# ml-jku/LRAM

Hardware: NVIDIA B200
Metric: env-steps/sec batched xLSTM recurrent inference (higher is better)
Workload: dtype f32

## Files before the change

include/xlstm_b200.h:

```cpp
#ifndef XLSTM_B200_H
#define XLSTM_B200_H

#include <stddef.h>
#include <stdint.h>

#ifdef __cplusplus
extern "C" {
#endif
#if defined(__GNUC__)
#pragma GCC visibility push(default)
#endif

#define XL_ABI_VERSION 3

typedef enum {
  XL_OK = 0,
  XL_ERR_INVALID_ARG = -1,
  XL_ERR_UNSUPPORTED = -2,
  XL_ERR_CUDA = -3,
  XL_ERR_NOT_READY = -4,
  XL_ERR_NO_DEVICE = -5
} xl_status;

typedef struct xl_handle xl_handle;

typedef struct {
  int32_t embedding_dim;
  int32_t num_blocks;
  int32_t num_heads;
  int32_t inner_dim;
  int32_t conv_kernel;
  int32_t qkv_blocksize;
  int32_t state_dim;
  int32_t act_dim;
  int32_t action_channels;
  int32_t discrete_actions;
  int32_t tokens_per_step;
  int32_t action_token_pos;
  int32_t max_batch;
  float ln_eps;
  float cell_eps;
  float embed_ln_eps;
  float tok_min_val;
  float tok_max_val;
  uint32_t slstm_mask_lo;
  uint32_t slstm_mask_hi;
  int32_t ffn_dim;
} xl_config;

typedef enum {
  XL_W_XLSTM_NORM = 0,
  XL_W_PROJ_UP = 1,
  XL_W_Q_PROJ = 2,
  XL_W_K_PROJ = 3,
  XL_W_V_PROJ = 4,
  XL_W_CONV_W = 5,
  XL_W_CONV_B = 6,
  XL_W_IGATE_W = 7,
  XL_W_IGATE_B = 8,
  XL_W_FGATE_W = 9,
  XL_W_FGATE_B = 10,
  XL_W_OUTNORM = 11,
  XL_W_SKIP = 12,
  XL_W_PROJ_DOWN = 13,
  XL_W_S_GATE_I = 14,
  XL_W_S_GATE_F = 15,
  XL_W_S_GATE_Z = 16,
  XL_W_S_GATE_O = 17,
  XL_W_S_RECURRENT = 18,
  XL_W_S_BIAS = 19,
  XL_W_S_GROUP_NORM = 20,
  XL_W_FFN_NORM = 21,
  XL_W_FFN_UP = 22,
  XL_W_FFN_DOWN = 23,
  XL_W_PER_BLOCK_COUNT = 24,
  XL_W_POST_NORM = 32,
  XL_W_EMBED_STATE_W = 33,
  XL_W_EMBED_STATE_B = 34,
  XL_W_EMBED_RETURN_W = 35,
  XL_W_EMBED_RETURN_B = 36,
  XL_W_EMBED_REWARD_W = 37,
  XL_W_EMBED_REWARD_B = 38,
  XL_W_EMBED_LN_W = 39,
  XL_W_EMBED_LN_B = 40,
  XL_W_HEAD_W = 41,
  XL_W_HEAD_B = 42
} xl_weight_id;

typedef enum { XL_STATE_C = 0, XL_STATE_N = 1, XL_STATE_M = 2, XL_STATE_CONV = 3, XL_STATE_SLSTM = 4 } xl_state_part;

#define XL_MODE_PER_TOKEN 0
#define XL_MODE_FUSED 1

#define XL_FLAG_DISCRETE 1u
#define XL_FLAG_GRAPH 2u
#define XL_FLAG_SIMPLE_GEMM 4u
#define XL_FLAG_STATE_EMBEDS 8u

int xl_abi_version(void);
const char* xl_last_error(void);

int xl_create(const xl_config* cfg, xl_handle** out);
void xl_destroy(xl_handle* h);

int xl_state_dim_padded(const xl_handle* h);

int xl_bind_weight(xl_handle* h, int layer, int which, const void* dev_ptr, int dtype, int64_t numel);
int xl_weights_ready(const xl_handle* h);
int xl_encoder_weights_ready(const xl_handle* h);

size_t xl_state_bytes(const xl_handle* h, int B);
int xl_state_layout(const xl_handle* h, int B, int layer, int part, size_t* offset_bytes, size_t* size_bytes);

int xl_state_reset(xl_handle* h, void* state, const uint8_t* env_mask, int B, void* stream);

int xl_set_token_ring(xl_handle* h, int32_t* ring, int slots, int next_slot, void* stream);

typedef struct {
  float temperature;
  float top_p;
  int32_t top_k;
  int32_t env_id_base;
  int32_t env_id_stride;
  uint64_t seed;
} xl_sampling;
int xl_set_sampling(xl_handle* h, const xl_sampling* params, uint32_t step0, void* stream);
int xl_sample_actions(xl_handle* h, const float* logits, int B, unsigned flags, const xl_sampling* params,
                      uint32_t step, int32_t* tokens, float* actions, void* stream);

int xl_encoder_step(xl_handle* h, void* state, const float* x_in, float* x_out, int B, int T, int mode,
                    unsigned flags, void* stream);

int xl_mlstm_cell_step(xl_handle* h, float* C, float* n, float* m, const float* qkv, const float* igate,
                       const float* fgate, const float* outnorm_w, float* h_norm, float* h_raw, int B, int T,
                       int rows_split, int cols_per_cta, void* stream);

int xl_policy_step(xl_handle* h, void* state, const float* states, const float* rtg, const float* rewards,
                   int32_t* tokens, float* actions, float* logits, float* hidden, int B, int mode,
                   unsigned flags, void* stream);

int xl_policy_step_host(xl_handle* h, void* state, const float* h_states, const float* h_rtg,
                        const float* h_rewards, int32_t* h_tokens, float* h_actions, int B, int mode,
                        unsigned flags, void* stream);

int xl_prefill(xl_handle* h, void* state, const float* x_in, float* y_out, int B, int S, unsigned flags, void* stream);

int xl_policy_prefill(xl_handle* h, void* state, const float* states, const float* rtg, const float* rewards, int B,
                      int Tn, unsigned flags, void* stream);

int xl_prefill_ragged(xl_handle* h, void* state, const float* x_in, float* y_out, const int32_t* lengths, int B, int S,
                      unsigned flags, void* stream);
int xl_policy_prefill_ragged(xl_handle* h, void* state, const float* states, const float* rtg, const float* rewards,
                             const int32_t* lengths, int B, int Tn, unsigned flags, void* stream);

typedef struct {
  int32_t* tokens;
  float* actions;
  float* logits;
  const int32_t* targets;
  float* logprobs;
} xl_seq_outputs;

int xl_policy_forward(xl_handle* h, void* state, const float* states, const float* rtg, const float* rewards,
                      const int32_t* lengths, int B, int Tn, const xl_seq_outputs* out, unsigned flags, void* stream);

int xl_policy_prefill_embeds(xl_handle* h, void* state, const float* state_embeds, const float* rtg,
                             const float* rewards, const int32_t* lengths, int B, int Tn, unsigned flags,
                             void* stream);
int xl_policy_forward_embeds(xl_handle* h, void* state, const float* state_embeds, const float* rtg,
                             const float* rewards, const int32_t* lengths, int B, int Tn, const xl_seq_outputs* out,
                             unsigned flags, void* stream);

int xl_linear(xl_handle* h, const float* A, const void* W_bf16, const float* bias, const float* residual,
              float* out, int M, int N, int K, int impl, void* stream);

int xl_set_option(xl_handle* h, const char* name, int value);

int64_t xl_launch_count(xl_handle* h);

int xl_profile_begin(xl_handle* h);
int xl_profile_end(xl_handle* h, double* state_kernel_ms, int64_t* state_kernel_launches, double* step_ms);

#if defined(__GNUC__)
#pragma GCC visibility pop
#endif
#ifdef __cplusplus
}
#endif
#endif
```

lram_b200/_lib.py:

```python
from __future__ import annotations

import ctypes as C
import os
import re

HERE = os.path.dirname(os.path.abspath(__file__))
LIB_PATH = os.path.join(HERE, "libxlstm_b200.so")
HEADER_PATH = os.path.join(os.path.dirname(HERE), "include", "xlstm_b200.h")

XL_OK = 0
XL_ERR_INVALID_ARG, XL_ERR_UNSUPPORTED, XL_ERR_CUDA, XL_ERR_NOT_READY, XL_ERR_NO_DEVICE = -1, -2, -3, -4, -5

XL_MODE_PER_TOKEN, XL_MODE_FUSED = 0, 1
XL_FLAG_DISCRETE, XL_FLAG_GRAPH, XL_FLAG_SIMPLE_GEMM, XL_FLAG_STATE_EMBEDS = 1, 2, 4, 8

XL_STATE_C, XL_STATE_N, XL_STATE_M, XL_STATE_CONV, XL_STATE_SLSTM = 0, 1, 2, 3, 4
XL_ABI_VERSION = 3

W = dict(
    XLSTM_NORM=0, PROJ_UP=1, Q_PROJ=2, K_PROJ=3, V_PROJ=4, CONV_W=5, CONV_B=6, IGATE_W=7, IGATE_B=8,
    FGATE_W=9, FGATE_B=10, OUTNORM=11, SKIP=12, PROJ_DOWN=13,
    S_GATE_I=14, S_GATE_F=15, S_GATE_Z=16, S_GATE_O=17, S_RECURRENT=18, S_BIAS=19, S_GROUP_NORM=20,
    FFN_NORM=21, FFN_UP=22, FFN_DOWN=23,
    POST_NORM=32, EMBED_STATE_W=33, EMBED_STATE_B=34, EMBED_RETURN_W=35, EMBED_RETURN_B=36,
    EMBED_REWARD_W=37, EMBED_REWARD_B=38, EMBED_LN_W=39, EMBED_LN_B=40, HEAD_W=41, HEAD_B=42,
)


class XLConfig(C.Structure):
    _fields_ = [
        ("embedding_dim", C.c_int32), ("num_blocks", C.c_int32), ("num_heads", C.c_int32),
        ("inner_dim", C.c_int32), ("conv_kernel", C.c_int32), ("qkv_blocksize", C.c_int32),
        ("state_dim", C.c_int32), ("act_dim", C.c_int32), ("action_channels", C.c_int32),
        ("discrete_actions", C.c_int32), ("tokens_per_step", C.c_int32), ("action_token_pos", C.c_int32),
        ("max_batch", C.c_int32),
        ("ln_eps", C.c_float), ("cell_eps", C.c_float), ("embed_ln_eps", C.c_float),
        ("tok_min_val", C.c_float), ("tok_max_val", C.c_float),
        ("slstm_mask_lo", C.c_uint32), ("slstm_mask_hi", C.c_uint32), ("ffn_dim", C.c_int32),
    ]


class XLSampling(C.Structure):
    _fields_ = [("temperature", C.c_float), ("top_p", C.c_float), ("top_k", C.c_int32), ("env_id_base", C.c_int32),
                ("env_id_stride", C.c_int32), ("seed", C.c_uint64)]


class XLSeqOutputs(C.Structure):
    _fields_ = [("tokens", C.c_void_p), ("actions", C.c_void_p), ("logits", C.c_void_p), ("targets", C.c_void_p),
                ("logprobs", C.c_void_p)]


class XLError(RuntimeError):
    def __init__(self, code: int, msg: str):
        super().__init__(f"xlstm_b200 error {code}: {msg}")
        self.code = code


_lib = None


def declared_symbols():
    with open(HEADER_PATH) as fh:
        src = fh.read()
    src = re.sub(r"/\*.*?\*/", "", src, flags=re.S)
    return sorted(set(re.findall(r"\b(xl_[a-z_0-9]+)\s*\(", src)))


def load():
    global _lib
    if _lib is not None:
        return _lib
    if not os.path.exists(LIB_PATH):
        from . import build as _build
        _build.build()
    if not os.path.exists(LIB_PATH):
        raise RuntimeError(f"{LIB_PATH} is missing and could not be built: the xlstm_b200 path has no "
                           f"CPU fallback")
    lib = C.CDLL(LIB_PATH)
    vp, i32, i64, u32, sz = C.c_void_p, C.c_int, C.c_int64, C.c_uint, C.c_size_t
    lib.xl_abi_version.restype = i32
    lib.xl_last_error.restype = C.c_char_p
    lib.xl_create.argtypes = [C.POINTER(XLConfig), C.POINTER(vp)]
    lib.xl_create.restype = i32
    lib.xl_destroy.argtypes = [vp]
    lib.xl_destroy.restype = None
    lib.xl_state_dim_padded.argtypes = [vp]
    lib.xl_state_dim_padded.restype = i32
    lib.xl_bind_weight.argtypes = [vp, i32, i32, vp, i32, i64]
    lib.xl_bind_weight.restype = i32
    lib.xl_weights_ready.argtypes = [vp]
    lib.xl_weights_ready.restype = i32
    lib.xl_encoder_weights_ready.argtypes = [vp]
    lib.xl_encoder_weights_ready.restype = i32
    lib.xl_state_bytes.argtypes = [vp, i32]
    lib.xl_state_bytes.restype = sz
    lib.xl_state_layout.argtypes = [vp, i32, i32, i32, C.POINTER(sz), C.POINTER(sz)]
    lib.xl_state_layout.restype = i32
    lib.xl_state_reset.argtypes = [vp, vp, vp, i32, vp]
    lib.xl_state_reset.restype = i32
    lib.xl_encoder_step.argtypes = [vp, vp, vp, vp, i32, i32, i32, u32, vp]
    lib.xl_encoder_step.restype = i32
    lib.xl_mlstm_cell_step.argtypes = [vp, vp, vp, vp, vp, vp, vp, vp, vp, vp, i32, i32, i32, i32, vp]
    lib.xl_mlstm_cell_step.restype = i32
    lib.xl_policy_step.argtypes = [vp, vp, vp, vp, vp, vp, vp, vp, vp, i32, i32, u32, vp]
    lib.xl_policy_step.restype = i32
    lib.xl_policy_step_host.argtypes = [vp, vp, vp, vp, vp, vp, vp, i32, i32, u32, vp]
    lib.xl_policy_step_host.restype = i32
    lib.xl_prefill.argtypes = [vp, vp, vp, vp, i32, i32, u32, vp]
    lib.xl_prefill.restype = i32
    lib.xl_policy_prefill.argtypes = [vp, vp, vp, vp, vp, i32, i32, u32, vp]
    lib.xl_policy_prefill.restype = i32
    lib.xl_prefill_ragged.argtypes = [vp, vp, vp, vp, vp, i32, i32, u32, vp]
    lib.xl_prefill_ragged.restype = i32
    lib.xl_policy_prefill_ragged.argtypes = [vp, vp, vp, vp, vp, vp, i32, i32, u32, vp]
    lib.xl_policy_prefill_ragged.restype = i32
    lib.xl_policy_forward.argtypes = [vp, vp, vp, vp, vp, vp, i32, i32, C.POINTER(XLSeqOutputs), u32, vp]
    lib.xl_policy_forward.restype = i32
    lib.xl_policy_prefill_embeds.argtypes = [vp, vp, vp, vp, vp, vp, i32, i32, u32, vp]
    lib.xl_policy_prefill_embeds.restype = i32
    lib.xl_policy_forward_embeds.argtypes = [vp, vp, vp, vp, vp, vp, i32, i32, C.POINTER(XLSeqOutputs), u32, vp]
    lib.xl_policy_forward_embeds.restype = i32
    lib.xl_linear.argtypes = [vp, vp, vp, vp, vp, vp, i32, i32, i32, i32, vp]
    lib.xl_linear.restype = i32
    lib.xl_set_token_ring.argtypes = [vp, vp, i32, i32, vp]
    lib.xl_set_token_ring.restype = i32
    lib.xl_set_sampling.argtypes = [vp, C.POINTER(XLSampling), u32, vp]
    lib.xl_set_sampling.restype = i32
    lib.xl_sample_actions.argtypes = [vp, vp, i32, u32, C.POINTER(XLSampling), u32, vp, vp, vp]
    lib.xl_sample_actions.restype = i32
    lib.xl_set_option.argtypes = [vp, C.c_char_p, i32]
    lib.xl_set_option.restype = i32
    lib.xl_profile_begin.argtypes = [vp]
    lib.xl_profile_begin.restype = i32
    lib.xl_profile_end.argtypes = [vp, C.POINTER(C.c_double), C.POINTER(i64), C.POINTER(C.c_double)]
    lib.xl_profile_end.restype = i32
    lib.xl_launch_count.argtypes = [vp]
    lib.xl_launch_count.restype = i64
    _lib = lib
    return lib


def check(rc: int):
    if rc != XL_OK:
        raise XLError(rc, load().xl_last_error().decode("utf-8", "replace"))
```

lram_b200/csrc/xl_api.cu:

```cuda
#include <cuda_bf16.h>
#include <cuda_runtime.h>

#include <algorithm>
#include <cmath>
#include <cstdarg>
#include <cstdio>
#include <cstring>
#include <new>
#include <utility>
#include <vector>

#include "../../include/xlstm_b200.h"
#include "xl_internal.h"

namespace {

thread_local char g_err[512] = "";

int fail(int code, const char* fmt, ...) {
  va_list ap;
  va_start(ap, fmt);
  vsnprintf(g_err, sizeof(g_err), fmt, ap);
  va_end(ap);
  return code;
}

#define XL_CUDA(expr)                                                                          \
  do {                                                                                         \
    cudaError_t _e = (expr);                                                                   \
    if (_e != cudaSuccess)                                                                     \
      return fail(XL_ERR_CUDA, "%s failed: %s (%s:%d)", #expr, cudaGetErrorString(_e), __FILE__, \
                  __LINE__);                                                                   \
  } while (0)

inline size_t align_up(size_t v, size_t a) { return (v + a - 1) / a * a; }

struct BlockWeights {
  const void* w[XL_W_PER_BLOCK_COUNT];
};

struct GraphCacheEntry {
  cudaGraphExec_t exec = nullptr;
  void* state = nullptr;
  const void *states = nullptr, *rtg = nullptr, *rewards = nullptr;
  void *tokens = nullptr, *actions = nullptr, *logits = nullptr, *hidden = nullptr;
  int B = 0, mode = 0;
  unsigned flags = 0;
  int64_t launches = 0;
};

}

constexpr int kCntRing = 0, kCntSample = 1, kCntUnitStep = 2, kCntArmed = 8, kCntUnit = 16;
constexpr int kMaxMicro = 8;
constexpr int kSplitMax = 8;
constexpr size_t kSplitRows = 1024;

struct xl_handle {
  xl_config cfg;
  int device = 0;
  int num_sms = 148;
  int DH = 0, NCH = 0, Kpad = 0, head_out = 0, num_actions = 0;
  uint64_t slstm_mask = 0;
  std::vector<BlockWeights> blocks;
  const void* pw[16];
  char* ws = nullptr;
  size_t ws_bytes = 0;
  float *x = nullptr, *xn = nullptr, *u = nullptr, *qkv = nullptr, *act = nullptr, *gate_part = nullptr,
        *gated = nullptr, *partial = nullptr, *s_emb = nullptr, *states_pad = nullptr, *logits = nullptr,
        *d_states = nullptr, *d_rtg = nullptr, *d_rew = nullptr, *d_actions = nullptr, *xtok = nullptr, *hid = nullptr;
  float* d_embeds = nullptr;
  int32_t* d_tokens = nullptr;
  unsigned int* counters = nullptr;
  __nv_bfloat16 *a_hi = nullptr, *a_lo = nullptr;
  int64_t launches = 0;
  std::vector<GraphCacheEntry> graphs;
  size_t a_cap = 0;
  size_t a_env = 0;
  int num_tickets = 0;
  cudaStream_t cap_stream = nullptr;
  cudaStream_t side[kMaxMicro - 1] = {};
  cudaEvent_t ev_fork = nullptr, ev_join[kMaxMicro - 1] = {}, ev_state[kMaxMicro] = {};
  int state_impl = 1;
  int state_stages = 0;
  int state_ctas_per_sm = 0;
  int state_rows_split = 0;
  int fuse_ends = 1;
  int up_fuse = 0;
  int gp_chunks = 16;
  int state_fuse = 0;
  int small_state_fuse = 0;
  int gemm_impl = 0;
  int gemm_splitk = 8;
  int gemm_up_bn = 0, gemm_up_splits = 0, gemm_down_bn = 0, gemm_down_splits = 0;
  int debug_skip = 0;
  float *part_up = nullptr, *part_down = nullptr;
  size_t part_rows = 0;
  int l2_prefetch_policy = 0;
  int conv_impl = 2;
  int microbatches = 0;
  int pipeline_order = 1;
  int l2_prefetch_mb = -1;
  char* pf_buf = nullptr;
  int pf_rows = 0;
  size_t pf_gsc_floats = 0;
  float *pf_x = nullptr, *pf_xn = nullptr, *pf_u = nullptr, *pf_qkv = nullptr, *pf_act = nullptr, *pf_gp = nullptr,
        *pf_gated = nullptr, *pf_num = nullptr, *pf_qn = nullptr, *pf_f = nullptr, *pf_i = nullptr, *pf_m = nullptr,
        *pf_semb = nullptr, *pf_spad = nullptr, *pf_sin = nullptr, *pf_rtg = nullptr, *pf_rew = nullptr, *pf_gsc = nullptr;
  __nv_bfloat16 *pf_hi = nullptr, *pf_lo = nullptr;
  uint8_t *pf_pc = nullptr, *pf_pv = nullptr;
  char* rg_state = nullptr;
  size_t rg_state_bytes = 0;
  int32_t* rg_idx = nullptr;
  std::vector<int32_t> rg_host;
  float* sq_logits = nullptr;
  size_t sq_logits_floats = 0;
  int prefill_gemm_2cta = 0;
  int prefill_rows = 16384;
  char* pf_tc = nullptr;
  size_t pf_tc_bytes = 0;
  int prefill_cell = 2;
  int smallm = -1;
  int host_zero_copy = 1;
  std::vector<std::pair<const void*, void*>> host_map;
  int32_t* tok_ring = nullptr;
  int tok_slots = 0;
  bool sampling = false;
  bool profiling = false;
  std::vector<cudaEvent_t> prof_state;
  std::vector<cudaEvent_t> prof_step;
};

namespace {

struct StateLayout {
  size_t c_off, n_off, m_off, conv_off, layer_bytes;
  size_t s_off, sconv_off, slayer_bytes;
};

inline bool is_slstm(const xl_handle* h, int i) { return (h->slstm_mask >> i) & 1ull; }

StateLayout state_layout(const xl_handle* h, int B) {
  const xl_config& c = h->cfg;
  StateLayout L;
  size_t off = 0;
  L.c_off = off;
  off = align_up(off + sizeof(float) * (size_t)B * c.num_heads * h->DH * h->DH, 256);
  L.n_off = off;
  off = align_up(off + sizeof(float) * (size_t)B * c.num_heads * h->DH, 256);
  L.m_off = off;
  off = align_up(off + sizeof(float) * (size_t)B * c.num_heads, 256);
  L.conv_off = off;
  off = align_up(off + sizeof(float) * (size_t)B * c.conv_kernel * c.inner_dim, 256);
  L.layer_bytes = off;
  off = 0;
  L.s_off = off;
  off = align_up(off + sizeof(float) * (size_t)4 * B * c.embedding_dim, 256);
  L.sconv_off = off;
  off = align_up(off + sizeof(float) * (size_t)B * c.conv_kernel * c.embedding_dim, 256);
  L.slayer_bytes = off;
  return L;
}

size_t layer_base(const xl_handle* h, const StateLayout& L, int i) {
  const uint64_t below = i >= 64 ? ~0ull : ((1ull << i) - 1ull);
  const int ns = __builtin_popcountll(h->slstm_mask & below);
  return (size_t)(i - ns) * L.layer_bytes + (size_t)ns * L.slayer_bytes;
}

int check_batch(const xl_handle* h, int B) {
  if (!h) return fail(XL_ERR_INVALID_ARG, "null handle");
  if (B <= 0 || B > h->cfg.max_batch)
    return fail(XL_ERR_INVALID_ARG, "B=%d outside [1, max_batch=%d]", B, h->cfg.max_batch);
  return XL_OK;
}

struct Ws {
  float *x, *xn, *xtok, *hid, *u, *qkv, *act, *gate_part, *gated, *partial, *s_emb, *states_pad, *logits;
  __nv_bfloat16 *a_hi, *a_lo;
  size_t a_cap;
  int low_smem;
};

Ws ws_slice(const xl_handle* h, int b0, int Bk) {
  const xl_config& c = h->cfg;
  const size_t d = c.embedding_dim, inner = c.inner_dim, e = (size_t)b0;
  Ws w;
  w.x = h->x + e * 4 * d; w.xn = h->xn + e * 4 * d; w.xtok = h->xtok + e * 4 * d; w.hid = h->hid + e * 4 * d;
  w.u = h->u + e * 4 * 2 * inner; w.qkv = h->qkv + e * 4 * 3 * inner; w.act = h->act + e * 4 * inner;
  w.gate_part = h->gate_part + e * 4 * h->gp_chunks * 2 * c.num_heads; w.gated = h->gated + e * 4 * inner;
  w.partial = h->partial + e * c.num_heads * 32 * 4 * h->DH;
  w.s_emb = h->s_emb + e * d; w.states_pad = h->states_pad + e * h->Kpad; w.logits = h->logits + e * h->head_out;
  w.a_hi = h->a_hi + e * h->a_env; w.a_lo = h->a_lo + e * h->a_env;
  w.a_cap = (size_t)Bk * h->a_env;
  w.low_smem = 0;
  return w;
}

int linear(xl_handle* h, const Ws& w, const float* A, const void* W, const float* bias, const float* residual,
           float* out, int M, int N, int K, int impl, cudaStream_t s, bool presplit = false, int bn = 0,
           int splits = 1, long long split_stride = 0) {
  if (K % 8 != 0) return fail(XL_ERR_UNSUPPORTED, "linear: K=%d must be a multiple of 8", K);
  const bool tc_ok = xl::gemm_tc_supported(M, N, K) && (size_t)M * K <= w.a_cap;
  if (impl == 2 && !tc_ok)
    return fail(XL_ERR_UNSUPPORTED, "linear: tcgen05 path needs K %% 64 == 0 and M*K <= %zu (got M=%d K=%d)",
                w.a_cap, M, K);
  if (impl == 2 || (impl == 0 && tc_ok)) {
    if (!presplit) {
      xl::launch_split_bf16(A, K, w.a_hi, w.a_lo, M, K, s);
      h->launches += 1;
    }
    XL_CUDA(xl::launch_gemm_tc(w.a_hi, w.a_lo, (const __nv_bfloat16*)W, bias, residual, out, M, N, K,
                               h->num_sms, bn, splits, split_stride, w.low_smem, s));
    h->launches += 1;
    return XL_OK;
  }
  if (splits > 1) return fail(XL_ERR_INVALID_ARG, "linear: split-K needs the tcgen05 path");
  xl::launch_gemm_simple(A, (const __nv_bfloat16*)W, bias, residual, out, M, N, K, s);
  h->launches += 1;
  XL_CUDA(cudaGetLastError());
  return XL_OK;
}

struct Slice {
  int B, b0, Bk;
  Ws ws;
  cudaStream_t s;
};

Slice make_slice(const xl_handle* h, int B, int b0, int Bk, cudaStream_t s) {
  Slice sl;
  sl.B = B; sl.b0 = b0; sl.Bk = Bk; sl.s = s;
  sl.ws = ws_slice(h, b0, Bk);
  return sl;
}

int smallm_chunks(const xl_handle* h, const Slice& sl, int T, unsigned flags) {
  const xl_config& c = h->cfg;
  if (!h->smallm || h->debug_skip || (flags & XL_FLAG_SIMPLE_GEMM)) return 0;
  if (h->smallm < 0 && (sl.Bk * T > 4 || c.embedding_dim > 1024)) return 0;
  if (sl.b0 != 0 || sl.Bk != sl.B || sl.ws.low_smem) return 0;
  return xl::smallm_pre_chunks(sl.Bk, T, c.embedding_dim, c.inner_dim, c.num_heads, c.conv_kernel);
}

constexpr unsigned kFlagLn0DoneEarly = 1u << 29;
constexpr unsigned kFlagHeadOnlyEarly = 1u << 28;

struct BlockPlan {
  bool tc_up, tc_down;
  bool up_fused;
  int impl;
  int up_bn, up_sp, down_bn, down_sp;
};

BlockPlan block_plan(const xl_handle* h, const Slice& sl, int T, unsigned flags) {
  const xl_config& c = h->cfg;
  const int M = sl.Bk * T;
  BlockPlan p;
  p.impl = (flags & XL_FLAG_SIMPLE_GEMM) ? 1 : h->gemm_impl;
  p.tc_up = p.impl != 1 && xl::gemm_tc_supported(M, 2 * c.inner_dim, c.embedding_dim) &&
            (size_t)M * c.embedding_dim <= sl.ws.a_cap;
  p.tc_down = p.impl != 1 && xl::gemm_tc_supported(M, c.embedding_dim, c.inner_dim) &&
              (size_t)M * c.inner_dim <= sl.ws.a_cap;
  const bool can_split = !sl.ws.low_smem && sl.b0 == 0 && (size_t)M <= h->part_rows && c.embedding_dim <= 4096 &&
                         !smallm_chunks(h, sl, T, flags);
  const int max_sp = can_split ? std::min(std::max(h->gemm_splitk, 1), kSplitMax) : 1;
  p.up_bn = p.down_bn = 0;
  p.up_sp = p.down_sp = 1;
  if (p.tc_up) {
    xl::gemm_tc_plan(M, 2 * c.inner_dim, c.embedding_dim, h->num_sms, max_sp, &p.up_bn, &p.up_sp);
    if (h->gemm_up_bn) p.up_bn = h->gemm_up_bn;
    if (h->gemm_up_splits && can_split && (c.embedding_dim / 64) % h->gemm_up_splits == 0 &&
        h->gemm_up_splits <= kSplitMax)
      p.up_sp = h->gemm_up_splits;
  }
  p.up_fused = h->up_fuse && p.tc_up && !sl.ws.low_smem && !h->debug_skip && !smallm_chunks(h, sl, T, flags) &&
               xl::gemm_up_conv_chunks(c.inner_dim) <= h->gp_chunks &&
               xl::gemm_up_conv_supported(T, c.conv_kernel, c.num_heads, c.inner_dim, c.embedding_dim);
  if (p.up_fused) { p.up_bn = 64; p.up_sp = 1; }
  if (p.tc_down) {
    xl::gemm_tc_plan(M, c.embedding_dim, c.inner_dim, h->num_sms, max_sp, &p.down_bn, &p.down_sp);
    if (h->gemm_down_bn) p.down_bn = h->gemm_down_bn;
    if (h->gemm_down_splits && can_split && (c.inner_dim / 64) % h->gemm_down_splits == 0 &&
        h->gemm_down_splits <= kSplitMax)
      p.down_sp = h->gemm_down_splits;
  }
  return p;
}

xl::StateStepParams state_params(const xl_handle* h, void* state, const Slice& sl, int i, int T, bool tc_down,
                                 int up_sp = 1, int small_nch = 0, bool up_fused = false) {
  const xl_config& c = h->cfg;
  const int inner = c.inner_dim, NH = c.num_heads, DH = h->DH;
  const StateLayout L = state_layout(h, sl.B);
  const BlockWeights& w = h->blocks[i];
  char* base = (char*)state + layer_base(h, L, i);
  const int M = sl.Bk * T;
  xl::StateStepParams sp;
  memset(&sp, 0, sizeof(sp));
  sp.C = (float*)(base + L.c_off) + (size_t)sl.b0 * NH * DH * DH;
  sp.n = (float*)(base + L.n_off) + (size_t)sl.b0 * NH * DH;
  sp.m = (float*)(base + L.m_off) + (size_t)sl.b0 * NH;
  sp.qk = sl.ws.qkv;
  sp.v = sl.ws.qkv + (size_t)2 * M * inner;
  sp.gate_part = sl.ws.gate_part;
  sp.igate_b = (const float*)w.w[XL_W_IGATE_B];
  sp.fgate_b = (const float*)w.w[XL_W_FGATE_B];
  sp.outnorm_w = (const float*)w.w[XL_W_OUTNORM];
  sp.skip = (const float*)w.w[XL_W_SKIP];
  sp.act = sl.ws.act;
  sp.u = up_sp > 1 ? h->part_up : sl.ws.u;
  sp.u_splits = up_sp;
  sp.u_stride = (int64_t)M * 2 * inner;
  sp.out = tc_down ? nullptr : sl.ws.gated;
  sp.out_hi = tc_down ? sl.ws.a_hi : nullptr;
  sp.out_lo = tc_down ? sl.ws.a_lo : nullptr;
  sp.partial = sl.ws.partial;
  sp.B = sl.Bk; sp.T = T; sp.NH = NH; sp.DH = DH; sp.inner = inner; sp.NCH = h->NCH;
  if (small_nch) sp.NCH = small_nch;
  if (up_fused) sp.NCH = xl::gemm_up_conv_chunks(inner);
  sp.ln_eps = c.ln_eps; sp.cell_eps = c.cell_eps;
  sp.impl = h->state_impl; sp.num_layers = c.num_blocks;
  sp.stages = h->state_stages; sp.ctas_per_sm = h->state_ctas_per_sm; sp.rows_split = h->state_rows_split;
  sp.fuse_finalize = (h->debug_skip & (8 | 16)) ? 0 : h->state_fuse;
  if (small_nch && h->state_fuse == 0 && h->small_state_fuse) {
    sp.fuse_finalize = 2;
    sp.max_cluster = h->small_state_fuse > 1 ? h->small_state_fuse : 0;
  }
  if (sl.ws.low_smem) {
    if (sp.stages <= 0) sp.stages = 4;
    sp.meta_slots = 2;
  }
  return sp;
}

int block_pre(xl_handle* h, void* state, const Slice& sl, int i, int T, unsigned flags) {
  const xl_config& c = h->cfg;
  const int d = c.embedding_dim, inner = c.inner_dim, NH = c.num_heads;
  const int M = sl.Bk * T;
  const StateLayout L = state_layout(h, sl.B);
  const BlockPlan bp = block_plan(h, sl, T, flags);
  const BlockWeights& w = h->blocks[i];
  const Ws& ws = sl.ws;
  char* base = (char*)state + layer_base(h, L, i);
  if (const int nch = smallm_chunks(h, sl, T, flags)) {
    xl::SmallPreParams sp;
    memset(&sp, 0, sizeof(sp));
    sp.x = ws.x;
    sp.norm_w = (const float*)w.w[XL_W_XLSTM_NORM];
    sp.w_up = (const __nv_bfloat16*)w.w[XL_W_PROJ_UP];
    sp.conv_w = (const float*)w.w[XL_W_CONV_W]; sp.conv_b = (const float*)w.w[XL_W_CONV_B];
    sp.wq = (const float*)w.w[XL_W_Q_PROJ]; sp.wk = (const float*)w.w[XL_W_K_PROJ]; sp.wv = (const float*)w.w[XL_W_V_PROJ];
    sp.wi = (const float*)w.w[XL_W_IGATE_W]; sp.wf = (const float*)w.w[XL_W_FGATE_W];
    sp.conv_state = (float*)(base + L.conv_off);
    sp.u = ws.u; sp.qk = ws.qkv; sp.v = ws.qkv + (size_t)2 * M * inner; sp.act = ws.act;
    sp.gate_part = ws.gate_part;
    sp.B = sl.Bk; sp.T = T; sp.d = d; sp.inner = inner; sp.NH = NH; sp.NCH = nch;
    sp.ln_eps = c.ln_eps;
    XL_CUDA(xl::launch_smallm_pre(sp, sl.s));
    h->launches += 1;
    return XL_OK;
  }
  if (h->debug_skip & 1) {
  } else if (i == 0 && (flags & kFlagLn0DoneEarly)) {
    h->launches -= 1;
  } else if (i > 0 && bp.down_sp > 1 && !is_slstm(h, i - 1)) {
    xl::launch_ln_rows_reduce(ws.x, h->part_down, bp.down_sp, (int64_t)M * d, bp.tc_up ? nullptr : ws.xn, d,
                              (const float*)w.w[XL_W_XLSTM_NORM], c.ln_eps, M, d, bp.tc_up ? ws.a_hi : nullptr,
                              bp.tc_up ? ws.a_lo : nullptr, sl.s);
  } else {
    xl::launch_ln_rows(ws.x, d, bp.tc_up ? nullptr : ws.xn, d, (const float*)w.w[XL_W_XLSTM_NORM], nullptr, 1,
                       c.ln_eps, M, d, bp.tc_up ? ws.a_hi : nullptr, bp.tc_up ? ws.a_lo : nullptr, sl.s);
  }
  h->launches += 1;
  if (bp.up_fused) {
    xl::UpEpiParams ep;
    ep.conv_state = (float*)(base + L.conv_off) + (size_t)sl.b0 * c.conv_kernel * inner;
    ep.conv_w = (const float*)w.w[XL_W_CONV_W]; ep.conv_b = (const float*)w.w[XL_W_CONV_B];
    ep.wq = (const float*)w.w[XL_W_Q_PROJ]; ep.wk = (const float*)w.w[XL_W_K_PROJ]; ep.wv = (const float*)w.w[XL_W_V_PROJ];
    ep.wi = (const float*)w.w[XL_W_IGATE_W]; ep.wf = (const float*)w.w[XL_W_FGATE_W];
    ep.qk = ws.qkv; ep.v = ws.qkv + (size_t)2 * M * inner; ep.act = ws.act; ep.gate_part = ws.gate_part;
    ep.B = sl.Bk; ep.T = T; ep.inner = inner; ep.NCH = xl::gemm_up_conv_chunks(inner);
    XL_CUDA(xl::launch_gemm_up_conv(ws.a_hi, ws.a_lo, (const __nv_bfloat16*)w.w[XL_W_PROJ_UP], ws.u, M, d, ep, sl.s));
    h->launches += 1;
    return XL_OK;
  }
  int rc = (h->debug_skip & 2) ? 0 : linear(h, ws, ws.xn, w.w[XL_W_PROJ_UP], nullptr, nullptr,
                  bp.up_sp > 1 ? h->part_up : ws.u, M, 2 * inner,
                  d, bp.impl, sl.s, bp.tc_up, bp.up_bn, bp.up_sp, (long long)M * 2 * inner);
  if (rc) return rc;
  if (h->debug_skip & 4) return XL_OK;
  xl::ConvQkvParams cp;
  cp.u = bp.up_sp > 1 ? h->part_up : ws.u;
  cp.u_splits = bp.up_sp;
  cp.u_stride = (int64_t)M * 2 * inner;
  cp.conv_state = (float*)(base + L.conv_off) + (size_t)sl.b0 * c.conv_kernel * inner;
  cp.conv_w = (const float*)w.w[XL_W_CONV_W];
  cp.conv_b = (const float*)w.w[XL_W_CONV_B];
  cp.wq = (const float*)w.w[XL_W_Q_PROJ];
  cp.wk = (const float*)w.w[XL_W_K_PROJ];
  cp.wv = (const float*)w.w[XL_W_V_PROJ];
  cp.wi = (const float*)w.w[XL_W_IGATE_W];
  cp.wf = (const float*)w.w[XL_W_FGATE_W];
  cp.qk = ws.qkv;
  cp.v = ws.qkv + (size_t)2 * M * inner;
  cp.act = ws.act;
  cp.gate_part = ws.gate_part;
  cp.B = sl.Bk; cp.T = T; cp.inner = inner; cp.NH = NH; cp.KS = c.conv_kernel; cp.NCH = h->NCH;
  cp.impl = h->conv_impl;
  if (!xl::launch_conv_qkv_gates(cp, sl.s))
    return fail(XL_ERR_UNSUPPORTED, "conv/qkv kernel not instantiated for KS=%d T=%d NH=%d", cp.KS, cp.T, cp.NH);
  h->launches += 1;
  return XL_OK;
}

int block_state(xl_handle* h, void* state, const Slice& sl, int i, int T, unsigned flags) {
  const BlockPlan bp = block_plan(h, sl, T, flags);
  const int small_nch = smallm_chunks(h, sl, T, flags);
  const xl::StateStepParams sp = small_nch ? state_params(h, state, sl, i, T, false, 1, small_nch)
                                           : state_params(h, state, sl, i, T, bp.tc_down, bp.up_sp, 0, bp.up_fused);
  cudaEvent_t pe0 = nullptr, pe1 = nullptr;
  if (h->profiling) {
    XL_CUDA(cudaEventCreate(&pe0));
    XL_CUDA(cudaEventCreate(&pe1));
    XL_CUDA(cudaEventRecord(pe0, sl.s));
  }
  if (!(h->debug_skip & 8)) XL_CUDA(xl::launch_state_step(sp, h->num_sms, sl.s));
  h->launches += 1;
  if (h->profiling) {
    XL_CUDA(cudaEventRecord(pe1, sl.s));
    h->prof_state.push_back(pe0);
    h->prof_state.push_back(pe1);
  }
  return XL_OK;
}

int block_post(xl_handle* h, void* state, const Slice& sl, int i, int T, unsigned flags) {
  const xl_config& c = h->cfg;
  const BlockPlan bp = block_plan(h, sl, T, flags);
  const int small_nch = smallm_chunks(h, sl, T, flags);
  const Ws& ws = sl.ws;
  const int M = sl.Bk * T;
  if (small_nch) {
    xl::StateStepParams sp = state_params(h, state, sl, i, T, false, 1, small_nch);
    const bool fused = xl::state_step_fuses_finalize(sp, h->num_sms);
    if (!fused) XL_CUDA(xl::launch_state_finalize(sp, h->num_sms, sl.s));
    xl::SmallDownParams dp;
    dp.g = ws.gated; dp.w_down = (const __nv_bfloat16*)h->blocks[i].w[XL_W_PROJ_DOWN]; dp.x = ws.x;
    dp.M = M; dp.d = c.embedding_dim; dp.inner = c.inner_dim;
    XL_CUDA(xl::launch_smallm_down(dp, sl.s));
    h->launches += fused ? 1 : 2;
    return XL_OK;
  }
  const xl::StateStepParams sp = state_params(h, state, sl, i, T, bp.tc_down, bp.up_sp, small_nch, bp.up_fused);
  if (!xl::state_step_fuses_finalize(sp, h->num_sms)) {
    if (!(h->debug_skip & 16)) XL_CUDA(xl::launch_state_finalize(sp, h->num_sms, sl.s));
    h->launches += 1;
  }
  if (h->debug_skip & 32) return XL_OK;
  if (bp.down_sp > 1)
    return linear(h, ws, ws.gated, h->blocks[i].w[XL_W_PROJ_DOWN], nullptr, nullptr, h->part_down, M,
                  c.embedding_dim, c.inner_dim, bp.impl, sl.s, bp.tc_down, bp.down_bn, bp.down_sp,
                  (long long)M * c.embedding_dim);
  return linear(h, ws, ws.gated, h->blocks[i].w[XL_W_PROJ_DOWN], nullptr, ws.x, ws.x, M, c.embedding_dim,
                c.inner_dim, bp.impl, sl.s, bp.tc_down, bp.down_bn);
}

int slstm_block(xl_handle* h, void* state, const Ws& ws, int Btot, int b0, int Bk, int i, int T, unsigned flags,
                int pend_sp, cudaStream_t s, const int32_t* len = nullptr, int pos = 0) {
  const xl_config& c = h->cfg;
  const int d = c.embedding_dim, NH = c.num_heads, ff = c.ffn_dim, KS = c.conv_kernel, M = Bk * T;
  const StateLayout L = state_layout(h, Btot);
  const BlockWeights& w = h->blocks[i];
  char* base = (char*)state + layer_base(h, L, i);
  float* st = (float*)(base + L.s_off) + (size_t)b0 * d;
  float* conv = (float*)(base + L.sconv_off) + (size_t)b0 * KS * d;
  const int impl = (flags & XL_FLAG_SIMPLE_GEMM) ? 1 : h->gemm_impl;
  const bool tc_up = impl != 1 && xl::gemm_tc_supported(M, 2 * ff, d) && (size_t)M * d <= ws.a_cap;
  const bool tc_down = impl != 1 && xl::gemm_tc_supported(M, d, ff) && (size_t)M * ff <= ws.a_cap;
  auto F = [&](int id) { return (const float*)w.w[id]; };
  if (pend_sp > 1)
    xl::launch_ln_rows_reduce(ws.x, h->part_down, pend_sp, (int64_t)M * d, ws.xn, d, F(XL_W_XLSTM_NORM), c.ln_eps, M,
                              d, nullptr, nullptr, s);
  else
    xl::launch_ln_rows(ws.x, d, ws.xn, d, F(XL_W_XLSTM_NORM), nullptr, 1, c.ln_eps, M, d, nullptr, nullptr, s);
  if (!xl::launch_slstm_conv(ws.xn, conv, F(XL_W_CONV_W), F(XL_W_CONV_B), ws.act, Bk, T, d, KS, s, len, pos))
    return fail(XL_ERR_UNSUPPORTED, "sLSTM conv kernel not instantiated for KS=%d", KS);
  xl::launch_slstm_gates(ws.act, ws.xn, F(XL_W_S_GATE_I), F(XL_W_S_GATE_F), F(XL_W_S_GATE_Z), F(XL_W_S_GATE_O),
                         F(XL_W_S_BIAS), ws.u, M, d, NH, s);
  for (int t = 0; t < T; ++t)
    XL_CUDA(xl::launch_slstm_cell(ws.u, F(XL_W_S_RECURRENT), st, ws.gated, Bk, Btot, T, t, d, NH, s, len, pos));
  xl::launch_slstm_out(ws.gated, F(XL_W_S_GROUP_NORM), ws.x, st, M, T, d, NH, c.ln_eps, s);
  xl::launch_ln_rows(ws.x, d, tc_up ? nullptr : ws.xn, d, F(XL_W_FFN_NORM), nullptr, 1, c.ln_eps, M, d,
                     tc_up ? ws.a_hi : nullptr, tc_up ? ws.a_lo : nullptr, s);
  h->launches += 5 + T;
  int rc = linear(h, ws, ws.xn, w.w[XL_W_FFN_UP], nullptr, nullptr, ws.qkv, M, 2 * ff, d, impl, s, tc_up);
  if (rc) return rc;
  xl::launch_ffn_gate(ws.qkv, tc_down ? nullptr : ws.gated, tc_down ? ws.a_hi : nullptr, tc_down ? ws.a_lo : nullptr,
                      M, ff, s);
  h->launches += 1;
  rc = linear(h, ws, ws.gated, w.w[XL_W_FFN_DOWN], nullptr, ws.x, ws.x, M, d, ff, impl, s, tc_down);
  if (rc) return rc;
  XL_CUDA(cudaGetLastError());
  return XL_OK;
}

int pending_planes(const xl_handle* h, const Slice& sl, int i, int T, unsigned flags) {
  if (i == 0 || is_slstm(h, i - 1)) return 1;
  return block_plan(h, sl, T, flags).down_sp;
}

void final_norm(xl_handle* h, const Slice& sl, int T, unsigned flags, float* out, int64_t out_stride) {
  const xl_config& c = h->cfg;
  const int d = c.embedding_dim, M = sl.Bk * T;
  const BlockPlan bp = block_plan(h, sl, T, flags);
  const float* post_w = (const float*)h->pw[XL_W_POST_NORM - XL_W_POST_NORM];
  if (bp.down_sp > 1 && !is_slstm(h, c.num_blocks - 1))
    xl::launch_ln_rows_reduce(sl.ws.x, h->part_down, bp.down_sp, (int64_t)M * d, out, out_stride, post_w, c.ln_eps,
                              M, d, nullptr, nullptr, sl.s);
  else
    xl::launch_ln_rows(sl.ws.x, d, out, out_stride, post_w, nullptr, 1, c.ln_eps, M, d, nullptr, nullptr, sl.s);
  h->launches += 1;
}

int run_blocks(xl_handle* h, void* state, const Slice& sl, int T, unsigned flags) {
  const int L = h->cfg.num_blocks;
  const StateLayout lay = state_layout(h, sl.B);
  const size_t c_bytes = sizeof(float) * (size_t)sl.B * h->cfg.num_heads * h->DH * h->DH;
  int warm_mb = h->l2_prefetch_mb;
  if (warm_mb < 0) warm_mb = (c_bytes >= ((size_t)100 << 20) && c_bytes <= ((size_t)300 << 20)) ? 48 : 0;
  const bool warm = warm_mb > 0 && sl.b0 == 0 && sl.Bk == sl.B && L > 1;
  const size_t warm_bytes = std::min(c_bytes, (size_t)warm_mb << 20);
  int rc = XL_OK;
  for (int i = 0; i < L && !rc; ++i) {
    if (is_slstm(h, i)) {
      rc = slstm_block(h, state, sl.ws, sl.B, sl.b0, sl.Bk, i, T, flags, pending_planes(h, sl, i, T, flags), sl.s);
      continue;
    }
    rc = block_pre(h, state, sl, i, T, flags);
    if (!rc) rc = block_state(h, state, sl, i, T, flags);
    if (!rc && warm) {
      XL_CUDA(cudaEventRecord(h->ev_state[0], sl.s));
      XL_CUDA(cudaStreamWaitEvent(h->side[0], h->ev_state[0], 0));
      int nx = (i + 1) % L;
      while (is_slstm(h, nx) && nx != i) nx = (nx + 1) % L;
      const char* next_c = (const char*)state + layer_base(h, lay, nx) + lay.c_off;
      xl::launch_l2_prefetch(next_c, warm_bytes, h->num_sms, h->l2_prefetch_policy, h->side[0]);
      h->launches += 1;
    }
    if (!rc) rc = block_post(h, state, sl, i, T, flags);
  }
  if (warm) {
    cudaEventRecord(h->ev_join[0], h->side[0]);
    cudaStreamWaitEvent(sl.s, h->ev_join[0], 0);
  }
  if (rc) return rc;
  XL_CUDA(cudaGetLastError());
  return XL_OK;
}

int run_encoder(xl_handle* h, void* state, const Slice& sl, const float* x_in, float* x_out, int T, int mode,
                unsigned flags) {
  const xl_config& c = h->cfg;
  const int d = c.embedding_dim;
  const int B = sl.Bk;
  const Ws& ws = sl.ws;
  cudaStream_t s = sl.s;
  const float* post_w = (const float*)h->pw[XL_W_POST_NORM - XL_W_POST_NORM];
  if (mode == XL_MODE_FUSED || T == 1) {
    if (x_in != ws.x) {
      XL_CUDA(cudaMemcpyAsync(ws.x, x_in, sizeof(float) * (size_t)B * T * d, cudaMemcpyDeviceToDevice, s));
    }
    int rc = run_blocks(h, state, sl, T, flags);
    if (rc) return rc;
    if (!(flags & kFlagHeadOnlyEarly)) final_norm(h, sl, T, flags, x_out, d);
  } else if (mode == XL_MODE_PER_TOKEN) {
    const float* src = x_in;
    if (x_in == x_out) {
      XL_CUDA(cudaMemcpyAsync(ws.xtok, x_in, sizeof(float) * (size_t)B * T * d, cudaMemcpyDeviceToDevice, s));
      src = ws.xtok;
    }
    for (int t = 0; t < T; ++t) {
      xl::launch_copy_rows(src + (size_t)t * d, (int64_t)T * d, ws.x, d, B, d, s);
      h->launches += 1;
      int rc = run_blocks(h, state, sl, 1, flags);
      if (rc) return rc;
      final_norm(h, sl, 1, flags, x_out + (size_t)t * d, (int64_t)T * d);
    }
  } else {
    return fail(XL_ERR_INVALID_ARG, "unknown mode %d", mode);
  }
  XL_CUDA(cudaGetLastError());
  return XL_OK;
}

constexpr unsigned kFlagLn0Done = 1u << 29;
constexpr unsigned kFlagHeadOnly = 1u << 28;
constexpr unsigned kFlagNoRing = 1u << 30;

struct StepArgs {
  void* state;
  const float *states, *rtg, *rewards;
  int32_t* tokens;
  float *actions, *logits, *hidden;
  int B, mode;
  unsigned flags;
};

int policy_front(xl_handle* h, const StepArgs& a, const Slice& sl, float* xt) {
  const xl_config& c = h->cfg;
  const int d = c.embedding_dim;
  const int impl = (a.flags & XL_FLAG_SIMPLE_GEMM) ? 1 : h->gemm_impl;
  auto PW = [&](int id) { return h->pw[id - XL_W_POST_NORM]; };
  const Ws& ws = sl.ws;
  const float* s_emb = ws.s_emb;
  if (a.flags & XL_FLAG_STATE_EMBEDS) {
    s_emb = a.states + (size_t)sl.b0 * d;
  } else {
    const bool tc = impl != 1 && xl::gemm_tc_supported(sl.Bk, d, h->Kpad) && (size_t)sl.Bk * h->Kpad <= ws.a_cap;
    if (tc) {
      xl::launch_pad_split(a.states + (size_t)sl.b0 * c.state_dim, c.state_dim, ws.a_hi, ws.a_lo, h->Kpad, sl.Bk, sl.s);
    } else {
      xl::launch_pad_rows(a.states + (size_t)sl.b0 * c.state_dim, c.state_dim, ws.states_pad, h->Kpad, sl.Bk, sl.s);
    }
    h->launches += 1;
    int rc = linear(h, ws, ws.states_pad, PW(XL_W_EMBED_STATE_W), (const float*)PW(XL_W_EMBED_STATE_B), nullptr,
                    ws.s_emb, sl.Bk, d, h->Kpad, impl, sl.s, tc);
    if (rc) return rc;
  }
  const float* ln0_w = nullptr;
  float* xn0 = nullptr;
  void *hi0 = nullptr, *lo0 = nullptr;
  if (a.flags & kFlagLn0Done) {
    const BlockPlan bp = block_plan(h, sl, c.tokens_per_step, a.flags);
    ln0_w = (const float*)h->blocks[0].w[XL_W_XLSTM_NORM];
    if (bp.tc_up) { hi0 = ws.a_hi; lo0 = ws.a_lo; } else { xn0 = ws.xn; }
  }
  xl::launch_embed_tokens(s_emb, a.rtg + sl.b0, a.rewards ? a.rewards + sl.b0 : nullptr,
                          (const float*)PW(XL_W_EMBED_RETURN_W), (const float*)PW(XL_W_EMBED_RETURN_B),
                          (const float*)PW(XL_W_EMBED_REWARD_W), (const float*)PW(XL_W_EMBED_REWARD_B),
                          (const float*)PW(XL_W_EMBED_LN_W), (const float*)PW(XL_W_EMBED_LN_B), c.embed_ln_eps, xt,
                          sl.Bk, d, (h->tok_ring && sl.b0 == 0 && !(a.flags & kFlagNoRing)) ? h->counters + kCntRing : nullptr,
                          (h->sampling && sl.b0 == 0 && !(a.flags & kFlagNoRing)) ? h->counters + kCntSample : nullptr,
                          ln0_w, c.ln_eps, xn0, hi0, lo0, sl.s);
  h->launches += 1;
  return XL_OK;
}

int policy_back(xl_handle* h, const StepArgs& a, const Slice& sl, const float* hid) {
  const xl_config& c = h->cfg;
  const int d = c.embedding_dim, T = c.tokens_per_step;
  const int impl = (a.flags & XL_FLAG_SIMPLE_GEMM) ? 1 : h->gemm_impl;
  auto PW = [&](int id) { return h->pw[id - XL_W_POST_NORM]; };
  const Ws& ws = sl.ws;
  cudaStream_t s = sl.s;
  const int Bk = sl.Bk;
  float* xa = ws.s_emb;
  const bool head_only = (a.flags & kFlagHeadOnly) != 0;
  if (head_only) {
    const BlockPlan bp = block_plan(h, sl, T, a.flags);
    const int pend = is_slstm(h, c.num_blocks - 1) ? 1 : bp.down_sp;
    xl::launch_ln_rows_gather(ws.x, h->part_down, pend, (int64_t)Bk * T * d, (const float*)PW(XL_W_POST_NORM), c.ln_eps,
                              Bk, d, T, c.action_token_pos, ws.a_hi, ws.a_lo, s);
  } else {
    xl::launch_copy_rows(hid + (size_t)c.action_token_pos * d, (int64_t)T * d, xa, d, Bk, d, s);
  }
  h->launches += 1;
  const bool discrete = (a.flags & XL_FLAG_DISCRETE) != 0;
  const int n_out = discrete ? h->num_actions : h->head_out;
  int32_t* tokens = a.tokens + (size_t)sl.b0 * c.act_dim;
  float* actions = a.actions + (size_t)sl.b0 * c.act_dim;
  float* logits = a.logits ? a.logits + (size_t)sl.b0 * n_out : nullptr;
  int rc;
  int32_t* ring = (h->tok_ring && !(a.flags & kFlagNoRing)) ? h->tok_ring + (size_t)sl.b0 * c.act_dim : nullptr;
  const int64_t ring_stride = (int64_t)a.B * c.act_dim;
  const bool sample = h->sampling && !(a.flags & kFlagNoRing);
  const float bw = (c.tok_max_val - c.tok_min_val) / (float)c.action_channels;
  if (discrete) {
    rc = linear(h, ws, xa, PW(XL_W_HEAD_W), (const float*)PW(XL_W_HEAD_B), nullptr, ws.logits, Bk, n_out, d, impl, s,
                head_only);
    if (rc) return rc;
    if (logits) {
      XL_CUDA(cudaMemcpyAsync(logits, ws.logits, sizeof(float) * (size_t)Bk * n_out, cudaMemcpyDeviceToDevice, s));
    }
    if (sample)
      xl::launch_sample_tokens(ws.logits, n_out, Bk, c.act_dim, n_out, c.discrete_actions, 1, 0.f, 0.f, tokens, actions,
                               ring, h->counters + kCntRing, h->tok_slots, ring_stride, h->counters + kCntArmed,
                               h->counters + kCntSample, sl.b0, s);
    else
      xl::launch_argmax_tokens(ws.logits, n_out, Bk, c.act_dim, n_out, c.discrete_actions, 1, 0.f, 0.f, tokens,
                               actions, ring, h->counters + kCntRing, h->tok_slots, ring_stride, s);
  } else {
    float* lg = logits ? logits : ws.logits;
    rc = linear(h, ws, xa, PW(XL_W_HEAD_W), (const float*)PW(XL_W_HEAD_B), nullptr, lg, Bk, n_out, d, impl, s, head_only);
    if (rc) return rc;
    if (sample)
      xl::launch_sample_tokens(lg, h->head_out, Bk, c.act_dim, h->num_actions, c.discrete_actions, 0, bw, c.tok_min_val,
                               tokens, actions, ring, h->counters + kCntRing, h->tok_slots, ring_stride,
                               h->counters + kCntArmed, h->counters + kCntSample, sl.b0, s);
    else
      xl::launch_argmax_tokens(lg, h->head_out, Bk, c.act_dim, h->num_actions, c.discrete_actions, 0, bw,
                               c.tok_min_val, tokens, actions, ring, h->counters + kCntRing, h->tok_slots, ring_stride, s);
  }
  h->launches += 1;
  return XL_OK;
}

int pick_microbatches(const xl_handle* h, int B, int mode) {
  if (mode != XL_MODE_FUSED) return 1;
  int mb = h->microbatches > 0 ? h->microbatches : 1;
  if (mb > kMaxMicro) mb = kMaxMicro;
  if (mb > B) mb = B;
  return mb < 1 ? 1 : mb;
}

int run_policy(xl_handle* h, const StepArgs& a, cudaStream_t s) {
  const xl_config& c = h->cfg;
  const int d = c.embedding_dim, T = c.tokens_per_step;
  const float* post_w = (const float*)h->pw[XL_W_POST_NORM - XL_W_POST_NORM];
  const int MB = pick_microbatches(h, a.B, a.mode);
  if (MB == 1) {
    const Slice sl = make_slice(h, a.B, 0, a.B, s);
    float* xt = (a.mode == XL_MODE_FUSED) ? sl.ws.x : sl.ws.xtok;
    StepArgs af = a;
    if (h->fuse_ends && a.mode == XL_MODE_FUSED && !h->debug_skip) {
      if (!is_slstm(h, 0) && !smallm_chunks(h, sl, T, a.flags)) af.flags |= kFlagLn0Done;
      const int impl = (a.flags & XL_FLAG_SIMPLE_GEMM) ? 1 : h->gemm_impl;
      const int n_out = (a.flags & XL_FLAG_DISCRETE) ? h->num_actions : h->head_out;
      if (!a.hidden && impl != 1 && xl::gemm_tc_supported(a.B, n_out, d) && (size_t)a.B * d <= sl.ws.a_cap &&
          d <= 4096)
        af.flags |= kFlagHeadOnly;
    }
    const StepArgs& a = af;
    int rc = policy_front(h, a, sl, xt);
    if (rc) return rc;
    float* hid = a.hidden ? a.hidden : sl.ws.hid;
    rc = run_encoder(h, a.state, sl, xt, hid, T, a.mode, a.flags);
    if (rc) return rc;
    rc = policy_back(h, a, sl, hid);
    if (rc) return rc;
    XL_CUDA(cudaGetLastError());
    return XL_OK;
  }
  Slice sl[kMaxMicro];
  int b0 = 0;
  for (int k = 0; k < MB; ++k) {
    const int Bk = a.B / MB + (k < a.B % MB ? 1 : 0);
    sl[k] = make_slice(h, a.B, b0, Bk, k == 0 ? s : h->side[k - 1]);
    sl[k].ws.low_smem = 1;
    b0 += Bk;
  }
  XL_CUDA(cudaEventRecord(h->ev_fork, s));
  for (int k = 1; k < MB; ++k) XL_CUDA(cudaStreamWaitEvent(sl[k].s, h->ev_fork, 0));
  int rc = XL_OK;
  for (int k = 0; k < MB && !rc; ++k) rc = policy_front(h, a, sl[k], sl[k].ws.x);
  for (int i = 0; i < c.num_blocks && !rc; ++i) {
    if (is_slstm(h, i)) {
      for (int k = 0; k < MB && !rc; ++k)
        rc = slstm_block(h, a.state, sl[k].ws, a.B, sl[k].b0, sl[k].Bk, i, T, a.flags,
                         pending_planes(h, sl[k], i, T, a.flags), sl[k].s);
      continue;
    }
    for (int k = 0; k < MB && !rc; ++k) rc = block_pre(h, a.state, sl[k], i, T, a.flags);
    for (int k = 0; k < MB && !rc; ++k) {
      if (h->pipeline_order && !(i == 0 && k == 0)) {
        XL_CUDA(cudaStreamWaitEvent(sl[k].s, h->ev_state[(k + MB - 1) % MB], 0));
      }
      rc = block_state(h, a.state, sl[k], i, T, a.flags);
      if (!rc && h->pipeline_order) XL_CUDA(cudaEventRecord(h->ev_state[k], sl[k].s));
    }
    for (int k = 0; k < MB && !rc; ++k) rc = block_post(h, a.state, sl[k], i, T, a.flags);
  }
  for (int k = 0; k < MB && !rc; ++k) {
    float* hid = a.hidden ? a.hidden + (size_t)sl[k].b0 * T * d : sl[k].ws.hid;
    final_norm(h, sl[k], T, a.flags, hid, d);
    rc = policy_back(h, a, sl[k], hid);
  }
  for (int k = 1; k < MB; ++k) {
    cudaEventRecord(h->ev_join[k - 1], sl[k].s);
    cudaStreamWaitEvent(s, h->ev_join[k - 1], 0);
  }
  if (rc) return rc;
  XL_CUDA(cudaGetLastError());
  return XL_OK;
}

int ensure_prefill_ws(xl_handle* h, int rows, size_t gsc_floats) {
  if (rows <= h->pf_rows && gsc_floats <= h->pf_gsc_floats) return XL_OK;
  rows = std::max(rows, h->pf_rows);
  gsc_floats = std::max(gsc_floats, h->pf_gsc_floats);
  const xl_config& c = h->cfg;
  const size_t d = c.embedding_dim, inner = c.inner_dim, NH = c.num_heads, R = (size_t)rows;
  const size_t kmax = std::max(std::max(inner, d), (size_t)h->Kpad);
  size_t off = 0;
  auto carve = [&](size_t bytes) {
    size_t o = off;
    off = align_up(off + bytes, 256);
    return o;
  };
  const size_t o_x = carve(4 * R * d), o_xn = carve(4 * R * d), o_u = carve(4 * R * 2 * inner);
  const size_t o_qkv = carve(4 * R * 3 * inner), o_act = carve(4 * R * inner), o_gp = carve(4 * R * 16 * 2 * NH);
  const size_t o_gated = carve(4 * R * inner), o_num = carve(4 * R * inner), o_qn = carve(4 * R * NH);
  const size_t o_f = carve(4 * R * NH), o_i = carve(4 * R * NH), o_m = carve(4 * R * NH);
  const size_t o_semb = carve(4 * R * d), o_spad = carve(4 * R * h->Kpad), o_sin = carve(4 * R * c.state_dim);
  const size_t o_rtg = carve(4 * R), o_rew = carve(4 * R);
  const size_t o_gsc = carve(4 * gsc_floats);
  const size_t o_hi = carve(2 * R * kmax), o_lo = carve(2 * R * kmax);
  size_t pc_bytes = 0, pv_bytes = 0;
  if (xl::prefill_cell_mma_supported(h->DH)) xl::prefill_cell_mma_ws(rows, (int)NH, h->DH, &pc_bytes, &pv_bytes);
  const size_t o_pc = carve(pc_bytes), o_pv = carve(pv_bytes);
  XL_CUDA(cudaDeviceSynchronize());
  if (h->pf_buf) cudaFree(h->pf_buf);
  h->pf_buf = nullptr;
  h->pf_rows = 0;
  h->pf_gsc_floats = 0;
  cudaError_t e = cudaMalloc((void**)&h->pf_buf, off);
  if (e != cudaSuccess) return fail(XL_ERR_CUDA, "cudaMalloc(prefill workspace %zu B) failed: %s", off, cudaGetErrorString(e));
  char* b = h->pf_buf;
  h->pf_x = (float*)(b + o_x); h->pf_xn = (float*)(b + o_xn); h->pf_u = (float*)(b + o_u);
  h->pf_qkv = (float*)(b + o_qkv); h->pf_act = (float*)(b + o_act); h->pf_gp = (float*)(b + o_gp);
  h->pf_gated = (float*)(b + o_gated); h->pf_num = (float*)(b + o_num); h->pf_qn = (float*)(b + o_qn);
  h->pf_f = (float*)(b + o_f); h->pf_i = (float*)(b + o_i); h->pf_m = (float*)(b + o_m);
  h->pf_semb = (float*)(b + o_semb); h->pf_spad = (float*)(b + o_spad); h->pf_sin = (float*)(b + o_sin);
  h->pf_rtg = (float*)(b + o_rtg); h->pf_rew = (float*)(b + o_rew);
  h->pf_gsc = (float*)(b + o_gsc);
  h->pf_hi = (__nv_bfloat16*)(b + o_hi); h->pf_lo = (__nv_bfloat16*)(b + o_lo);
  h->pf_pc = (uint8_t*)(b + o_pc); h->pf_pv = (uint8_t*)(b + o_pv);
  h->pf_rows = rows;
  h->pf_gsc_floats = gsc_floats;
  return XL_OK;
}

int ensure_prefill_tc_ws(xl_handle* h, int B, int Sc) {
  const size_t need = xl::prefill_cell_tc_ws_bytes(B, Sc, h->cfg.num_heads, h->DH);
  if (need <= h->pf_tc_bytes) return XL_OK;
  XL_CUDA(cudaDeviceSynchronize());
  if (h->pf_tc) cudaFree(h->pf_tc);
  h->pf_tc = nullptr;
  h->pf_tc_bytes = 0;
  cudaError_t e = cudaMalloc((void**)&h->pf_tc, need);
  if (e != cudaSuccess) return fail(XL_ERR_CUDA, "cudaMalloc(prefill cell workspace %zu B) failed: %s", need, cudaGetErrorString(e));
  h->pf_tc_bytes = need;
  return XL_OK;
}

Ws prefill_ws(const xl_handle* h) {
  Ws w;
  memset(&w, 0, sizeof(w));
  w.x = h->pf_x; w.xn = h->pf_xn; w.u = h->pf_u; w.qkv = h->pf_qkv; w.act = h->pf_act; w.gate_part = h->pf_gp;
  w.gated = h->pf_gated; w.s_emb = h->pf_semb; w.states_pad = h->pf_spad;
  w.a_hi = h->pf_hi; w.a_lo = h->pf_lo;
  const size_t kmax = std::max(std::max((size_t)h->cfg.inner_dim, (size_t)h->cfg.embedding_dim), (size_t)h->Kpad);
  w.a_cap = (size_t)h->pf_rows * kmax;
  w.low_smem = h->prefill_gemm_2cta;
  return w;
}

int prefill_chunk_tokens(const xl_handle* h, int B) {
  int sc = h->prefill_rows / B;
  if (sc < 48) sc = 48;
  return sc / 48 * 48;
}

int prefill_blocks(xl_handle* h, void* state, int Btot, int B, int Sc, unsigned flags, cudaStream_t s,
                   const int32_t* len = nullptr, int pos = 0) {
  const xl_config& c = h->cfg;
  const int d = c.embedding_dim, inner = c.inner_dim, NH = c.num_heads, DH = h->DH;
  const int M = B * Sc;
  const StateLayout L = state_layout(h, Btot);
  const Ws ws = prefill_ws(h);
  const int impl = (flags & XL_FLAG_SIMPLE_GEMM) ? 1 : h->gemm_impl;
  const bool tc_up = impl != 1 && xl::gemm_tc_supported(M, 2 * inner, d) && (size_t)M * d <= ws.a_cap;
  const bool tc_down = impl != 1 && xl::gemm_tc_supported(M, d, inner) && (size_t)M * inner <= ws.a_cap;
// ... 378 lines not shown
  const size_t o_semb = carve(4 * B * d), o_sp = carve(4 * B * h->Kpad), o_lg = carve(4 * B * h->head_out);
  const size_t o_ds = carve(4 * B * c.state_dim), o_dr = carve(4 * B), o_dw = carve(4 * B);
  const size_t o_da = carve(4 * B * c.act_dim), o_dt = carve(4 * B * c.act_dim);
  h->num_tickets = 4096;
  const size_t o_cnt = carve(4 * (size_t)h->num_tickets);

  size_t a_cap = M * (inner > d ? inner : d);
  if (a_cap < B * (size_t)h->Kpad) a_cap = B * (size_t)h->Kpad;
  if (a_cap < (size_t)1 << 20) a_cap = (size_t)1 << 20;
  h->a_cap = a_cap;
  h->a_env = 4 * (inner > d ? inner : d);
  const size_t o_hi = carve(2 * a_cap), o_lo = carve(2 * a_cap);
  h->part_rows = M < kSplitRows ? M : kSplitRows;
  const size_t o_pu = carve(4 * (size_t)kSplitMax * h->part_rows * 2 * inner);
  const size_t o_pd = carve(4 * (size_t)kSplitMax * h->part_rows * d);
  const size_t o_de = carve(4 * B * d);
  h->ws_bytes = off;
  cudaError_t e = cudaMalloc((void**)&h->ws, h->ws_bytes);
  if (e != cudaSuccess) {
    delete h;
    return fail(XL_ERR_CUDA, "cudaMalloc(workspace %zu B) failed: %s", off, cudaGetErrorString(e));
  }
  cudaMemset(h->ws, 0, h->ws_bytes);
  cudaStreamCreateWithFlags(&h->cap_stream, cudaStreamNonBlocking);
  for (int k = 0; k < kMaxMicro - 1; ++k) {
    cudaStreamCreateWithFlags(&h->side[k], cudaStreamNonBlocking);
    cudaEventCreateWithFlags(&h->ev_join[k], cudaEventDisableTiming);
  }
  for (int k = 0; k < kMaxMicro; ++k) cudaEventCreateWithFlags(&h->ev_state[k], cudaEventDisableTiming);
  cudaEventCreateWithFlags(&h->ev_fork, cudaEventDisableTiming);
  h->x = (float*)(h->ws + o_x); h->xn = (float*)(h->ws + o_xn); h->xtok = (float*)(h->ws + o_xtok);
  h->hid = (float*)(h->ws + o_hid);
  h->u = (float*)(h->ws + o_u); h->qkv = (float*)(h->ws + o_qkv); h->act = (float*)(h->ws + o_act);
  h->gate_part = (float*)(h->ws + o_gp); h->gated = (float*)(h->ws + o_gated);
  h->partial = (float*)(h->ws + o_part); h->s_emb = (float*)(h->ws + o_semb);
  h->states_pad = (float*)(h->ws + o_sp); h->logits = (float*)(h->ws + o_lg);
  h->d_states = (float*)(h->ws + o_ds); h->d_rtg = (float*)(h->ws + o_dr); h->d_rew = (float*)(h->ws + o_dw);
  h->d_actions = (float*)(h->ws + o_da); h->d_tokens = (int32_t*)(h->ws + o_dt);
  h->counters = (unsigned int*)(h->ws + o_cnt);

  h->a_hi = (__nv_bfloat16*)(h->ws + o_hi); h->a_lo = (__nv_bfloat16*)(h->ws + o_lo);
  h->part_up = (float*)(h->ws + o_pu); h->part_down = (float*)(h->ws + o_pd);
  h->d_embeds = (float*)(h->ws + o_de);
  *out = h;
  return XL_OK;
}

void xl_destroy(xl_handle* h) {
  if (!h) return;
  for (auto& g : h->graphs)
    if (g.exec) cudaGraphExecDestroy(g.exec);
  if (h->ws) cudaFree(h->ws);
  if (h->pf_tc) cudaFree(h->pf_tc);
  if (h->pf_buf) cudaFree(h->pf_buf);
  if (h->rg_state) cudaFree(h->rg_state);
  if (h->rg_idx) cudaFree(h->rg_idx);
  if (h->sq_logits) cudaFree(h->sq_logits);
  if (h->cap_stream) cudaStreamDestroy(h->cap_stream);
  for (int k = 0; k < kMaxMicro - 1; ++k) {
    if (h->side[k]) cudaStreamDestroy(h->side[k]);
    if (h->ev_join[k]) cudaEventDestroy(h->ev_join[k]);
  }
  for (int k = 0; k < kMaxMicro; ++k)
    if (h->ev_state[k]) cudaEventDestroy(h->ev_state[k]);
  if (h->ev_fork) cudaEventDestroy(h->ev_fork);
  delete h;
}

int xl_state_dim_padded(const xl_handle* h) { return h ? h->Kpad : 0; }

int xl_bind_weight(xl_handle* h, int layer, int which, const void* dev_ptr, int dtype, int64_t numel) {
  if (!h || !dev_ptr) return fail(XL_ERR_INVALID_ARG, "null argument");
  const xl_config& c = h->cfg;
  const int64_t d = c.embedding_dim, inner = c.inner_dim, NH = c.num_heads, KS = c.conv_kernel;
  int64_t want = -1;
  int want_dtype = 0;
  if (layer >= 0) {
    if (layer >= c.num_blocks) return fail(XL_ERR_INVALID_ARG, "layer %d >= num_blocks", layer);
    const int64_t DHs = d / NH, ff = c.ffn_dim;
    if (is_slstm(h, layer)) switch (which) {
      case XL_W_XLSTM_NORM: case XL_W_CONV_B: case XL_W_S_GROUP_NORM: case XL_W_FFN_NORM: want = d; break;
      case XL_W_CONV_W: want = d * KS; break;
      case XL_W_S_GATE_I: case XL_W_S_GATE_F: case XL_W_S_GATE_Z: case XL_W_S_GATE_O: want = NH * DHs * DHs; break;
      case XL_W_S_RECURRENT: want = NH * DHs * 4 * DHs; break;
      case XL_W_S_BIAS: want = NH * 4 * DHs; break;
      case XL_W_FFN_UP: want = 2 * ff * d; want_dtype = 1; break;
      case XL_W_FFN_DOWN: want = d * ff; want_dtype = 1; break;
      default: return fail(XL_ERR_INVALID_ARG, "weight id %d does not belong to an sLSTM block (layer %d)", which, layer);
    }
    else switch (which) {
      case XL_W_XLSTM_NORM: want = d; break;
      case XL_W_PROJ_UP: want = 2 * inner * d; want_dtype = 1; break;
      case XL_W_Q_PROJ: case XL_W_K_PROJ: case XL_W_V_PROJ: want = inner * 4; break;
      case XL_W_CONV_W: want = inner * KS; break;
      case XL_W_CONV_B: want = inner; break;
      case XL_W_IGATE_W: case XL_W_FGATE_W: want = NH * 3 * inner; break;
      case XL_W_IGATE_B: case XL_W_FGATE_B: want = NH; break;
      case XL_W_OUTNORM: case XL_W_SKIP: want = inner; break;
      case XL_W_PROJ_DOWN: want = d * inner; want_dtype = 1; break;
      default: return fail(XL_ERR_INVALID_ARG, "unknown per-block weight id %d", which);
    }
  } else {
    switch (which) {
      case XL_W_POST_NORM: want = d; break;
      case XL_W_EMBED_STATE_W: want = d * h->Kpad; want_dtype = 1; break;
      case XL_W_EMBED_STATE_B: case XL_W_EMBED_RETURN_W: case XL_W_EMBED_RETURN_B:
      case XL_W_EMBED_REWARD_W: case XL_W_EMBED_REWARD_B: case XL_W_EMBED_LN_W: case XL_W_EMBED_LN_B:
        want = d; break;
      case XL_W_HEAD_W: want = (int64_t)h->head_out * d; want_dtype = 1; break;
      case XL_W_HEAD_B: want = h->head_out; break;
      default: return fail(XL_ERR_INVALID_ARG, "unknown policy weight id %d", which);
    }
  }
  if (numel != want) return fail(XL_ERR_INVALID_ARG, "weight %d (layer %d): numel %lld, expected %lld", which,
                                 layer, (long long)numel, (long long)want);
  if (dtype != want_dtype)
    return fail(XL_ERR_INVALID_ARG, "weight %d (layer %d): dtype %d, expected %d (0=fp32,1=bf16)", which, layer,
                dtype, want_dtype);
  if (((uintptr_t)dev_ptr) % 16) return fail(XL_ERR_INVALID_ARG, "weight pointer must be 16-byte aligned");
  if (layer >= 0) h->blocks[layer].w[which] = dev_ptr;
  else h->pw[which - XL_W_POST_NORM] = dev_ptr;
  for (auto& g : h->graphs)
    if (g.exec) cudaGraphExecDestroy(g.exec);
  h->graphs.clear();
  return XL_OK;
}

static int weights_ready(const xl_handle* h, bool encoder_only) {
  if (!h) return fail(XL_ERR_INVALID_ARG, "null handle");
  static const int s_ids[] = {XL_W_XLSTM_NORM, XL_W_CONV_W, XL_W_CONV_B, XL_W_S_GATE_I, XL_W_S_GATE_F, XL_W_S_GATE_Z,
                              XL_W_S_GATE_O, XL_W_S_RECURRENT, XL_W_S_BIAS, XL_W_S_GROUP_NORM, XL_W_FFN_NORM,
                              XL_W_FFN_UP, XL_W_FFN_DOWN};
  for (int i = 0; i < h->cfg.num_blocks; ++i) {
    if (is_slstm(h, i)) {
      for (int k : s_ids)
        if (!h->blocks[i].w[k]) return fail(XL_ERR_NOT_READY, "sLSTM block %d weight id %d not bound", i, k);
      continue;
    }
    for (int k = 0; k <= XL_W_PROJ_DOWN; ++k)
      if (!h->blocks[i].w[k]) return fail(XL_ERR_NOT_READY, "block %d weight id %d not bound", i, k);
  }
  const int last = encoder_only ? XL_W_POST_NORM : XL_W_HEAD_B;
  for (int id = XL_W_POST_NORM; id <= last; ++id)
    if (!h->pw[id - XL_W_POST_NORM]) return fail(XL_ERR_NOT_READY, "policy weight id %d not bound", id);
  return XL_OK;
}

int xl_weights_ready(const xl_handle* h) { return weights_ready(h, false); }

int xl_encoder_weights_ready(const xl_handle* h) { return weights_ready(h, true); }

size_t xl_state_bytes(const xl_handle* h, int B) {
  if (!h || B <= 0) return 0;
  return layer_base(h, state_layout(h, B), h->cfg.num_blocks);
}

int xl_state_layout(const xl_handle* h, int B, int layer, int part, size_t* offset_bytes, size_t* size_bytes) {
  if (!h || !offset_bytes || !size_bytes) return fail(XL_ERR_INVALID_ARG, "null argument");
  if (layer < 0 || layer >= h->cfg.num_blocks || B <= 0) return fail(XL_ERR_INVALID_ARG, "bad layer/B");
  const StateLayout L = state_layout(h, B);
  const xl_config& c = h->cfg;
  size_t o, sz;
  if (is_slstm(h, layer)) {
    switch (part) {
      case XL_STATE_SLSTM: o = L.s_off; sz = sizeof(float) * (size_t)4 * B * c.embedding_dim; break;
      case XL_STATE_CONV: o = L.sconv_off; sz = sizeof(float) * (size_t)B * c.conv_kernel * c.embedding_dim; break;
      default: return fail(XL_ERR_INVALID_ARG, "state part %d does not exist in sLSTM block %d", part, layer);
    }
    *offset_bytes = layer_base(h, L, layer) + o;
    *size_bytes = sz;
    return XL_OK;
  }
  switch (part) {
    case XL_STATE_C: o = L.c_off; sz = sizeof(float) * (size_t)B * c.num_heads * h->DH * h->DH; break;
    case XL_STATE_N: o = L.n_off; sz = sizeof(float) * (size_t)B * c.num_heads * h->DH; break;
    case XL_STATE_M: o = L.m_off; sz = sizeof(float) * (size_t)B * c.num_heads; break;
    case XL_STATE_CONV: o = L.conv_off; sz = sizeof(float) * (size_t)B * c.conv_kernel * c.inner_dim; break;
    default: return fail(XL_ERR_INVALID_ARG, "bad state part %d", part);
  }
  *offset_bytes = layer_base(h, L, layer) + o;
  *size_bytes = sz;
  return XL_OK;
}

int xl_state_reset(xl_handle* h, void* state, const uint8_t* env_mask, int B, void* stream) {
  int rc = check_batch(h, B);
  if (rc) return rc;
  if (!state) return fail(XL_ERR_INVALID_ARG, "null state");
  cudaStream_t s = (cudaStream_t)stream;
  const StateLayout L = state_layout(h, B);
  const xl_config& c = h->cfg;
  if (!env_mask) {
    XL_CUDA(cudaMemsetAsync(state, 0, layer_base(h, L, c.num_blocks), s));
    return XL_OK;
  }
  for (int i = 0; i < c.num_blocks; ++i) {
    char* base = (char*)state + layer_base(h, L, i);
    if (is_slstm(h, i)) {
      const int64_t d = c.embedding_dim, Bd = (int64_t)B * d;
      float* st = (float*)(base + L.s_off);
      xl::launch_state_reset((float*)(base + L.sconv_off), st, st + Bd, st + 2 * Bd, env_mask, B,
                             (int64_t)c.conv_kernel * d, d, d, d, s);
      xl::launch_state_reset(nullptr, st + 3 * Bd, nullptr, nullptr, env_mask, B, 0, d, 0, 0, s);
      h->launches += 2;
      continue;
    }
    xl::launch_state_reset((float*)(base + L.c_off), (float*)(base + L.n_off), (float*)(base + L.m_off),
                           (float*)(base + L.conv_off), env_mask, B, (int64_t)c.num_heads * h->DH * h->DH,
                           (int64_t)c.num_heads * h->DH, c.num_heads, (int64_t)c.conv_kernel * c.inner_dim, s);
    h->launches += 1;
  }
  XL_CUDA(cudaGetLastError());
  return XL_OK;
}

int xl_encoder_step(xl_handle* h, void* state, const float* x_in, float* x_out, int B, int T, int mode,
                    unsigned flags, void* stream) {
  int rc = check_batch(h, B);
  if (rc) return rc;
  if (!state || !x_in || !x_out) return fail(XL_ERR_INVALID_ARG, "null argument");
  if (T < 1 || T > 4) return fail(XL_ERR_UNSUPPORTED, "T=%d outside [1,4]", T);
  rc = weights_ready(h, true);
  if (rc) return rc;
  cudaStream_t s = (cudaStream_t)stream;
  if (!(flags & XL_FLAG_GRAPH) || h->profiling) {
    const Slice sl = make_slice(h, B, 0, B, s);
    return run_encoder(h, state, sl, x_in, x_out, T, mode, flags & ~(unsigned)XL_FLAG_GRAPH);
  }
  const int key_mode = mode | (T << 8) | (1 << 16);
  for (auto& g : h->graphs) {
    if (g.state == state && g.states == x_in && g.hidden == x_out && !g.rtg && !g.tokens && g.B == B &&
        g.mode == key_mode && g.flags == flags) {
      XL_CUDA(cudaGraphLaunch(g.exec, s));
      h->launches += g.launches;
      return XL_OK;
    }
  }
  GraphCacheEntry g;
  g.state = state; g.states = x_in; g.hidden = x_out; g.B = B; g.mode = key_mode; g.flags = flags;
  cudaGraph_t graph = nullptr;
  const int64_t before = h->launches;
  XL_CUDA(cudaStreamBeginCapture(h->cap_stream, cudaStreamCaptureModeThreadLocal));
  {
    const Slice sl = make_slice(h, B, 0, B, h->cap_stream);
    rc = run_encoder(h, state, sl, x_in, x_out, T, mode, flags & ~(unsigned)XL_FLAG_GRAPH);
  }
  cudaError_t e = cudaStreamEndCapture(h->cap_stream, &graph);
  g.launches = h->launches - before;
  h->launches = before;
  if (rc) {
    if (graph) cudaGraphDestroy(graph);
    return rc;
  }
  if (e != cudaSuccess) return fail(XL_ERR_CUDA, "cudaStreamEndCapture: %s", cudaGetErrorString(e));
  e = cudaGraphInstantiate(&g.exec, graph, 0);
  cudaGraphDestroy(graph);
  if (e != cudaSuccess) return fail(XL_ERR_CUDA, "cudaGraphInstantiate: %s", cudaGetErrorString(e));
  if (h->graphs.size() >= 8) {
    cudaGraphExecDestroy(h->graphs.front().exec);
    h->graphs.erase(h->graphs.begin());
  }
  h->graphs.push_back(g);
  XL_CUDA(cudaGraphLaunch(g.exec, s));
  h->launches += g.launches;
  return XL_OK;
}

int xl_mlstm_cell_step(xl_handle* h, float* C, float* n, float* m, const float* qkv, const float* igate,
                       const float* fgate, const float* outnorm_w, float* h_norm, float* h_raw, int B, int T,
                       int rows_split, int cols_per_cta, void* stream) {
  int rc = check_batch(h, B);
  if (rc) return rc;
  if (!C || !n || !m || !qkv || !igate || !fgate || !outnorm_w || !h_norm)
    return fail(XL_ERR_INVALID_ARG, "null argument");
  if (T < 1 || T > 4) return fail(XL_ERR_UNSUPPORTED, "T=%d outside [1,4]", T);
  if (rows_split > 32) return fail(XL_ERR_UNSUPPORTED, "rows_split > 32");
  const xl_config& c = h->cfg;
  cudaStream_t s = (cudaStream_t)stream;
  const int M = B * T, NH = c.num_heads;
  XL_CUDA(cudaMemcpy2DAsync(h->gate_part, sizeof(float) * 2 * NH, igate, sizeof(float) * NH, sizeof(float) * NH,
                            M, cudaMemcpyDeviceToDevice, s));
  XL_CUDA(cudaMemcpy2DAsync(h->gate_part + NH, sizeof(float) * 2 * NH, fgate, sizeof(float) * NH,
                            sizeof(float) * NH, M, cudaMemcpyDeviceToDevice, s));
  xl::StateStepParams sp;
  memset(&sp, 0, sizeof(sp));
  xl::launch_repack_qkv(qkv, h->qkv, h->qkv + (size_t)2 * M * c.inner_dim, M, c.inner_dim, s);
  sp.C = C; sp.n = n; sp.m = m; sp.qk = h->qkv; sp.v = h->qkv + (size_t)2 * M * c.inner_dim;
  sp.gate_part = h->gate_part;
  sp.outnorm_w = outnorm_w; sp.out = h_norm; sp.h_raw = h_raw;
  sp.partial = h->partial;
  sp.B = B; sp.T = T; sp.NH = NH; sp.DH = h->DH; sp.inner = c.inner_dim; sp.NCH = 1;
  sp.rows_split = rows_split; sp.cols_per_cta = cols_per_cta;
  sp.ln_eps = c.ln_eps; sp.cell_eps = c.cell_eps;
  sp.impl = h->state_impl; sp.num_layers = c.num_blocks;
  sp.stages = h->state_stages; sp.ctas_per_sm = h->state_ctas_per_sm;
  sp.fuse_finalize = h->state_fuse;
  cudaEvent_t pe0 = nullptr, pe1 = nullptr;
  if (h->profiling) {
    XL_CUDA(cudaEventCreate(&pe0));
    XL_CUDA(cudaEventCreate(&pe1));
    XL_CUDA(cudaEventRecord(pe0, s));
  }
  XL_CUDA(xl::launch_state_step(sp, h->num_sms, s));
  if (h->profiling) {
    XL_CUDA(cudaEventRecord(pe1, s));
    h->prof_state.push_back(pe0);
    h->prof_state.push_back(pe1);
  }
  if (!xl::state_step_fuses_finalize(sp, h->num_sms)) XL_CUDA(xl::launch_state_finalize(sp, h->num_sms, s));
  h->launches += 3;
  return XL_OK;
}

int xl_policy_step(xl_handle* h, void* state, const float* states, const float* rtg, const float* rewards,
                   int32_t* tokens, float* actions, float* logits, float* hidden, int B, int mode,
                   unsigned flags, void* stream) {
  int rc = check_batch(h, B);
  if (rc) return rc;
  if (!state || !states || !rtg || !tokens || !actions) return fail(XL_ERR_INVALID_ARG, "null argument");
  if (mode != XL_MODE_FUSED && mode != XL_MODE_PER_TOKEN) return fail(XL_ERR_INVALID_ARG, "unknown mode %d", mode);
  cudaStream_t s = (cudaStream_t)stream;
  StepArgs args;
  args.state = state; args.states = states; args.rtg = rtg; args.rewards = rewards; args.tokens = tokens;
  args.actions = actions; args.logits = logits; args.hidden = hidden; args.B = B; args.mode = mode; args.flags = flags;
  if (!(flags & XL_FLAG_GRAPH) || h->profiling) {
    rc = xl_weights_ready(h);
    if (rc) return rc;
    args.flags &= ~(unsigned)XL_FLAG_GRAPH;
    cudaEvent_t pe0 = nullptr, pe1 = nullptr;
    if (h->profiling) {
      XL_CUDA(cudaEventCreate(&pe0));
      XL_CUDA(cudaEventCreate(&pe1));
      XL_CUDA(cudaEventRecord(pe0, s));
    }
    rc = run_policy(h, args, s);
    if (h->profiling) {
      cudaEventRecord(pe1, s);
      h->prof_step.push_back(pe0);
      h->prof_step.push_back(pe1);
    }
    return rc;
  }
  for (auto& g : h->graphs) {
    if (g.state == state && g.states == states && g.rtg == rtg && g.rewards == rewards &&
        g.tokens == tokens && g.actions == actions && g.logits == logits && g.hidden == hidden && g.B == B &&
        g.mode == mode && g.flags == flags) {
      XL_CUDA(cudaGraphLaunch(g.exec, s));
      h->launches += g.launches;
      return XL_OK;
    }
  }
  rc = xl_weights_ready(h);
  if (rc) return rc;
  GraphCacheEntry g;
  g.state = state; g.states = states; g.rtg = rtg; g.rewards = rewards; g.tokens = tokens; g.actions = actions;
  g.logits = logits; g.hidden = hidden; g.B = B; g.mode = mode; g.flags = flags;
  cudaGraph_t graph = nullptr;
  const int64_t before = h->launches;
  XL_CUDA(cudaStreamBeginCapture(h->cap_stream, cudaStreamCaptureModeThreadLocal));
  rc = run_policy(h, args, h->cap_stream);
  cudaError_t e = cudaStreamEndCapture(h->cap_stream, &graph);
  g.launches = h->launches - before;
  h->launches = before;
  if (rc) {
    if (graph) cudaGraphDestroy(graph);
    return rc;
  }
  if (e != cudaSuccess) return fail(XL_ERR_CUDA, "cudaStreamEndCapture: %s", cudaGetErrorString(e));
  e = cudaGraphInstantiate(&g.exec, graph, 0);
  cudaGraphDestroy(graph);
  if (e != cudaSuccess) return fail(XL_ERR_CUDA, "cudaGraphInstantiate: %s", cudaGetErrorString(e));
  if (h->graphs.size() >= 8) {
    cudaGraphExecDestroy(h->graphs.front().exec);
    h->graphs.erase(h->graphs.begin());
  }
  h->graphs.push_back(g);
  XL_CUDA(cudaGraphLaunch(g.exec, s));
  h->launches += g.launches;
  return XL_OK;
}

int xl_policy_step_host(xl_handle* h, void* state, const float* h_states, const float* h_rtg,
                        const float* h_rewards, int32_t* h_tokens, float* h_actions, int B, int mode,
                        unsigned flags, void* stream) {
  int rc = check_batch(h, B);
  if (rc) return rc;
  if (!state || !h_states || !h_rtg || !h_tokens || !h_actions) return fail(XL_ERR_INVALID_ARG, "null argument");
  if (flags & XL_FLAG_STATE_EMBEDS)
    return fail(XL_ERR_UNSUPPORTED, "xl_policy_step_host takes raw states; state embeddings are device tensors "
                                    "(use xl_policy_step with XL_FLAG_STATE_EMBEDS)");
  cudaStream_t s = (cudaStream_t)stream;
  const xl_config& c = h->cfg;
  if (h->host_zero_copy) {
    auto alias = [&](const void* p) -> void* {
      for (auto& kv : h->host_map)
        if (kv.first == p) return kv.second;
      cudaPointerAttributes at;
      void* d = nullptr;
      if (cudaPointerGetAttributes(&at, p) == cudaSuccess && at.type == cudaMemoryTypeHost) d = at.devicePointer;
      cudaGetLastError();
      if (h->host_map.size() >= 64) h->host_map.erase(h->host_map.begin());
      h->host_map.emplace_back(p, d);
      return d;
    };
    void* ds = alias(h_states);
    void* dr = alias(h_rtg);
    void* dw = h_rewards ? alias(h_rewards) : nullptr;
    void* dt = alias(h_tokens);
    void* da = alias(h_actions);
    if (ds && dr && dt && da && (!h_rewards || dw)) {
      rc = xl_policy_step(h, state, (const float*)ds, (const float*)dr, (const float*)dw, (int32_t*)dt, (float*)da,
                          nullptr, nullptr, B, mode, flags, s);
      if (rc) return rc;
      XL_CUDA(cudaStreamSynchronize(s));
      return XL_OK;
    }
  }
  XL_CUDA(cudaMemcpyAsync(h->d_states, h_states, sizeof(float) * (size_t)B * c.state_dim, cudaMemcpyHostToDevice, s));
  XL_CUDA(cudaMemcpyAsync(h->d_rtg, h_rtg, sizeof(float) * (size_t)B, cudaMemcpyHostToDevice, s));
  if (h_rewards) XL_CUDA(cudaMemcpyAsync(h->d_rew, h_rewards, sizeof(float) * (size_t)B, cudaMemcpyHostToDevice, s));
  rc = xl_policy_step(h, state, h->d_states, h->d_rtg, h_rewards ? h->d_rew : nullptr, h->d_tokens, h->d_actions,
                      nullptr, nullptr, B, mode, flags, s);
  if (rc) return rc;
  XL_CUDA(cudaMemcpyAsync(h_tokens, h->d_tokens, sizeof(int32_t) * (size_t)B * c.act_dim, cudaMemcpyDeviceToHost, s));
  XL_CUDA(cudaMemcpyAsync(h_actions, h->d_actions, sizeof(float) * (size_t)B * c.act_dim, cudaMemcpyDeviceToHost, s));
  XL_CUDA(cudaStreamSynchronize(s));
  return XL_OK;
}

static void seq_embed_chunk(xl_handle* h, const float* embeds, const float* rtg, const float* rewards,
                            const int32_t* perm, const int32_t* len, int Bk, int Tn, int Tc, int pos, cudaStream_t s) {
  const xl_config& c = h->cfg;
  auto PW = [&](int id) { return (const float*)h->pw[id - XL_W_POST_NORM]; };
  xl::SeqEmbedParams p;
  p.s_emb = embeds; p.rtg = rtg; p.rew = rewards;
  p.perm = perm; p.len = len; p.len_div = c.tokens_per_step;
  p.Tn = Tn; p.Tc = Tc; p.pos = pos; p.rows = Bk * Tc; p.d = c.embedding_dim;
  p.w_ret = PW(XL_W_EMBED_RETURN_W); p.b_ret = PW(XL_W_EMBED_RETURN_B);
  p.w_rew = PW(XL_W_EMBED_REWARD_W); p.b_rew = PW(XL_W_EMBED_REWARD_B);
  p.ln_w = PW(XL_W_EMBED_LN_W); p.ln_b = PW(XL_W_EMBED_LN_B); p.eps = c.embed_ln_eps;
  p.x = prefill_ws(h).x;
  xl::launch_seq_embed_tokens(p, s);
  h->launches += 1;
}

struct SeqCall {
  enum Input { kTokens, kStates, kEmbeds };
  const char* fn;
  Input in;
  void* state;
  const float *x, *rtg, *rewards;
  const int32_t* lengths;
  int B, S;
  unsigned flags;
  void* stream;
  bool ragged = false;
  float* y_out = nullptr;
  bool head = false;
  const xl_seq_outputs* out = nullptr;
  SeqCall(const char* fn, Input in, void* state, const float* x, const float* rtg, const float* rewards,
          const int32_t* lengths, int B, int S, unsigned flags, void* stream)
      : fn(fn), in(in), state(state), x(x), rtg(rtg), rewards(rewards), lengths(lengths), B(B), S(S), flags(flags),
        stream(stream) {}
};

static int run_seq(xl_handle* h, SeqCall c) {
  const bool enc = c.in == SeqCall::kTokens;
  if (c.head) {
    if (!h) return fail(XL_ERR_INVALID_ARG, "null handle");
    if (!c.out) return fail(XL_ERR_INVALID_ARG, "null outputs");
    if (c.out->logprobs && !c.out->targets) return fail(XL_ERR_INVALID_ARG, "logprobs need targets");
  }
  if (c.in == SeqCall::kStates && (c.flags & XL_FLAG_STATE_EMBEDS))
    return fail(XL_ERR_UNSUPPORTED, "%s takes raw states; state embeddings go through xl_policy_prefill_embeds / "
                                    "xl_policy_forward_embeds", c.fn);
  if (c.in == SeqCall::kEmbeds) {
    if (!h) return fail(XL_ERR_INVALID_ARG, "null handle");
    if ((uintptr_t)c.x % 16)
      return fail(XL_ERR_INVALID_ARG, "state_embeds must be 16-byte aligned (rows are loaded as float4)");
    c.flags |= XL_FLAG_STATE_EMBEDS;
  }
  int rc = check_batch(h, c.B);
  if (rc) return rc;
  if (!c.state || !c.x || (!enc && !c.rtg)) return fail(XL_ERR_INVALID_ARG, "null argument");
  const char* unit = enc ? "S" : "Tn";
  if (c.S <= 0) return fail(XL_ERR_INVALID_ARG, "%s=%d must be positive", unit, c.S);
  if ((c.lengths || c.ragged) && (rc = check_lengths(c.lengths, c.B, c.S, unit))) return rc;
  if ((rc = weights_ready(h, enc))) return rc;
  cudaStream_t s = (cudaStream_t)c.stream;
  const xl_config& cf = h->cfg;
  const int B = c.B, S = c.S, d = cf.embedding_dim, sd = cf.state_dim;
  SeqHead hd;
  const SeqHead* head = nullptr;
  if (c.head) {
    hd.out = *c.out;
    hd.discrete = (c.flags & XL_FLAG_DISCRETE) ? 1 : 0;
    hd.n_out = hd.discrete ? h->num_actions : h->head_out;
    hd.Tn = S;
    head = &hd;
  }
  const int32_t* lengths = c.lengths;
  if (lengths) {
    const int nfull = (int)std::count(lengths, lengths + B, S), nzero = (int)std::count(lengths, lengths + B, 0);
    if (nfull == B) {
      lengths = nullptr;
    } else {
      if (nzero < B && !prefill_fast_path(h))
        return fail(XL_ERR_UNSUPPORTED, "ragged prefill needs the sequence path (conv_kernel 4, a cell plan for DH=%d)",
                    h->DH);
      if (c.y_out) XL_CUDA(cudaMemsetAsync(c.y_out, 0, sizeof(float) * (size_t)B * S * d, s));
      if (head && (rc = seq_clear_outputs(h, hd, B, s))) return rc;
      if (nzero == B) return XL_OK;
    }
  }
  SeqPlan p;
  p.T = enc ? 1 : cf.tokens_per_step;
  if ((rc = seq_plan(h, c.state, lengths, B, S, p, s))) return rc;
  auto gather = [&](const SeqChunk& ch, const float* src, float* dst, int width) {
    return chunk_rows(h, p, ch, const_cast<float*>(src), dst, S, width, 0, s);
  };
  const Ws ws = prefill_ws(h);
  const int impl = (c.flags & XL_FLAG_SIMPLE_GEMM) ? 1 : h->gemm_impl;
  auto PW = [&](int id) { return (const float*)h->pw[id - XL_W_POST_NORM]; };
  for (const SeqChunk& ch : p.chunks) {
    const int rows = ch.Bk * ch.n;
    if (c.in == SeqCall::kTokens) {
      if ((rc = gather(ch, c.x, ws.x, d))) return rc;
    } else if (c.in == SeqCall::kEmbeds) {
      seq_embed_chunk(h, c.x, c.rtg, c.rewards, p.d_perm, p.d_len, ch.Bk, S, ch.n, ch.pos, s);
    } else {
      if ((rc = gather(ch, c.x, h->pf_sin, sd)) || (rc = gather(ch, c.rtg, h->pf_rtg, 1)) ||
          (c.rewards && (rc = gather(ch, c.rewards, h->pf_rew, 1))))
        return rc;
      xl::launch_pad_rows(h->pf_sin, sd, ws.states_pad, h->Kpad, rows, s);
      h->launches += 1;
      rc = linear(h, ws, ws.states_pad, PW(XL_W_EMBED_STATE_W), PW(XL_W_EMBED_STATE_B), nullptr,
                  ws.s_emb, rows, d, h->Kpad, impl, s);
      if (rc) return rc;
      xl::launch_embed_tokens(ws.s_emb, h->pf_rtg, c.rewards ? h->pf_rew : nullptr, PW(XL_W_EMBED_RETURN_W),
                              PW(XL_W_EMBED_RETURN_B), PW(XL_W_EMBED_REWARD_W), PW(XL_W_EMBED_REWARD_B),
                              PW(XL_W_EMBED_LN_W), PW(XL_W_EMBED_LN_B), cf.embed_ln_eps, ws.x, rows, d, nullptr, nullptr,
                              nullptr, 0.f, nullptr, nullptr, nullptr, s);
      h->launches += 1;
    }
    if ((rc = prefill_blocks(h, p.st, p.Btot, ch.Bk, ch.n * p.T, c.flags, s, p.d_len, ch.pos * p.T))) return rc;
    if (c.y_out) {
      xl::launch_ln_rows(h->pf_x, d, h->pf_xn, d, PW(XL_W_POST_NORM), nullptr, 1, cf.ln_eps, rows, d, nullptr, nullptr,
                         s);
      h->launches += 1;
      if ((rc = chunk_rows(h, p, ch, c.y_out, h->pf_xn, S, d, 1, s))) return rc;
    }
    if (head && (rc = seq_head_chunk(h, hd, ch.Bk, ch.n, ch.pos, p.d_perm, p.d_len, c.flags, s))) return rc;
    XL_CUDA(cudaGetLastError());
  }
  if ((rc = ragged_end(h, c.state, B, p, s))) return rc;
  if (enc) {
    const Slice sl = make_slice(h, B, 0, B, s);
    for (int pos = p.tail; pos < S;) {
      const SeqChunk ch = {pos, B, std::min(4, S - pos)};
      if ((rc = gather(ch, c.x, sl.ws.x, d))) return rc;
      if ((rc = run_encoder(h, c.state, sl, sl.ws.x, sl.ws.hid, ch.n, XL_MODE_FUSED, c.flags))) return rc;
      if (c.y_out && (rc = chunk_rows(h, p, ch, c.y_out, sl.ws.hid, S, d, 1, s))) return rc;
      pos += ch.n;
    }
    return XL_OK;
  }
  if (head && p.tail < S && (rc = ensure_seq_logits(h, (size_t)B * hd.n_out))) return rc;
  const bool embeds = c.in == SeqCall::kEmbeds;
  float* stage = embeds ? h->d_embeds : h->d_states;
  for (int pos = p.tail; pos < S; ++pos) {
    const SeqChunk ch = {pos, B, 1};
    if ((rc = gather(ch, c.x, stage, embeds ? d : sd)) || (rc = gather(ch, c.rtg, h->d_rtg, 1)) ||
        (c.rewards && (rc = gather(ch, c.rewards, h->d_rew, 1))))
      return rc;
    StepArgs a;
    a.state = c.state; a.states = stage; a.rtg = h->d_rtg; a.rewards = c.rewards ? h->d_rew : nullptr;
    a.tokens = h->d_tokens; a.actions = h->d_actions; a.logits = head ? h->sq_logits : nullptr; a.hidden = nullptr;
    a.B = B; a.mode = XL_MODE_FUSED; a.flags = (c.flags & ~(unsigned)XL_FLAG_GRAPH) | kFlagNoRing;
    if ((rc = run_policy(h, a, s))) return rc;
    if (head) seq_head_reduce(h, hd, B, 1, pos, nullptr, nullptr, s);
  }
  return XL_OK;
}

int xl_prefill(xl_handle* h, void* state, const float* x_in, float* y_out, int B, int S, unsigned flags, void* stream) {
  SeqCall c("xl_prefill", SeqCall::kTokens, state, x_in, nullptr, nullptr, nullptr, B, S, flags, stream);
  c.y_out = y_out;
  return run_seq(h, c);
}

int xl_prefill_ragged(xl_handle* h, void* state, const float* x_in, float* y_out, const int32_t* lengths, int B, int S,
                      unsigned flags, void* stream) {
  SeqCall c("xl_prefill_ragged", SeqCall::kTokens, state, x_in, nullptr, nullptr, lengths, B, S, flags, stream);
  c.ragged = true;
  c.y_out = y_out;
  return run_seq(h, c);
}

int xl_policy_prefill(xl_handle* h, void* state, const float* states, const float* rtg, const float* rewards, int B,
                      int Tn, unsigned flags, void* stream) {
  return run_seq(h, SeqCall("xl_policy_prefill", SeqCall::kStates, state, states, rtg, rewards, nullptr, B, Tn, flags,
                            stream));
}

int xl_policy_prefill_ragged(xl_handle* h, void* state, const float* states, const float* rtg, const float* rewards,
                             const int32_t* lengths, int B, int Tn, unsigned flags, void* stream) {
  SeqCall c("xl_policy_prefill_ragged", SeqCall::kStates, state, states, rtg, rewards, lengths, B, Tn, flags, stream);
  c.ragged = true;
  return run_seq(h, c);
}

int xl_policy_forward(xl_handle* h, void* state, const float* states, const float* rtg, const float* rewards,
                      const int32_t* lengths, int B, int Tn, const xl_seq_outputs* out, unsigned flags, void* stream) {
  SeqCall c("xl_policy_forward", SeqCall::kStates, state, states, rtg, rewards, lengths, B, Tn, flags, stream);
  c.head = true;
  c.out = out;
  return run_seq(h, c);
}

int xl_policy_prefill_embeds(xl_handle* h, void* state, const float* state_embeds, const float* rtg,
                             const float* rewards, const int32_t* lengths, int B, int Tn, unsigned flags,
                             void* stream) {
  return run_seq(h, SeqCall("xl_policy_prefill_embeds", SeqCall::kEmbeds, state, state_embeds, rtg, rewards, lengths, B,
                            Tn, flags, stream));
}

int xl_policy_forward_embeds(xl_handle* h, void* state, const float* state_embeds, const float* rtg,
                             const float* rewards, const int32_t* lengths, int B, int Tn, const xl_seq_outputs* out,
                             unsigned flags, void* stream) {
  SeqCall c("xl_policy_forward_embeds", SeqCall::kEmbeds, state, state_embeds, rtg, rewards, lengths, B, Tn, flags,
            stream);
  c.head = true;
  c.out = out;
  return run_seq(h, c);
}

int xl_linear(xl_handle* h, const float* A, const void* W_bf16, const float* bias, const float* residual,
              float* out, int M, int N, int K, int impl, void* stream) {
  if (!h || !A || !W_bf16 || !out) return fail(XL_ERR_INVALID_ARG, "null argument");
  if (M <= 0 || N <= 0 || K <= 0) return fail(XL_ERR_INVALID_ARG, "bad GEMM shape");
  Ws w = ws_slice(h, 0, h->cfg.max_batch);
  w.a_cap = h->a_cap;
  return linear(h, w, A, W_bf16, bias, residual, out, M, N, K, impl, (cudaStream_t)stream);
}

int xl_set_token_ring(xl_handle* h, int32_t* ring, int slots, int next_slot, void* stream) {
  if (!h) return fail(XL_ERR_INVALID_ARG, "null handle");
  if (ring && (slots <= 0 || next_slot < 0 || next_slot >= slots))
    return fail(XL_ERR_INVALID_ARG, "token ring: slots=%d next_slot=%d", slots, next_slot);
  if (ring != h->tok_ring || (ring && slots != h->tok_slots)) {
    for (auto& g : h->graphs)
      if (g.exec) cudaGraphExecDestroy(g.exec);
    h->graphs.clear();
    h->tok_ring = ring;
    h->tok_slots = ring ? slots : 0;
  }
  if (ring) {
    xl::launch_set_u32(h->counters + kCntRing, (unsigned)next_slot, (cudaStream_t)stream);
    XL_CUDA(cudaGetLastError());
  }
  return XL_OK;
}

static int check_sampling(const xl_handle* h, const xl_sampling* p) {
  if (!(p->temperature > 0.f) || !std::isfinite(p->temperature))
    return fail(XL_ERR_INVALID_ARG, "sampling: temperature %g must be finite and > 0", (double)p->temperature);
  if (!(p->top_p >= 0.f && p->top_p <= 1.f)) return fail(XL_ERR_INVALID_ARG, "sampling: top_p %g outside [0, 1]", (double)p->top_p);
// ... 210 lines not shown
```

lram_b200/csrc/xl_internal.h:

```cpp
#pragma once
#include <cuda_bf16.h>
#include <cuda_runtime.h>
#include <stdint.h>

namespace xl {

extern int g_use_pdl;

void launch_ln_rows(const float* in, int64_t in_stride, float* out, int64_t out_stride, const float* w,
                    const float* bias, int residual_weight, float eps, int rows, int d, void* a_hi,
                    void* a_lo, cudaStream_t s);
void launch_ln_rows_reduce(float* x, const float* part, int splits, int64_t part_stride, float* out,
                           int64_t out_stride, const float* w, float eps, int rows, int d, void* a_hi, void* a_lo,
                           cudaStream_t s);

void launch_embed_tokens(const float* s_emb, const float* rtg, const float* rew, const float* w_ret,
                         const float* b_ret, const float* w_rew, const float* b_rew, const float* ln_w,
                         const float* ln_b, float eps, float* x, int B, int d, unsigned* step_counter,
                         unsigned* sample_counter, const float* ln0_w, float ln0_eps, float* xn0, void* a_hi,
                         void* a_lo, cudaStream_t s);
void launch_pad_split(const float* in, int K, void* hi, void* lo, int Kpad, int rows, cudaStream_t s);
void launch_ln_rows_gather(const float* x, const float* part, int splits, int64_t part_stride, const float* w,
                           float eps, int rows, int d, int row_mul, int row_off, void* a_hi, void* a_lo,
                           cudaStream_t s);

void launch_pad_rows(const float* in, int K, float* out, int Kpad, int rows, cudaStream_t s);
void launch_copy_rows(const float* in, int64_t in_stride, float* out, int64_t out_stride, int rows, int d,
                      cudaStream_t s);

struct ConvQkvParams {
  const float* u;
  int u_splits;
  int64_t u_stride;
  float* conv_state;
  const float* conv_w;
  const float* conv_b;
  const float* wq;
  const float* wk;
  const float* wv;
  const float* wi;
  const float* wf;
  float* qk;
  float* v;
  float* act;
  float* gate_part;
  int B, T, inner, NH, KS, NCH;
  int impl;
};
bool launch_conv_qkv_gates(const ConvQkvParams& p, cudaStream_t s);

void launch_argmax_tokens(const float* logits, int64_t row_pitch, int B, int act_dim, int num_actions,
                          int discrete_actions, int discrete, float bin_width, float min_val,
                          int32_t* tokens, float* actions, int32_t* ring, const unsigned* step_counter,
                          int ring_slots, int64_t ring_slot_stride, cudaStream_t s);
void launch_set_u32(unsigned* p, unsigned v, cudaStream_t s);

constexpr int kSampleMaxActions = 512;
constexpr int kSampleMaxRows = 8;
void launch_sample_tokens(const float* logits, int64_t row_pitch, int B, int act_dim, int num_actions,
                          int discrete_actions, int discrete, float bin_width, float min_val, int32_t* tokens,
                          float* actions, int32_t* ring, const unsigned* ring_counter, int ring_slots,
                          int64_t ring_slot_stride, const void* prm, const unsigned* step_counter, int env_offset,
                          cudaStream_t s);
void launch_set_sampling(void* dst, const void* params, unsigned* counter, unsigned counter_value, cudaStream_t s);

void launch_state_reset(float* C, float* n, float* m, float* conv, const uint8_t* mask, int B,
                        int64_t c_per_env, int64_t n_per_env, int64_t m_per_env, int64_t conv_per_env,
                        cudaStream_t s);

struct StateCopyGeom {
  uint64_t slstm_mask;
  int num_blocks;
  int B[2];
  size_t layer_bytes[2], slayer_bytes[2];
  size_t c_off[2], n_off[2], m_off[2], conv_off[2], s_off[2], sconv_off[2];
  size_t c_env, n_env, m_env, conv_env, s_env, sconv_env;
};
void launch_state_permute(void* caller, void* compact, const int32_t* perm, int Bc, const StateCopyGeom& g,
                          int to_caller, cudaStream_t s);
void launch_ragged_rows(float* caller, float* compact, const int32_t* perm, const int32_t* len, int len_div, int Bk,
                        int S, int Sc, int pos, int width, int to_caller, cudaStream_t s);

struct SeqHeadParams {
  const float* logits;
  int rows, Tc, pos, Tn;
  int n_out, act_dim, num_actions, discrete_actions, discrete;
  float bin_width, min_val;
  const int32_t* perm;
  const int32_t* len;
  int len_div;
  int32_t* tokens;
  float* actions;
  float* out_logits;
  const int32_t* targets;
  float* logprobs;
};
void launch_seq_head(const SeqHeadParams& p, cudaStream_t s);

struct SeqEmbedParams {
  const float* s_emb;
  const float* rtg;
  const float* rew;
  const int32_t* perm;
  const int32_t* len;
  int len_div, Tn, Tc, pos;
  int rows, d;
  const float *w_ret, *b_ret, *w_rew, *b_rew, *ln_w, *ln_b;
  float eps;
  float* x;
};
void launch_seq_embed_tokens(const SeqEmbedParams& p, cudaStream_t s);

void launch_l2_prefetch(const void* base, size_t bytes, int num_sms, int evict_last, cudaStream_t s);

struct StateStepParams {
  float* C;
  float* n;
  float* m;
  const float* qk;
  const float* v;
  const float* gate_part;
  const float* igate_b;
  const float* fgate_b;
  const float* outnorm_w;
  const float* skip;
  const float* act;
  const float* u;
  int u_splits;
  int64_t u_stride;
  float* out;
  void* out_hi;
  void* out_lo;
  float* h_raw;
  float* partial;
  int B, T, NH, DH, inner, NCH;
  int rows_split;
  int cols_per_cta;
  int impl;
  int stages;
  int ctas_per_sm;
  int meta_slots;
  int sk_grid, sk_q, sk_r, sk_smax;
  int num_layers;
  int max_cluster;
  int fuse_finalize;
  float ln_eps, cell_eps;
};
cudaError_t launch_state_step(StateStepParams p, int num_sms, cudaStream_t s);
bool state_step_fuses_finalize(StateStepParams p, int num_sms);
cudaError_t launch_state_finalize(StateStepParams p, int num_sms, cudaStream_t s);
void state_step_auto_tiling(int B, int NH, int DH, int num_sms, int* rows_split, int* cols_per_cta);
void launch_repack_qkv(const float* qkv, float* qk, float* v, int M, int inner, cudaStream_t s);

bool launch_slstm_conv(const float* xn, float* conv_state, const float* cw, const float* cb, float* xc, int B,
                       int T, int d, int KS, cudaStream_t s, const int32_t* len = nullptr, int pos = 0);
void launch_slstm_gates(const float* xc, const float* xn, const float* w_i, const float* w_f, const float* w_z,
                        const float* w_o, const float* bias, float* pre, int M, int d, int NH, cudaStream_t s);
cudaError_t launch_slstm_cell(const float* pre, const float* R, float* st, float* y_out, int B, int stB, int T, int t,
                              int d, int NH, cudaStream_t s, const int32_t* len = nullptr, int pos = 0);
void launch_slstm_out(const float* y_out, const float* gn_w, float* x, float* st_y, int M, int T, int d, int NH,
                      float eps, cudaStream_t s);
void launch_ffn_gate(const float* up, float* out, void* hi, void* lo, int M, int ff, cudaStream_t s);

bool prefill_cell_supported(int DH);
bool launch_conv_qkv_gates_seq(const ConvQkvParams& p, int S, cudaStream_t s, const int32_t* len = nullptr,
                               int pos = 0);
size_t gate_scan_seq_scratch_floats(int B, int S, int NH);
void launch_gate_scan_seq(const float* gate_part, const float* igate_b, const float* fgate_b, float* m_state,
                          float* fseq, float* iseq, float* mseq, float* scratch, int B, int S, int NH, int NCH,
                          cudaStream_t s, const int32_t* len = nullptr, int pos = 0);
cudaError_t launch_cell_seq(float* C, float* n, const float* q, const float* k, const float* v, const float* fseq,
                            const float* iseq, float* num, float* qn, int B, int S, int NH, int DH, int inner,
                            cudaStream_t s);
bool prefill_cell_mma_supported(int DH);
int prefill_cell_mma_chunk();
void prefill_cell_mma_ws(int rows, int NH, int DH, size_t* common_bytes, size_t* vblk_bytes);
cudaError_t launch_cell_mma(float* C, float* n, const float* q, const float* k, const float* v, const float* fseq,
                            const float* iseq, float* num, float* qn, void* common, void* vblk, int B, int S, int NH,
                            int DH, int inner, cudaStream_t s);
extern int g_gemm_2cta;
extern int g_prefill_tc_fused;
extern int g_prefill_conv_run;
extern int g_prefill_conv_impl;
extern int g_prefill_conv_persist;
extern int g_prefill_prep;
bool prefill_cell_tc_supported(int DH);
int prefill_cell_tc_chunk();
size_t prefill_cell_tc_ws_bytes(int B, int S, int NH, int DH);
extern int g_prefill_tc_overlap;
extern int g_prefill_scan_split;
struct CellSideStream {
  cudaStream_t stream;
  cudaEvent_t fork, join;
};
cudaError_t launch_cell_tc(float* C, float* n, const float* q, const float* k, const float* v, const float* fseq,
                           const float* iseq, float* num, float* qn, void* ws, int B, int S, int NH, int DH, int inner,
                           cudaStream_t s, const CellSideStream* side = nullptr);
cudaError_t launch_finalize_seq(const float* num, const float* qn, const float* mseq, const float* outnorm_w,
                                const float* skip, const float* act, const float* u, float* out, void* out_hi,
                                void* out_lo, int B, int S, int NH, int DH, int inner, float ln_eps, float cell_eps,
                                cudaStream_t s);

struct SmallPreParams {
  const float* x;
  const float* norm_w;
  const __nv_bfloat16* w_up;
  const float *conv_w, *conv_b, *wq, *wk, *wv, *wi, *wf;
  float* conv_state;
  float* u;
  float* qk;
  float* v;
  float* act;
  float* gate_part;
  int B, T, d, inner, NH, NCH;
  float ln_eps;
};
int smallm_pre_chunks(int B, int T, int d, int inner, int NH, int KS);
cudaError_t launch_smallm_pre(const SmallPreParams& p, cudaStream_t s);
struct SmallDownParams {
  const float* g;
  const __nv_bfloat16* w_down;
  float* x;
  int M, d, inner;
};
cudaError_t launch_smallm_down(const SmallDownParams& p, cudaStream_t s);

void launch_gemm_simple(const float* A, const __nv_bfloat16* W, const float* bias, const float* residual,
                        float* out, int M, int N, int K, cudaStream_t s);

struct UpEpiParams {
  float* conv_state;
  const float *conv_w, *conv_b, *wq, *wk, *wv, *wi, *wf;
  float *qk, *v, *act, *gate_part;
  int B, T, inner, NCH;
};
bool gemm_up_conv_supported(int T, int KS, int NH, int inner, int d);
int gemm_up_conv_chunks(int inner);
cudaError_t launch_gemm_up_conv(const void* a_hi, const void* a_lo, const __nv_bfloat16* W, float* u, int M, int d,
                                const UpEpiParams& ep, cudaStream_t s);

bool gemm_tc_supported(int M, int N, int K);
extern int g_gemm_cluster;
extern int g_gemm_bm;
void gemm_tc_set_m64_layout(int contiguous);
void launch_split_bf16(const float* in, int64_t in_stride, void* hi, void* lo, int rows, int K, cudaStream_t s);
cudaError_t launch_gemm_tc(const void* a_hi, const void* a_lo, const __nv_bfloat16* W, const float* bias,
                           const float* residual, float* out, int M, int N, int K, int num_sms, int bn, int splits,
                           long long split_stride, int low_smem, cudaStream_t s);
void gemm_tc_plan(int M, int N, int K, int num_sms, int max_splits, int* bn_out, int* splits_out);

}
```

lram_b200/csrc/xl_state_step.cu:

```cuda
#include <cuda.h>
#include <cuda_bf16.h>

#include "xl_common.cuh"
#include "xl_internal.h"

namespace xl {

constexpr int kThreads = 256;
constexpr int kUnroll = 8;
constexpr int kMaxNCH = 128;

__host__ __device__ __forceinline__ int sk_start(const StateStepParams& p, int c) {
  return c * p.sk_q + (c < p.sk_r ? c : p.sk_r);
}
__host__ __device__ __forceinline__ int sk_cta_of(const StateStepParams& p, int tile) {
  const int big = p.sk_r * (p.sk_q + 1);
  return tile < big ? tile / (p.sk_q + 1) : p.sk_r + (tile - big) / p.sk_q;
}

template <int T>
__device__ __forceinline__ float gate_preact(const StateStepParams& p, int b, int hd, int lane) {
  const int NH = p.NH;
  const int pair = lane >> 2, sub = lane & 3;
  const int t = pair >> 1, is_f = pair & 1;
// ... 314 lines not shown
    float M2 = 0.f;
    for (int k = 0; k < CS; ++k) {
      const float dk = s_x[k * 8 + t] * (1.f / W) - mu;
      M2 += s_x[k * 8 + T + t] + (float)W * dk * dk;
    }
    mean[t] = mu;
    rstd[t] = rsqrtf(M2 / (float)DH + p.ln_eps);
  }
  if (col) {
#pragma unroll
    for (int t = 0; t < T; ++t) {
      const int64_t row = (int64_t)tc.b * T + t;
      float o = (num[t] - mean[t]) * rstd[t] * (1.f + wn);
      if (p.h_raw) p.h_raw[row * inner + ch] = num[t];
      if (p.skip) o = (o + wskip * act[t]) * silu_fast(zz[t]);
      if (p.out) p.out[row * inner + ch] = o;
      if (p.out_hi) {
        const __nv_bfloat16 hi = __float2bfloat16_rn(o);
        reinterpret_cast<__nv_bfloat16*>(p.out_hi)[row * inner + ch] = hi;
        reinterpret_cast<__nv_bfloat16*>(p.out_lo)[row * inner + ch] = __float2bfloat16_rn(o - __bfloat162float(hi));
      }
    }
  }
  if (tc.cs == 0) {
#pragma unroll
    for (int j = 0; j < kNRowsMax; ++j) {
      const int r = tid + j * kThreads;
      if (r < DH) p.n[(int64_t)tc.bh * DH + r] = nreg[j];
    }
    if (tid == 0) p.m[tc.bh] = s_m[T];
  }
}

template <int T>
__device__ __forceinline__ void leader_sum(float (&v)[kNRowsMax][T], float (&out)[T], float* red ,
                                           int warp, int lane, int nw) {
#pragma unroll
  for (int j = 0; j < kNRowsMax; ++j)
#pragma unroll
    for (int t = 0; t < T; ++t) v[j][t] = warp_sum(v[j][t]);
  asm volatile("bar.sync 1, %0;" ::"n"(kThreads) : "memory");
  if (lane == 0) {
#pragma unroll
    for (int j = 0; j < kNRowsMax; ++j)
      if (warp + 8 * j < nw) {
#pragma unroll
        for (int t = 0; t < T; ++t) red[t * 32 + warp + 8 * j] = v[j][t];
      }
  }
  asm volatile("bar.sync 1, %0;" ::"n"(kThreads) : "memory");
#pragma unroll
  for (int t = 0; t < T; ++t) out[t] = warp_sum(lane < nw ? red[t * 32 + lane] : 0.f);
}

template <int T>
__device__ __forceinline__ void leader_finalize(const StateStepParams& p, const TileCoord& tc, const float* sacc,
                                                const float* sqk, const float* sqkh, const float* sn, float* snum,
                                                int tstride, const float* s_f, const float* s_i, const float* s_m,
                                                float* s_red, uint32_t xbar, int tid) {
  constexpr int W = 128;
  const int DH = p.DH, inner = p.inner, CS = DH / W, RS = p.rows_split;
  const int warp = tid >> 5, lane = tid & 31;
  const int tile = tc.rs * CS + tc.cs;
  if (tid < W) {
    const uint32_t rbase = mapa_u32(smem_u32(snum + (tile * T) * W + tid), 0u);
    const uint32_t rbar = mapa_u32(xbar, 0u);
#pragma unroll
    for (int t = 0; t < T; ++t) {
      float s = 0.f;
      for (int y = 0; y < 8; ++y) s += sacc[(y * T + t) * W + tid];
      st_async_f32(rbase + (uint32_t)(t * W * sizeof(float)), s, rbar);
    }
  }
  if (tile != 0) return;
  const float* qkh = RS > 1 ? sqkh : sqk;
  const int hstride = RS > 1 ? 2 * DH : tstride;
  const int nw = (DH + 31) >> 5;
  const float kscale = rsqrtf((float)DH);
  float nreg[kNRowsMax], v[kNRowsMax][T], qn[T];
#pragma unroll
  for (int j = 0; j < kNRowsMax; ++j) {
    const int r = tid + j * kThreads;
    float nv = r < DH ? sn[r] : 0.f;
#pragma unroll
    for (int t = 0; t < T; ++t) {
      const float2 q2 = r < DH ? *reinterpret_cast<const float2*>(qkh + t * hstride + 2 * r) : make_float2(0.f, 0.f);
      nv = fmaf(s_f[t], nv, s_i[t] * kscale * q2.y);
      v[j][t] = q2.x * nv;
    }
    nreg[j] = nv;
  }
  leader_sum<T>(v, qn, s_red, warp, lane, nw);
  float den[T];
#pragma unroll
  for (int t = 0; t < T; ++t) den[t] = fmaxf(fabsf(qn[t]), expf(-s_m[t + 1])) + p.cell_eps;
  mbar_wait(xbar, 0);
  float hh[kNRowsMax][T], mean[T], var[T];
#pragma unroll
  for (int j = 0; j < kNRowsMax; ++j) {
    const int c = tid + j * kThreads;
#pragma unroll
    for (int t = 0; t < T; ++t) {
      float s = 0.f;
      if (c < DH)
        for (int r = 0; r < RS; ++r) s += snum[((r * CS + (c >> 7)) * T + t) * W + (c & 127)];
      hh[j][t] = s / den[t];
      v[j][t] = hh[j][t];
    }
  }
  leader_sum<T>(v, mean, s_red, warp, lane, nw);
#pragma unroll
  for (int t = 0; t < T; ++t) mean[t] /= (float)DH;
#pragma unroll
  for (int j = 0; j < kNRowsMax; ++j) {
    const int c = tid + j * kThreads;
#pragma unroll
    for (int t = 0; t < T; ++t) {
      const float dlt = c < DH ? hh[j][t] - mean[t] : 0.f;
      v[j][t] = dlt * dlt;
    }
  }
  leader_sum<T>(v, var, s_red, warp, lane, nw);
#pragma unroll
  for (int j = 0; j < kNRowsMax; ++j) {
    const int c = tid + j * kThreads;
    if (c < DH) {
      const int ch = tc.hd * DH + c;
      const float wn = p.outnorm_w[ch];
      const float wskip = p.skip ? p.skip[ch] : 0.f;
#pragma unroll
      for (int t = 0; t < T; ++t) {
        const int64_t row = (int64_t)tc.b * T + t;
        const float rstd = rsqrtf(var[t] / (float)DH + p.ln_eps);
        float o = (hh[j][t] - mean[t]) * rstd * (1.f + wn);
        if (p.h_raw) p.h_raw[row * inner + ch] = hh[j][t];
        if (p.skip) {
          float z = p.u[row * 2 * inner + inner + ch];
          for (int zz = 1; zz < p.u_splits; ++zz) z += p.u[zz * p.u_stride + row * 2 * inner + inner + ch];
          o = (o + wskip * p.act[row * inner + ch]) * silu_fast(z);
        }
        if (p.out) p.out[row * inner + ch] = o;
        if (p.out_hi) {
          const __nv_bfloat16 hi = __float2bfloat16_rn(o);
          reinterpret_cast<__nv_bfloat16*>(p.out_hi)[row * inner + ch] = hi;
          reinterpret_cast<__nv_bfloat16*>(p.out_lo)[row * inner + ch] = __float2bfloat16_rn(o - __bfloat162float(hi));
        }
      }
      p.n[(int64_t)tc.bh * DH + c] = nreg[j];
    }
  }
  if (tid == 0) p.m[tc.bh] = s_m[T];
}

template <int T, bool kStream, bool kFused>
__global__ void __launch_bounds__(kBlock, 3)
mlstm_state_stream_tma_kernel(const __grid_constant__ CUtensorMap mapC, StateStepParams p) {
  extern __shared__ uint8_t smem_raw[];
  __shared__ float s_f[T], s_i[T], s_m[T + 1], s_pre[2 * T];
  __shared__ __align__(8) uint64_t s_bar[2 * kStages + 2];
  __shared__ float s_red[4 * 32], s_x[kMaxCluster * 8];

  const TileCoord tc = tile_coord(p);
  const int DH = p.DH;
  const int W = p.cols_per_cta;
  const bool leader = kFused && p.fuse_finalize == 2 && tc.rs == 0 && tc.cs == 0;
  const bool head_qk = leader && p.rows_split > 1;
  const int TX = W >> 2, TY = kThreads / TX;
  const int tid = threadIdx.x, warp = tid >> 5, lane = tid & 31;
  const int tstride = 2 * tc.rows_per;
  const int nblk = (tc.nrows + kStageRows - 1) / kStageRows;
  const uint32_t stage_bytes = (uint32_t)(kStageRows * W * sizeof(float));

  const uint32_t sbase = (smem_u32(smem_raw) + 127u) & ~127u;
  float* stage0 = reinterpret_cast<float*>(smem_raw + (sbase - smem_u32(smem_raw)));
  float* sqk = stage0 + (size_t)kStages * kStageRows * W;
  float* sn = sqk + (size_t)T * tstride;
  float* snum = sn + DH;
  float* sqkh = snum + (size_t)p.rows_split * T * DH;
  float* sacc = stage0;
  const uint32_t bar0 = smem_u32(s_bar);
  auto full_bar = [&](int s) { return bar0 + 8u * s; };
  auto empty_bar = [&](int s) { return bar0 + 8u * (kStages + s); };
  const uint32_t qk_bar = bar0 + 8u * (2 * kStages);
  const uint32_t xbar = bar0 + 8u * (2 * kStages + 1);

  if (tid == 0) {
    for (int s = 0; s < kStages; ++s) {
      mbar_init(full_bar(s), 1);
      mbar_init(empty_bar(s), kConsumerWarps);
    }
    mbar_init(qk_bar, 1);
    if (kFused) {
      mbar_init(xbar, 1);
      if (p.fuse_finalize == 2) {
        if (leader) mbar_expect_tx(xbar, (uint32_t)(p.rows_split * DH * T * sizeof(float)));
      } else {
        mbar_expect_tx(xbar, (uint32_t)((DH / 128) * 2 * T * sizeof(float)));
      }
    }
    asm volatile("fence.mbarrier_init.release.cluster;" ::: "memory");
  }
  __syncthreads();
  if (kFused) cluster_arrive();

  if (warp == kConsumerWarps) {
    if (lane == 0) {
      asm volatile("prefetch.tensormap [%0];" ::"l"(&mapC) : "memory");
      uint64_t policy = 0;
      if (kStream) asm volatile("createpolicy.fractional.L2::evict_first.b64 %0, 1.0;" : "=l"(policy));
      const int grow0 = tc.slab_row0;
      auto issue = [&](int i) {
        const int s = i % kStages;
        mbar_wait(empty_bar(s), ((i / kStages) & 1) ^ 1);
        mbar_expect_tx(full_bar(s), stage_bytes);
        const uint32_t dst = sbase + s * stage_bytes;
        if (kStream) {
          asm volatile(
              "cp.async.bulk.tensor.2d.shared::cluster.global.mbarrier::complete_tx::bytes.L2::cache_hint "
              "[%0], [%1, {%3, %4}], [%2], %5;"
              ::"r"(dst), "l"(&mapC), "r"(full_bar(s)), "r"(tc.cin), "r"(grow0 + i * kStageRows), "l"(policy)
              : "memory");
        } else {
          asm volatile(
              "cp.async.bulk.tensor.2d.shared::cluster.global.mbarrier::complete_tx::bytes [%0], [%1, {%3, %4}], [%2];"
              ::"r"(dst), "l"(&mapC), "r"(full_bar(s)), "r"(tc.cin), "r"(grow0 + i * kStageRows)
              : "memory");
        }
      };
      const int pre = nblk < kStages ? nblk : kStages;
      for (int i = 0; i < pre; ++i) issue(i);
      pdl_wait();
      pdl_trigger();
      if (kFused) cluster_wait();
      mbar_expect_tx(qk_bar, (uint32_t)(T * tc.nrows * 8 + (kFused ? DH * 4 : 0) + (head_qk ? T * DH * 8 : 0)));
      if (kFused) bulk_copy_g2s(smem_u32(sn), p.n + (int64_t)tc.bh * DH, (uint32_t)(DH * 4), qk_bar);
      if (head_qk) {
#pragma unroll
        for (int t = 0; t < T; ++t)
          bulk_copy_g2s(smem_u32(sqkh + t * 2 * DH), p.qk + ((((int64_t)tc.b * T + t) * p.NH + tc.hd) * DH) * 2,
                        (uint32_t)(DH * 8), qk_bar);
      }
#pragma unroll
      for (int t = 0; t < T; ++t)
        bulk_copy_g2s(smem_u32(sqk + t * tstride),
                      p.qk + ((((int64_t)tc.b * T + t) * p.NH + tc.hd) * DH + tc.r0) * 2,
                      (uint32_t)(tc.nrows * 8), qk_bar);
      for (int i = pre; i < nblk; ++i) issue(i);
    } else {
      pdl_wait();
      pdl_trigger();
      if (kFused) cluster_wait();
    }
    return;
  }

  const int tx = tid % TX, ty = tid / TX;
  pdl_wait();
  pdl_trigger();
  if (kFused) cluster_wait();
  if (warp == 0) compute_gates<T>(p, tc.b, tc.hd, tc.bh, s_f, s_i, s_m, s_pre);
  float vi[T][4];
#pragma unroll
  for (int t = 0; t < T; ++t) {
    const float4 vv = *reinterpret_cast<const float4*>(p.v + ((int64_t)tc.b * T + t) * p.inner + tc.hd * DH +
                                                       tc.c0 + 4 * tx);
    vi[t][0] = vv.x; vi[t][1] = vv.y; vi[t][2] = vv.z; vi[t][3] = vv.w;
  }
  asm volatile("bar.sync 1, %0;" ::"n"(kThreads) : "memory");
  const float kscale = rsqrtf((float)DH);
  float f[T];
#pragma unroll
  for (int t = 0; t < T; ++t) {
    f[t] = s_f[t];
    const float it = s_i[t] * kscale;
#pragma unroll
    for (int j = 0; j < 4; ++j) vi[t][j] *= it;
  }
  float acc[T][4];
#pragma unroll
  for (int t = 0; t < T; ++t) acc[t][0] = acc[t][1] = acc[t][2] = acc[t][3] = 0.f;

  float4* Cp = reinterpret_cast<float4*>(p.C + (int64_t)tc.slab_row0 * tc.wc + tc.cin) + tx;
  const int64_t rs4 = tc.wc >> 2;
  constexpr int kRowsPerThread = 4;
  const bool fast = (TY * kRowsPerThread == kStageRows);
  mbar_wait(qk_bar, 0);
  for (int i = 0; i < nblk; ++i) {
    const int s = i % kStages;
    const float* st = stage0 + (size_t)s * kStageRows * W;
    const int rblk = i * kStageRows;
    const int rcur = min(kStageRows, tc.nrows - rblk);
    mbar_wait(full_bar(s), (i / kStages) & 1);
    if (fast && rcur == kStageRows) {
      float4 cv[kRowsPerThread];
#pragma unroll
      for (int j = 0; j < kRowsPerThread; ++j)
        cv[j] = *reinterpret_cast<const float4*>(st + (ty + j * 8) * W + 4 * tx);
      __syncwarp();
      if (lane == 0) mbar_arrive(empty_bar(s));
      float4* rp = Cp + (int64_t)(rblk + ty) * rs4;
#pragma unroll
      for (int j = 0; j < kRowsPerThread; ++j) {
        float c[4] = {cv[j].x, cv[j].y, cv[j].z, cv[j].w};
        row_update<T>(c, sqk + 2 * (rblk + ty + j * 8), tstride, f, vi, acc);
        const float4 o = make_float4(c[0], c[1], c[2], c[3]);
        if (kStream) st_stream(rp + (int64_t)j * 8 * rs4, o);
        else rp[(int64_t)j * 8 * rs4] = o;
      }
    } else {
      for (int r = ty; r < rcur; r += TY) {
        const float4 cv = *reinterpret_cast<const float4*>(st + r * W + 4 * tx);
        float c[4] = {cv.x, cv.y, cv.z, cv.w};
        row_update<T>(c, sqk + 2 * (rblk + r), tstride, f, vi, acc);
        Cp[(int64_t)(rblk + r) * rs4] = make_float4(c[0], c[1], c[2], c[3]);
      }
      __syncwarp();
      if (lane == 0) mbar_arrive(empty_bar(s));
    }
  }
  asm volatile("bar.sync 1, %0;" ::"n"(kThreads) : "memory");
  if (kFused) {
#pragma unroll
    for (int t = 0; t < T; ++t)
      *reinterpret_cast<float4*>(sacc + ((ty * T + t) * TX + tx) * 4) =
          make_float4(acc[t][0], acc[t][1], acc[t][2], acc[t][3]);
    asm volatile("bar.sync 1, %0;" ::"n"(kThreads) : "memory");
    if (p.fuse_finalize == 2)
      leader_finalize<T>(p, tc, sacc, sqk, sqkh, sn, snum, tstride, s_f, s_i, s_m, s_red, xbar, tid);
    else
      fused_finalize<T>(p, tc, sacc, sqk, sn, tstride, s_f, s_i, s_m, s_red, s_x, xbar, tid);
    return;
  }
  write_partials<T>(p, tc, sacc, acc, tx, ty, TX, TY, tid);
}

typedef CUresult (*EncodeTiledFn)(CUtensorMap*, CUtensorMapDataType, cuuint32_t, void*, const cuuint64_t*,
                                  const cuuint64_t*, const cuuint32_t*, const cuuint32_t*, CUtensorMapInterleave,
                                  CUtensorMapSwizzle, CUtensorMapL2promotion, CUtensorMapFloatOOBfill);
static EncodeTiledFn get_encode() {
  static const EncodeTiledFn fn = [] {
    void* p = nullptr;
    cudaDriverEntryPointQueryResult q;
    if (cudaGetDriverEntryPoint("cuTensorMapEncodeTiled", &p, cudaEnableDefault, &q) == cudaSuccess &&
        q == cudaDriverEntryPointSuccess)
      return (EncodeTiledFn)p;
    return (EncodeTiledFn) nullptr;
  }();
  return fn;
}

template <int T, bool kStream, bool kFused>
static cudaError_t launch(const StateStepParams& p, cudaStream_t s) {
  EncodeTiledFn enc = get_encode();
  if (!enc) return cudaErrorUnknown;
  CUtensorMap map;
  const int wc = slab_width(p.DH);
  cuuint64_t gdim[2] = {(cuuint64_t)wc, (cuuint64_t)p.B * p.NH * (p.DH / wc) * p.DH};
  cuuint64_t gstride[1] = {(cuuint64_t)wc * sizeof(float)};
  cuuint32_t box[2] = {(cuuint32_t)p.cols_per_cta, (cuuint32_t)kStageRows};
  cuuint32_t estr[2] = {1, 1};
  if (enc(&map, CU_TENSOR_MAP_DATA_TYPE_FLOAT32, 2, p.C, gdim, gstride, box, estr, CU_TENSOR_MAP_INTERLEAVE_NONE,
          CU_TENSOR_MAP_SWIZZLE_NONE, CU_TENSOR_MAP_L2_PROMOTION_NONE, CU_TENSOR_MAP_FLOAT_OOB_FILL_NONE) !=
      CUDA_SUCCESS)
    return cudaErrorInvalidValue;
  const int rows_per = (p.DH + p.rows_split - 1) / p.rows_split;
  const size_t ring = sizeof(float) * (size_t)kStages * kStageRows * p.cols_per_cta;
  const int TY = kThreads / (p.cols_per_cta / 4);
  const size_t red = sizeof(float) * (size_t)TY * T * p.cols_per_cta;
  const size_t smem = 128 + (ring > red ? ring : red) +
                      sizeof(float) * ((size_t)2 * T * rows_per +
                                       (kFused ? (size_t)p.DH * (1 + T * p.rows_split + (p.rows_split > 1 ? 2 * T : 0)) : 0));
  if (cudaError_t e = ensure_dyn_smem<&mlstm_state_stream_tma_kernel<T, kStream, kFused>>(smem); e != cudaSuccess)
    return e;
  const int CS = p.DH / p.cols_per_cta;
  const int64_t grid = (int64_t)p.B * p.NH * CS * p.rows_split;
  if (!kFused && p.fuse_finalize != 3)
    return launch_k(mlstm_state_stream_tma_kernel<T, kStream, false>, dim3((unsigned)grid), dim3(kBlock), smem, s, map,
                    p);
  const int csize = CS * p.rows_split;
  if (csize > 8) {
    static std::atomic<bool> allowed[kMaxDevices];
    int dev = 0;
    if (cudaError_t e = cudaGetDevice(&dev); e != cudaSuccess) return e;
    const bool tracked = dev >= 0 && dev < kMaxDevices;
    if (!tracked || !allowed[dev].load(std::memory_order_acquire)) {
      if (cudaError_t e = cudaFuncSetAttribute(mlstm_state_stream_tma_kernel<T, kStream, kFused>,
                                               cudaFuncAttributeNonPortableClusterSizeAllowed, 1);
          e != cudaSuccess)
        return e;
      if (tracked) allowed[dev].store(true, std::memory_order_release);
    }
  }
  cudaLaunchConfig_t cfg = {};
  cfg.gridDim = dim3((unsigned)grid);
  cfg.blockDim = dim3(kBlock);
  cfg.dynamicSmemBytes = smem;
  cfg.stream = s;
  cudaLaunchAttribute attr[2];
  attr[0].id = cudaLaunchAttributeClusterDimension;
  attr[0].val.clusterDim.x = (unsigned)csize;
  attr[0].val.clusterDim.y = 1;
  attr[0].val.clusterDim.z = 1;
  attr[1].id = cudaLaunchAttributeProgrammaticStreamSerialization;
  attr[1].val.programmaticStreamSerializationAllowed = 1;
  cfg.attrs = attr;
  cfg.numAttrs = g_use_pdl ? 2 : 1;
  return cudaLaunchKernelEx(&cfg, mlstm_state_stream_tma_kernel<T, kStream, kFused>, map, p);
}

}

namespace pers {

using tma::bulk_copy_g2s;
using tma::mbar_arrive;
using tma::mbar_expect_tx;
using tma::mbar_init;
using tma::mbar_wait;
using tma::smem_u32;

constexpr int kStageRows = 32;
constexpr int kW = 128;
constexpr int kMaxStages = 8;
constexpr int kMaxMetaSlots = 4;
constexpr int kConsumerWarps = kThreads / 32;
constexpr int kBlock = kThreads + 64;
constexpr int kStageFloats = kStageRows * kW;

__device__ __forceinline__ void mbar_expect_tx_only(uint32_t bar, uint32_t bytes) {
  asm volatile("mbarrier.expect_tx.relaxed.cta.shared::cta.b64 [%0], %1;" ::"r"(bar), "r"(bytes) : "memory");
}

__host__ __device__ inline int meta_floats(int T, int DH) { return T * DH * 2 + T * kW + 16; }

template <int T, bool kStream>
__global__ void __launch_bounds__(kBlock, 2)
mlstm_state_stream_persistent_kernel(const __grid_constant__ CUtensorMap mapC, StateStepParams p, int stages,
                                     int meta_slots) {
  extern __shared__ uint8_t smem_raw[];
  __shared__ __align__(8) uint64_t s_bar[2 * kMaxStages + 2 * kMaxMetaSlots];

  const int DH = p.DH, CS = DH / kW, NH = p.NH;
  const int nblk = DH / kStageRows;
  const int mfl = meta_floats(T, DH);
  const int tid = threadIdx.x, warp = tid >> 5, lane = tid & 31;
  const int cta = blockIdx.x;
  const int tile_begin = sk_start(p, cta), tile_end = sk_start(p, cta + 1);

  const uint32_t sbase = (smem_u32(smem_raw) + 127u) & ~127u;
  float* ring = reinterpret_cast<float*>(smem_raw + (sbase - smem_u32(smem_raw)));
  float* meta = ring + (size_t)stages * kStageFloats;
  float* red = meta + (size_t)meta_slots * mfl;
  const uint32_t bar0 = smem_u32(s_bar);
  auto full_bar = [&](int s) { return bar0 + 8u * s; };
  auto empty_bar = [&](int s) { return bar0 + 8u * (kMaxStages + s); };
  auto meta_full = [&](int s) { return bar0 + 8u * (2 * kMaxStages + s); };
  auto meta_empty = [&](int s) { return bar0 + 8u * (2 * kMaxStages + kMaxMetaSlots + s); };

  if (tid == 0) {
    for (int s = 0; s < stages; ++s) {
      mbar_init(full_bar(s), 1);
      mbar_init(empty_bar(s), kConsumerWarps);
    }
    for (int s = 0; s < meta_slots; ++s) {
      mbar_init(meta_full(s), 1);
      mbar_init(meta_empty(s), kConsumerWarps);
    }
    asm volatile("fence.mbarrier_init.release.cluster;" ::: "memory");
  }
  __syncthreads();

  if (warp == kConsumerWarps) {
    if (lane == 0) {
      asm volatile("prefetch.tensormap [%0];" ::"l"(&mapC) : "memory");
      uint64_t policy = 0;
      if (kStream) asm volatile("createpolicy.fractional.L2::evict_first.b64 %0, 1.0;" : "=l"(policy));
      int s = 0;
      uint32_t ph = 0;
      int item = tile_begin / nblk;
      int i = tile_begin - item * nblk;
      bool waited = false;
      for (int tile = tile_begin; tile < tile_end; ++tile) {
        if (!waited && tile - tile_begin == stages) {
          pdl_wait();
          pdl_trigger();
          waited = true;
        }
        mbar_wait(empty_bar(s), ph ^ 1);
        mbar_expect_tx(full_bar(s), (uint32_t)(kStageFloats * sizeof(float)));
        const uint32_t dst = sbase + (uint32_t)(s * kStageFloats * sizeof(float));
        const int c0 = 0, r0 = tile * kStageRows;
        if (kStream) {
          asm volatile(
              "cp.async.bulk.tensor.2d.shared::cluster.global.mbarrier::complete_tx::bytes.L2::cache_hint "
              "[%0], [%1, {%3, %4}], [%2], %5;"
              ::"r"(dst), "l"(&mapC), "r"(full_bar(s)), "r"(c0), "r"(r0), "l"(policy)
              : "memory");
        } else {
          asm volatile(
              "cp.async.bulk.tensor.2d.shared::cluster.global.mbarrier::complete_tx::bytes [%0], [%1, {%3, %4}], [%2];"
              ::"r"(dst), "l"(&mapC), "r"(full_bar(s)), "r"(c0), "r"(r0)
              : "memory");
        }
        if (++s == stages) { s = 0; ph ^= 1; }
        if (++i == nblk) { i = 0; ++item; }
      }
      if (!waited) {
        pdl_wait();
        pdl_trigger();
      }
    } else {
      pdl_wait();
      pdl_trigger();
    }
    return;
  }

  if (warp == kConsumerWarps + 1) {
    pdl_wait();
    pdl_trigger();
    int slot = 0;
    uint32_t ph = 0;
    for (int tile = tile_begin; tile < tile_end;) {
      const int item = tile / nblk, i0 = tile - item * nblk;
      const int cnt = min(nblk - i0, tile_end - tile);
      const int bh = item / CS, cs = item - bh * CS;
      const int b = bh / NH, hd = bh - b * NH;
      const int r0 = i0 * kStageRows, rows = cnt * kStageRows;
      float* ms = meta + (size_t)slot * mfl;
      float* s_gate = ms + T * DH * 2 + T * kW;
      const float pre = gate_preact<T>(p, b, hd, lane);
      float mprev = p.m[bh];
      if (lane == 0) {
        mbar_wait(meta_empty(slot), ph ^ 1);
        mbar_expect_tx_only(meta_full(slot), (uint32_t)(T * rows * 8 + T * kW * 4));
#pragma unroll
        for (int t = 0; t < T; ++t) {
          bulk_copy_g2s(smem_u32(ms + t * DH * 2),
                        p.qk + ((((int64_t)b * T + t) * NH + hd) * DH + r0) * 2, (uint32_t)(rows * 8),
                        meta_full(slot));
          bulk_copy_g2s(smem_u32(ms + T * DH * 2 + t * kW),
                        p.v + ((int64_t)b * T + t) * p.inner + hd * DH + cs * kW, (uint32_t)(kW * 4),
                        meta_full(slot));
        }
      }
      float fv[T], iv[T];
#pragma unroll
      for (int t = 0; t < T; ++t) {
        const float ig = __shfl_sync(0xffffffffu, pre, 8 * t);
        const float fg = __shfl_sync(0xffffffffu, pre, 8 * t + 4);
        const float lf = log_sigmoid(fg);
        const float mnew = fmaxf(lf + mprev, ig);
        fv[t] = expf(lf + mprev - mnew);
        iv[t] = expf(ig - mnew);
        mprev = mnew;
      }
      if (lane == 0) {
#pragma unroll
        for (int t = 0; t < T; ++t) {
          s_gate[t] = fv[t];
          s_gate[4 + t] = iv[t];
        }
        mbar_arrive(meta_full(slot));
      }
      __syncwarp();
      if (++slot == meta_slots) { slot = 0; ph ^= 1; }
      tile += cnt;
    }
    return;
  }

  const int tx = lane, ty = warp;
  const float kscale = rsqrtf((float)DH);
  const int64_t rs4 = kW >> 2;
  const int tstride = 2 * DH;
  pdl_wait();
  pdl_trigger();
  int s = 0, slot = 0, seg = 0;
  uint32_t ph = 0, mph = 0;
  for (int tile = tile_begin; tile < tile_end; ++seg) {
    const int item = tile / nblk, i0 = tile - item * nblk;
    const int cnt = min(nblk - i0, tile_end - tile);
    const int bh = item / CS, cs = item - bh * CS;
    const float* ms = meta + (size_t)slot * mfl;
    const float* sqk = ms;
    const float* sv = ms + T * DH * 2;
    const float* s_gate = sv + T * kW;
    mbar_wait(meta_full(slot), mph);
    float f[T], vi[T][4], acc[T][4];
#pragma unroll
    for (int t = 0; t < T; ++t) {
      f[t] = s_gate[t];
      const float it_ = s_gate[4 + t] * kscale;
      const float4 vv = *reinterpret_cast<const float4*>(sv + t * kW + 4 * tx);
      vi[t][0] = vv.x * it_; vi[t][1] = vv.y * it_; vi[t][2] = vv.z * it_; vi[t][3] = vv.w * it_;
      acc[t][0] = acc[t][1] = acc[t][2] = acc[t][3] = 0.f;
    }
    float4* Cp = reinterpret_cast<float4*>(p.C + (int64_t)tile * kStageFloats) + tx;
    for (int i = 0; i < cnt; ++i) {
      const float* st = ring + (size_t)s * kStageFloats;
      const int rblk = i * kStageRows;
      mbar_wait(full_bar(s), ph);
      float4 cv[4];
#pragma unroll
      for (int r = 0; r < 4; ++r) cv[r] = *reinterpret_cast<const float4*>(st + (ty + r * 8) * kW + 4 * tx);
      __syncwarp();
      if (lane == 0) mbar_arrive(empty_bar(s));
      if (++s == stages) { s = 0; ph ^= 1; }
      float4* rp = Cp + (int64_t)(rblk + ty) * rs4;
#pragma unroll
      for (int r = 0; r < 4; ++r) {
        float c[4] = {cv[r].x, cv[r].y, cv[r].z, cv[r].w};
        row_update<T>(c, sqk + 2 * (rblk + ty + r * 8), tstride, f, vi, acc);
        const float4 o = make_float4(c[0], c[1], c[2], c[3]);
        if (kStream) st_stream(rp + (int64_t)r * 8 * rs4, o);
        else rp[(int64_t)r * 8 * rs4] = o;
      }
    }
    float* rb = red + (seg & 1) * (kConsumerWarps * T * kW);
#pragma unroll
    for (int t = 0; t < T; ++t)
      *reinterpret_cast<float4*>(rb + (ty * T + t) * kW + 4 * tx) =
          make_float4(acc[t][0], acc[t][1], acc[t][2], acc[t][3]);
    __syncwarp();
    if (lane == 0) mbar_arrive(meta_empty(slot));
    if (++slot == meta_slots) { slot = 0; mph ^= 1; }
    asm volatile("bar.sync 1, %0;" ::"n"(kThreads) : "memory");
    const int pslot = cta - sk_cta_of(p, item * nblk);
    float* dst = p.partial + (((int64_t)item * p.sk_smax + pslot) * T) * kW;
    for (int idx = tid; idx < T * kW; idx += kThreads) {
      float sum = 0.f;
      const int t = idx / kW, c = idx - t * kW;
#pragma unroll
      for (int y = 0; y < kConsumerWarps; ++y) sum += rb[(y * T + t) * kW + c];
      dst[idx] = sum;
    }
    tile += cnt;
  }
}

static size_t smem_bytes(int T, int DH, int stages, int meta_slots) {
  return 128 + sizeof(float) * ((size_t)stages * kStageFloats + (size_t)meta_slots * meta_floats(T, DH) +
                                2 * (size_t)kConsumerWarps * T * kW);
}

template <int T, bool kStream>
static cudaError_t launch(const StateStepParams& p, cudaStream_t s) {
  tma::EncodeTiledFn enc = tma::get_encode();
  if (!enc) return cudaErrorUnknown;
  CUtensorMap map;
  cuuint64_t gdim[2] = {(cuuint64_t)kW, (cuuint64_t)p.B * p.NH * p.DH * (p.DH / kW)};
  cuuint64_t gstride[1] = {(cuuint64_t)kW * sizeof(float)};
  cuuint32_t box[2] = {(cuuint32_t)kW, (cuuint32_t)kStageRows};
  cuuint32_t estr[2] = {1, 1};
  if (enc(&map, CU_TENSOR_MAP_DATA_TYPE_FLOAT32, 2, p.C, gdim, gstride, box, estr, CU_TENSOR_MAP_INTERLEAVE_NONE,
          CU_TENSOR_MAP_SWIZZLE_NONE, CU_TENSOR_MAP_L2_PROMOTION_NONE, CU_TENSOR_MAP_FLOAT_OOB_FILL_NONE) !=
      CUDA_SUCCESS)
    return cudaErrorInvalidValue;
  int stages = p.stages > 0 ? p.stages : 6;
  if (stages > kMaxStages) stages = kMaxStages;
  if (stages < 2) stages = 2;
  const int meta_slots = p.meta_slots >= 2 && p.meta_slots <= kMaxMetaSlots ? p.meta_slots : 3;
  const size_t smem = smem_bytes(T, p.DH, stages, meta_slots);
  if (cudaError_t e = ensure_dyn_smem<&mlstm_state_stream_persistent_kernel<T, kStream>>(smem); e != cudaSuccess)
    return e;
  return launch_k(mlstm_state_stream_persistent_kernel<T, kStream>, dim3((unsigned)p.sk_grid), dim3(kBlock), smem,
                  s, map, p, stages, meta_slots);
}

}

template <int N>
__device__ __forceinline__ void block_sum_n(float (&v)[N], float* red ) {
  const int lane = threadIdx.x & 31, wid = threadIdx.x >> 5;
  const int nw = (blockDim.x + 31) >> 5;
#pragma unroll
  for (int k = 0; k < N; ++k) v[k] = warp_sum(v[k]);
  __syncthreads();
  if (lane == 0) {
#pragma unroll
    for (int k = 0; k < N; ++k) red[k * 32 + wid] = v[k];
  }
  __syncthreads();
#pragma unroll
  for (int k = 0; k < N; ++k) {
    float r = (lane < nw) ? red[k * 32 + lane] : 0.f;
    v[k] = warp_sum(r);
  }
}

template <int T>
__global__ void __launch_bounds__(1024) mlstm_state_finalize_kernel(StateStepParams p) {
  __shared__ float s_f[T], s_i[T], s_m[T + 1], s_pre[2 * T];
  __shared__ float s_red[T * 32];
  const int bh = blockIdx.x;
  const int b = bh / p.NH, hd = bh - b * p.NH;
  const int DH = p.DH, inner = p.inner, RS = p.rows_split;
  const int a = threadIdx.x;
  const bool ok = a < DH;
  const int ch = hd * DH + (ok ? a : 0);

  float nreg = ok ? p.n[(int64_t)bh * DH + a] : 0.f;
  const float wn = ok ? p.outnorm_w[ch] : 0.f;
  const float wskip = (ok && p.skip) ? p.skip[ch] : 0.f;
  float2 qk[T];
  float num[T], act[T], zz[T];
  int sk_item = 0, sk_nseg = 0;
  if (p.sk_grid > 0 && ok) {
    const int nblk = DH >> 5;
    sk_item = bh * (DH >> 7) + (a >> 7);
    sk_nseg = sk_cta_of(p, (sk_item + 1) * nblk - 1) - sk_cta_of(p, sk_item * nblk) + 1;
  }
#pragma unroll
  for (int t = 0; t < T; ++t) {
    const int64_t row = (int64_t)b * T + t;
    qk[t] = ok ? reinterpret_cast<const float2*>(p.qk)[(row * p.NH + hd) * DH + a] : make_float2(0.f, 0.f);
    act[t] = (ok && p.skip) ? p.act[row * inner + ch] : 0.f;
    zz[t] = (ok && p.skip) ? p.u[row * 2 * inner + inner + ch] : 0.f;
    if (ok && p.skip)
      for (int z = 1; z < p.u_splits; ++z) zz[t] += p.u[z * p.u_stride + row * 2 * inner + inner + ch];
  }
  if (threadIdx.x < 32) compute_gates<T>(p, b, hd, bh, s_f, s_i, s_m, s_pre);
  __syncthreads();
  const float kscale = rsqrtf((float)DH);
  float qn[T], den[T];
#pragma unroll
  for (int t = 0; t < T; ++t) {
    nreg = fmaf(s_f[t], nreg, s_i[t] * kscale * qk[t].y);
    qn[t] = qk[t].x * nreg;
  }
  block_sum_n<T>(qn, s_red);
#pragma unroll
  for (int t = 0; t < T; ++t) den[t] = fmaxf(fabsf(qn[t]), expf(-s_m[t + 1])) + p.cell_eps;
  pdl_wait();
  pdl_trigger();
#pragma unroll
  for (int t = 0; t < T; ++t) {
    float s = 0.f;
    if (ok) {
      if (p.sk_grid > 0) {
        const float* pp = p.partial + ((int64_t)sk_item * p.sk_smax * T + t) * 128 + (a & 127);
        for (int r = 0; r < sk_nseg; ++r) s += pp[(int64_t)r * T * 128];
      } else {
        const float* pp = p.partial + ((int64_t)bh * RS * T + t) * DH + a;
        if (RS == 1) {
          s += pp[0];
        } else {
          float pr[8];
#pragma unroll
          for (int r = 0; r < 8; ++r) pr[r] = pp[(int64_t)(r < RS ? r : 0) * T * DH];
#pragma unroll
          for (int r = 0; r < 8; ++r)
            if (r < RS) s += pr[r];
          for (int r = 8; r < RS; ++r) s += pp[(int64_t)r * T * DH];
        }
      }
    }
    num[t] = s;
  }
  if (ok) p.n[(int64_t)bh * DH + a] = nreg;
  float mean[T], var[T];
#pragma unroll
  for (int t = 0; t < T; ++t) {
    num[t] = num[t] / den[t];
    mean[t] = num[t];
  }
  block_sum_n<T>(mean, s_red);
#pragma unroll
  for (int t = 0; t < T; ++t) {
    mean[t] /= (float)DH;
    const float dlt = ok ? num[t] - mean[t] : 0.f;
    var[t] = dlt * dlt;
  }
  block_sum_n<T>(var, s_red);
  if (ok) {
#pragma unroll
    for (int t = 0; t < T; ++t) {
      const float rstd = rsqrtf(var[t] / (float)DH + p.ln_eps);
      const int64_t row = (int64_t)b * T + t;
      float o = (num[t] - mean[t]) * rstd * (1.f + wn);
      if (p.h_raw) p.h_raw[row * inner + ch] = num[t];
      if (p.skip) o = (o + wskip * act[t]) * silu_fast(zz[t]);
      if (p.out) p.out[row * inner + ch] = o;
      if (p.out_hi) {
        const __nv_bfloat16 hi = __float2bfloat16_rn(o);
        reinterpret_cast<__nv_bfloat16*>(p.out_hi)[row * inner + ch] = hi;
        reinterpret_cast<__nv_bfloat16*>(p.out_lo)[row * inner + ch] = __float2bfloat16_rn(o - __bfloat162float(hi));
      }
    }
  }
  if (threadIdx.x == 0) p.m[bh] = s_m[T];
}

void state_step_auto_tiling(int B, int NH, int DH, int num_sms, int* rows_split, int* cols_per_cta) {
  int cols = 128;
  while (cols > 4 && (DH % cols) != 0) cols >>= 1;
  if (cols > DH) cols = DH;
  const int CS = DH / cols;
  const int64_t target = (int64_t)num_sms * 3;
  int rs = 1;
  while ((int64_t)B * NH * CS * rs < target && (DH % (rs * 2 * 32)) == 0 && rs < 32) rs *= 2;
  *rows_split = rs;
  *cols_per_cta = cols;
}

static bool persistent_ok(const StateStepParams& p) {
  return p.impl == 2 && p.DH % pers::kW == 0 && p.DH >= pers::kW && p.rows_split <= 0 &&
         (p.cols_per_cta <= 0 || p.cols_per_cta == pers::kW);
}

template <int T>
static cudaError_t launch_T(const StateStepParams& p, cudaStream_t s) {
  const size_t c_bytes = sizeof(float) * (size_t)p.B * p.NH * p.DH * p.DH;
  const bool stream = c_bytes * (size_t)(p.num_layers > 0 ? p.num_layers : 1) > ((size_t)64 << 20);
  if (p.sk_grid > 0) return stream ? pers::launch<T, true>(p, s) : pers::launch<T, false>(p, s);
  const int rows_per = (p.DH + p.rows_split - 1) / p.rows_split;
  cudaError_t e;
  if (p.impl >= 1 && rows_per % 4 == 0) {
    if (p.fuse_finalize == 1 || p.fuse_finalize == 2)
      e = stream ? tma::launch<T, true, true>(p, s) : tma::launch<T, false, true>(p, s);
    else
      e = stream ? tma::launch<T, true, false>(p, s) : tma::launch<T, false, false>(p, s);
  } else {
    const int TX = p.cols_per_cta / 4, TY = kThreads / TX;
    const size_t smem = sizeof(float) * ((size_t)2 * T * rows_per + (size_t)TY * T * p.cols_per_cta);
    e = ensure_dyn_smem<&mlstm_state_stream_ldg_kernel<T>>(smem);
    if (e != cudaSuccess) return e;
    const int CS = p.DH / p.cols_per_cta;
    const int64_t grid = (int64_t)p.B * p.NH * CS * p.rows_split;
    e = launch_k(mlstm_state_stream_ldg_kernel<T>, dim3((unsigned)grid), dim3(kThreads), smem, s, p);
  }
  return e;
}

static void resolve_tiling(StateStepParams& p, int num_sms) {
  p.sk_grid = 0;
  if (persistent_ok(p)) {
    const int64_t N = (int64_t)p.B * p.NH * (p.DH / pers::kW) * (p.DH / pers::kStageRows);
    const int64_t cap = (int64_t)num_sms * (p.ctas_per_sm > 0 ? p.ctas_per_sm : 1);
    const int G = (int)(N < cap ? N : cap);
    const int nblk = p.DH / pers::kStageRows;
    p.sk_grid = G;
    p.sk_q = (int)(N / G);
    p.sk_r = (int)(N % G);
    const int by_q = (nblk + p.sk_q - 1) / p.sk_q + 1;
    p.sk_smax = by_q < nblk ? by_q : nblk;
    p.cols_per_cta = pers::kW;
    p.rows_split = 1;
    return;
  }
  if (p.rows_split <= 0 || p.cols_per_cta <= 0) {
    int rs, cols;
    state_step_auto_tiling(p.B, p.NH, p.DH, num_sms, &rs, &cols);
    if (p.fuse_finalize == 2 && cols == 128) {
      const int cap = (p.max_cluster > 0 && p.max_cluster < tma::kMaxClusterOptIn) ? p.max_cluster : tma::kMaxClusterOptIn;
      while (rs > 1 && (p.DH / 128) * rs > cap) rs >>= 1;
    }
    if (p.rows_split <= 0) p.rows_split = rs;
    if (p.cols_per_cta <= 0) p.cols_per_cta = cols;
  }
}

bool state_step_fuses_finalize(StateStepParams p, int num_sms) {
  if (p.fuse_finalize != 1 && p.fuse_finalize != 2) return false;
  if (p.impl != 1) return false;
  resolve_tiling(p, num_sms);
  if (p.sk_grid != 0 || p.cols_per_cta != 128 || p.DH % 128 != 0 || p.DH > tma::kNRowsMax * kThreads || p.T > 4)
    return false;
  const int CS = p.DH / 128;
  if (p.fuse_finalize == 1) return p.rows_split == 1 && CS <= tma::kMaxCluster;
  return p.DH % (p.rows_split * 4) == 0 && CS * p.rows_split <= tma::kMaxClusterOptIn &&
         (p.rows_split == 1 ? CS <= tma::kMaxCluster : true);
}

static void drop_unfusable(StateStepParams& p, int num_sms) {
  if (!state_step_fuses_finalize(p, num_sms)) {
    StateStepParams q = p;
    q.fuse_finalize = 1;
    p.fuse_finalize = (p.fuse_finalize == 3 && state_step_fuses_finalize(q, num_sms)) ? 3 : 0;
  }
}

cudaError_t launch_state_finalize(StateStepParams p, int num_sms, cudaStream_t s) {
  drop_unfusable(p, num_sms);
  resolve_tiling(p, num_sms);
  const int thr = ((p.DH + 31) / 32) * 32;
  switch (p.T) {
    case 1: return launch_k(mlstm_state_finalize_kernel<1>, dim3(p.B * p.NH), dim3(thr), 0, s, p);
    case 2: return launch_k(mlstm_state_finalize_kernel<2>, dim3(p.B * p.NH), dim3(thr), 0, s, p);
    case 3: return launch_k(mlstm_state_finalize_kernel<3>, dim3(p.B * p.NH), dim3(thr), 0, s, p);
    case 4: return launch_k(mlstm_state_finalize_kernel<4>, dim3(p.B * p.NH), dim3(thr), 0, s, p);
    default: return cudaErrorInvalidValue;
  }
  return cudaGetLastError();
}

cudaError_t launch_state_step(StateStepParams p, int num_sms, cudaStream_t s) {
  drop_unfusable(p, num_sms);
  resolve_tiling(p, num_sms);
  if (p.cols_per_cta % 4 || p.DH % p.cols_per_cta || slab_width(p.DH) % p.cols_per_cta ||
      kThreads % (p.cols_per_cta / 4) || p.DH > 1024 || p.NCH > kMaxNCH || p.rows_split > p.DH)
    return cudaErrorInvalidValue;
  switch (p.T) {
    case 1: return launch_T<1>(p, s);
    case 2: return launch_T<2>(p, s);
    case 3: return launch_T<3>(p, s);
    case 4: return launch_T<4>(p, s);
    default: return cudaErrorInvalidValue;
  }
}

__global__ void repack_qkv_kernel(const float* __restrict__ qkv, float* __restrict__ qk, float* __restrict__ v,
                                  int M, int inner) {
  const int64_t i = (int64_t)blockIdx.x * blockDim.x + threadIdx.x;
  pdl_wait();
  pdl_trigger();
  if (i >= (int64_t)M * inner) return;
  const int64_t m = i / inner;
  const int c = (int)(i - m * inner);
  const float* row = qkv + m * 3 * inner;
  reinterpret_cast<float2*>(qk)[i] = make_float2(row[c], row[inner + c]);
  v[i] = row[2 * inner + c];
}
void launch_repack_qkv(const float* qkv, float* qk, float* v, int M, int inner, cudaStream_t s) {
  const int64_t n = (int64_t)M * inner;
  launch_k(repack_qkv_kernel, dim3((unsigned)((n + 255) / 256)), dim3(256), 0, s, qkv, qk, v, M, inner);
}

}
```

lram_b200/engine.py:

```python
from __future__ import annotations

import ctypes as C
import functools
import math
from typing import Dict, Optional

import numpy as np
import torch

from . import _lib as L
from .config import XLSTMPolicyConfig
from .synth import is_bf16_weight

_BLOCK_KEYS = {
    "xlstm_norm.weight": "XLSTM_NORM",
    "xlstm.proj_up.weight": "PROJ_UP",
    "xlstm.q_proj.weight": "Q_PROJ",
    "xlstm.k_proj.weight": "K_PROJ",
    "xlstm.v_proj.weight": "V_PROJ",
    "xlstm.conv1d.conv.weight": "CONV_W",
    "xlstm.conv1d.conv.bias": "CONV_B",
    "xlstm.mlstm_cell.igate.weight": "IGATE_W",
    "xlstm.mlstm_cell.igate.bias": "IGATE_B",
    "xlstm.mlstm_cell.fgate.weight": "FGATE_W",
    "xlstm.mlstm_cell.fgate.bias": "FGATE_B",
    "xlstm.mlstm_cell.outnorm.weight": "OUTNORM",
    "xlstm.learnable_skip": "SKIP",
    "xlstm.proj_down.weight": "PROJ_DOWN",
}
_SLSTM_BLOCK_KEYS = {
    "xlstm_norm.weight": "XLSTM_NORM",
    "xlstm.conv1d.conv.weight": "CONV_W",
    "xlstm.conv1d.conv.bias": "CONV_B",
    "xlstm.fgate.weight": "S_GATE_I",
    "xlstm.igate.weight": "S_GATE_F",
    "xlstm.zgate.weight": "S_GATE_Z",
    "xlstm.ogate.weight": "S_GATE_O",
    "xlstm.slstm_cell._recurrent_kernel_": "S_RECURRENT",
    "xlstm.slstm_cell._bias_": "S_BIAS",
    "xlstm.group_norm.weight": "S_GROUP_NORM",
    "ffn_norm.weight": "FFN_NORM",
    "ffn.proj_up.weight": "FFN_UP",
    "ffn.proj_down.weight": "FFN_DOWN",
}
_POLICY_KEYS = {
    "encoder.layers.post_blocks_norm.weight": "POST_NORM",
    "embed_state.weight": "EMBED_STATE_W",
    "embed_state.bias": "EMBED_STATE_B",
    "embed_return.weight": "EMBED_RETURN_W",
    "embed_return.bias": "EMBED_RETURN_B",
    "embed_rewards.weight": "EMBED_REWARD_W",
    "embed_rewards.bias": "EMBED_REWARD_B",
    "embed_ln.weight": "EMBED_LN_W",
    "embed_ln.bias": "EMBED_LN_B",
    "action_net.0.weight": "HEAD_W",
    "action_net.0.bias": "HEAD_B",
}


def strip_checkpoint_prefixes(sd: Dict[str, torch.Tensor]) -> Dict[str, torch.Tensor]:
    out = {}
    for k, v in sd.items():
        for pref in ("module.", "_orig_mod."):
            while k.startswith(pref):
                k = k[len(pref):]
        k = k.replace("._orig_mod.", ".").replace(".module.", ".")
        out[k] = v
    return out


def slab_width(DH: int) -> int:
    return 128 if DH % 128 == 0 else DH


def c_to_slab(c: torch.Tensor) -> torch.Tensor:
    B, NH, DH, _ = c.shape
    W = slab_width(DH)
    return c.reshape(B, NH, DH, DH // W, W).permute(0, 1, 3, 2, 4).contiguous()


def c_from_slab(p: torch.Tensor) -> torch.Tensor:
    B, NH, CS, DH, W = p.shape
    return p.permute(0, 1, 3, 2, 4).reshape(B, NH, DH, CS * W)


def _ptr(t: Optional[torch.Tensor]):
    return C.c_void_p(0 if t is None else t.data_ptr())


class StateCache:

    def __init__(self, engine: "XLSTMEngine", B: int):
        self.engine = engine
        self.B = B
        nbytes = engine.lib.xl_state_bytes(engine.handle, B)
        self.buf = torch.zeros(nbytes // 4, dtype=torch.float32, device=engine.device)

    def view(self, layer: int, part: int) -> torch.Tensor:
        off, size = C.c_size_t(), C.c_size_t()
        L.check(self.engine.lib.xl_state_layout(self.engine.handle, self.B, layer, part, C.byref(off), C.byref(size)))
        flat = self.buf[off.value // 4: (off.value + size.value) // 4]
        cfg = self.engine.cfg
        NH, DH = cfg.num_heads, cfg.head_dim
        W = slab_width(DH)
        if cfg.is_slstm(layer):
            shape = {L.XL_STATE_SLSTM: (4, self.B, cfg.d),
                     L.XL_STATE_CONV: (self.B, cfg.conv1d_kernel_size, cfg.d)}[part]
        else:
            shape = {L.XL_STATE_C: (self.B, NH, DH // W, DH, W), L.XL_STATE_N: (self.B, NH, DH),
                     L.XL_STATE_M: (self.B, NH), L.XL_STATE_CONV: (self.B, cfg.conv1d_kernel_size, cfg.inner)}[part]
        return flat.view(*shape)

    def c_logical(self, layer: int) -> torch.Tensor:
        return c_from_slab(self.view(layer, L.XL_STATE_C))

    def nbytes(self) -> int:
        return self.buf.numel() * 4

    def to_past_key_values(self) -> Dict[str, Dict[str, tuple]]:
        out = {}
        for i in range(self.engine.cfg.num_blocks):
            if self.engine.cfg.is_slstm(i):
                out[f"block_{i}"] = {"slstm_state": self.view(i, L.XL_STATE_SLSTM).clone(),
                                     "conv_state": (self.view(i, L.XL_STATE_CONV).clone(),)}
                continue
            c = self.c_logical(i)
            n = self.view(i, L.XL_STATE_N).clone().unsqueeze(-1)
            m = self.view(i, L.XL_STATE_M).clone().view(self.B, -1, 1, 1)
            conv = self.view(i, L.XL_STATE_CONV).clone()
            out[f"block_{i}"] = {"mlstm_state": (c, n, m), "conv_state": (conv,)}
        return out

    def load_past_key_values(self, pkv: Dict[str, Dict[str, tuple]]) -> None:
        for i in range(self.engine.cfg.num_blocks):
            st = pkv[f"block_{i}"]
            if self.engine.cfg.is_slstm(i):
                self.view(i, L.XL_STATE_SLSTM).copy_(st["slstm_state"].to(self.buf.device, torch.float32))
                self.view(i, L.XL_STATE_CONV).copy_(st["conv_state"][0].to(self.buf.device, torch.float32))
                continue
            c, n, m = st["mlstm_state"]
            self.view(i, L.XL_STATE_C).copy_(c_to_slab(c.to(self.buf.device, torch.float32)))
            self.view(i, L.XL_STATE_N).copy_(n.to(self.buf.device, torch.float32).reshape(self.B, -1, n.shape[2]))
            self.view(i, L.XL_STATE_M).copy_(m.to(self.buf.device, torch.float32).reshape(self.B, -1))
            self.view(i, L.XL_STATE_CONV).copy_(st["conv_state"][0].to(self.buf.device, torch.float32))


def sampling_params(cfg: XLSTMPolicyConfig, temperature: float = 1.0, top_k: int = 0, top_p: float = 0.5,
                    seed: int = 0, env_id_base: int = 0, env_id_stride: int = 1) -> L.XLSampling:
    temperature, top_p = float(temperature), float(top_p)
    if not (math.isfinite(temperature) and temperature > 0.0):
        raise ValueError(f"temperature={temperature} must be finite and > 0")
    if not 0.0 <= top_p <= 1.0:
        raise ValueError(f"top_p={top_p} outside [0, 1]")
    if not 0 <= int(top_k) <= cfg.num_actions:
        raise ValueError(f"top_k={top_k} outside [0, num_actions={cfg.num_actions}]")
    if int(env_id_base) < 0 or int(env_id_stride) < 1:
        raise ValueError(f"env_id_base={env_id_base} must be >= 0 and env_id_stride={env_id_stride} >= 1")
    if not 0 <= int(seed) < 2 ** 64:
        raise ValueError(f"seed={seed} outside [0, 2^64)")
    return L.XLSampling(temperature=temperature, top_p=top_p, top_k=int(top_k), env_id_base=int(env_id_base),
                        env_id_stride=int(env_id_stride), seed=int(seed))


def check_lengths(lengths, B: int, S: int, what: str = "S") -> np.ndarray:
    if isinstance(lengths, torch.Tensor):
        if lengths.device.type != "cpu":
            raise ValueError(f"lengths must be on the host, got a tensor on {lengths.device}")
        if lengths.dtype.is_floating_point or lengths.dtype.is_complex or lengths.dtype == torch.bool:
            raise ValueError(f"lengths must be integers, got {lengths.dtype}")
        lengths = lengths.numpy()
    arr = np.asarray(lengths)
    if arr.ndim != 1 or arr.shape[0] != B:
        raise ValueError(f"lengths must hold one value per env ({B}), got shape {arr.shape}")
    if arr.dtype == np.bool_ or not np.issubdtype(arr.dtype, np.integer):
        raise ValueError(f"lengths must be integers, got dtype {arr.dtype}")
    if (arr < 0).any() or (arr > S).any():
        raise ValueError(f"lengths must lie in [0, {what}={S}], got min {arr.min()} max {arr.max()}")
    return np.ascontiguousarray(arr, dtype=np.int32)


def _on_device(fn):
    @functools.wraps(fn)
    def wrapped(self, *args, **kwargs):
        if torch.cuda.current_device() == self.device.index:
            return fn(self, *args, **kwargs)
        with torch.cuda.device(self.device):
            return fn(self, *args, **kwargs)
    return wrapped


class XLSTMEngine:

    def __init__(self, cfg: XLSTMPolicyConfig, state_dict: Dict[str, torch.Tensor], max_batch: int,
                 device: Optional[torch.device] = None, encoder_only: bool = False):
        if not torch.cuda.is_available():
            raise RuntimeError("XLSTMEngine needs a CUDA device: the xlstm_b200 path has no CPU fallback")
        cfg.validate()
        self.cfg = cfg
        self.device = torch.device("cuda", torch.cuda.current_device()) if device is None else torch.device(device)
        if self.device.type != "cuda":
            raise RuntimeError(f"XLSTMEngine needs a CUDA device, got {self.device}: there is no CPU fallback")
        if self.device.index is None:
            self.device = torch.device("cuda", torch.cuda.current_device())
        self.encoder_only = bool(encoder_only)
        self.max_batch = int(max_batch)
        self.lib = L.load()
        if self.lib.xl_abi_version() != L.XL_ABI_VERSION:
            raise RuntimeError("libxlstm_b200.so ABI mismatch")
        c = L.XLConfig(
            embedding_dim=cfg.d, num_blocks=cfg.num_blocks, num_heads=cfg.num_heads, inner_dim=cfg.inner,
            conv_kernel=cfg.conv1d_kernel_size, qkv_blocksize=cfg.qkv_proj_blocksize, state_dim=cfg.state_dim,
            act_dim=cfg.act_dim, action_channels=cfg.action_channels, discrete_actions=cfg.discrete_actions,
            tokens_per_step=cfg.tokens_per_step, action_token_pos=cfg.action_token_pos, max_batch=self.max_batch,
            ln_eps=cfg.ln_eps, cell_eps=cfg.cell_eps, embed_ln_eps=cfg.embed_ln_eps, tok_min_val=-1.0,
            tok_max_val=1.0, slstm_mask_lo=cfg.slstm_mask & 0xFFFFFFFF, slstm_mask_hi=cfg.slstm_mask >> 32,
            ffn_dim=cfg.ffn_dim if cfg.slstm_at else 0)
        self.handle = C.c_void_p()
        with torch.cuda.device(self.device):
            L.check(self.lib.xl_create(C.byref(c), C.byref(self.handle)))
        self._weights = []
        with torch.cuda.device(self.device):
            self._bind_all(strip_checkpoint_prefixes(state_dict))
            L.check((self.lib.xl_encoder_weights_ready if self.encoder_only else self.lib.xl_weights_ready)(self.handle))

    def _bind(self, layer: int, slot: str, t: torch.Tensor, bf16: bool):
        t = t.detach().to(self.device, torch.bfloat16 if bf16 else torch.float32).contiguous()
        self._weights.append(t)
        L.check(self.lib.xl_bind_weight(self.handle, layer, L.W[slot], _ptr(t), 1 if bf16 else 0, t.numel()))

    def _bind_all(self, sd):
        cfg = self.cfg
        for i in range(cfg.num_blocks):
            slstm = cfg.is_slstm(i)
            for key, slot in (_SLSTM_BLOCK_KEYS if slstm else _BLOCK_KEYS).items():
                name = f"encoder.layers.blocks.{i}.{key}"
                if name not in sd:
                    raise KeyError(f"state_dict is missing {name}")
                t = sd[name]
                if slot == "CONV_W":
                    t = t.reshape(cfg.d if slstm else cfg.inner, cfg.conv1d_kernel_size)
                self._bind(i, slot, t, is_bf16_weight(name))
        kpad = self.lib.xl_state_dim_padded(self.handle)
        for name, slot in _POLICY_KEYS.items():
            if self.encoder_only and slot != "POST_NORM":
                continue
            if name not in sd:
                raise KeyError(f"state_dict is missing {name}")
            t = sd[name]
            if slot == "EMBED_STATE_W":
                w = torch.zeros(cfg.d, kpad, dtype=torch.float32)
                w[:, : cfg.state_dim] = t.detach().float().cpu()
                t = w
            elif slot in ("EMBED_RETURN_W", "EMBED_REWARD_W"):
                t = t.reshape(-1)
            self._bind(-1, slot, t, is_bf16_weight(name))

    def new_state(self, B: int) -> StateCache:
        if B > self.max_batch:
            raise ValueError(f"B={B} > max_batch={self.max_batch}")
        return StateCache(self, B)

    def _stream(self):
        return C.c_void_p(torch.cuda.current_stream(self.device).cuda_stream)

    @_on_device
    def reset(self, state: StateCache, mask: Optional[torch.Tensor] = None):
        if mask is not None:
            mask = mask.to(self.device, torch.uint8).contiguous()
            assert mask.numel() == state.B
        L.check(self.lib.xl_state_reset(self.handle, _ptr(state.buf), _ptr(mask), state.B, self._stream()))

    @_on_device
    def encoder_step(self, state: StateCache, x: torch.Tensor, mode: int = L.XL_MODE_FUSED, flags: int = 0,
                     out: Optional[torch.Tensor] = None):
        assert x.is_cuda and x.dtype == torch.float32 and x.dim() == 3 and x.shape[0] == state.B
        x = x.contiguous()
        if out is None:
            out = torch.empty_like(x)
        assert out.is_contiguous() and out.shape == x.shape and out.dtype == torch.float32
        L.check(self.lib.xl_encoder_step(self.handle, _ptr(state.buf), _ptr(x), _ptr(out), x.shape[0], x.shape[1],
                                         mode, flags, self._stream()))
        return out

    def prefill(self, state: StateCache, x: torch.Tensor, want_hidden: bool = True, flags: int = 0, lengths=None):
        lens = None if lengths is None else check_lengths(lengths, state.B, x.shape[1], "S")
        return self._prefill(state, x, want_hidden, flags, lens)

    @_on_device
    def _prefill(self, state, x, want_hidden, flags, lens):
        assert x.is_cuda and x.dtype == torch.float32 and x.dim() == 3 and x.shape[0] == state.B
        x = x.contiguous()
        out = torch.empty_like(x) if want_hidden else None
        if lens is None:
            L.check(self.lib.xl_prefill(self.handle, _ptr(state.buf), _ptr(x), _ptr(out), x.shape[0], x.shape[1],
                                        flags, self._stream()))
        else:
            L.check(self.lib.xl_prefill_ragged(self.handle, _ptr(state.buf), _ptr(x), _ptr(out),
                                               lens.ctypes.data_as(C.c_void_p), x.shape[0], x.shape[1], flags,
                                               self._stream()))
        return out

    def _check_state_embeds(self, states, B: int):
        want = f"an fp32 tensor [B={B}, Tn, d={self.cfg.d}] on {self.device}"
        if not isinstance(states, torch.Tensor):
            raise ValueError(f"state embeddings must be {want}, got {type(states).__name__}")
        if states.dim() != 3 or states.shape[0] != B or states.shape[2] != self.cfg.d:
            raise ValueError(f"state embeddings must be {want}, got shape {tuple(states.shape)}")
        if states.dtype != torch.float32:
            raise ValueError(f"state embeddings must be {want}, got {states.dtype}")
        if states.device != self.device:
            raise ValueError(f"state embeddings must be {want}, got a tensor on {states.device}")

    @staticmethod
    def _embeds_operand(states: torch.Tensor) -> torch.Tensor:
        states = states.contiguous()
        return states.clone() if states.data_ptr() % 16 else states

    def policy_prefill(self, state: StateCache, states: torch.Tensor, rtg: torch.Tensor,
                       rewards: Optional[torch.Tensor] = None, flags: int = 0, lengths=None,
                       state_embeds: bool = False):
        if state_embeds:
            self._check_state_embeds(states, state.B)
        lens = None if lengths is None else check_lengths(lengths, state.B, states.shape[1], "Tn")
        self._seq_call(state, states, rtg, rewards, lens, flags, state_embeds)

    @_on_device
    def _seq_call(self, state, states, rtg, rewards, lens, flags, state_embeds, outputs=None):
        B, Tn = state.B, states.shape[1]
        assert states.is_cuda and states.dtype == torch.float32 and tuple(states.shape) == \
            (B, Tn, self.cfg.d if state_embeds else self.cfg.state_dim)
        assert rtg.is_cuda and rtg.dtype == torch.float32 and rtg.numel() == B * Tn
        states = self._embeds_operand(states) if state_embeds else states.contiguous()
        rtg = rtg.contiguous()
        if rewards is not None:
            rewards = rewards.to(self.device, torch.float32).contiguous()
            assert rewards.numel() == B * Tn
        args = (self.handle, _ptr(state.buf), _ptr(states), _ptr(rtg), _ptr(rewards))
        lp = None if lens is None else lens.ctypes.data_as(C.c_void_p)
        if outputs is not None:
            fn = self.lib.xl_policy_forward_embeds if state_embeds else self.lib.xl_policy_forward
            rc = fn(*args, lp, B, Tn, C.byref(outputs), flags, self._stream())
        elif state_embeds:
            rc = self.lib.xl_policy_prefill_embeds(*args, lp, B, Tn, flags, self._stream())
        elif lens is None:
            rc = self.lib.xl_policy_prefill(*args, B, Tn, flags, self._stream())
        else:
            rc = self.lib.xl_policy_prefill_ragged(*args, lp, B, Tn, flags, self._stream())
        L.check(rc)

    def policy_forward(self, state: StateCache, states: torch.Tensor, rtg: torch.Tensor,
                       rewards: Optional[torch.Tensor] = None, lengths=None, discrete: bool = False,
                       targets: Optional[torch.Tensor] = None, want_logits: bool = False,
                       state_embeds: bool = False) -> dict:
        cfg = self.cfg
        if state_embeds:
            self._check_state_embeds(states, state.B)
        B, Tn = state.B, states.shape[1]
        lens = None if lengths is None else check_lengths(lengths, B, Tn, "Tn")
        if targets is not None:
            if not isinstance(targets, torch.Tensor):
                raise ValueError(f"targets must be a tensor, got {type(targets).__name__}")
            if targets.dtype.is_floating_point or targets.dtype.is_complex or targets.dtype == torch.bool:
                raise ValueError(f"targets must be integers, got {targets.dtype}")
            if tuple(targets.shape) != (B, Tn, cfg.act_dim):
                raise ValueError(f"targets must have shape {(B, Tn, cfg.act_dim)}, got {tuple(targets.shape)}")
            if targets.device != self.device:
                raise ValueError(f"targets must be on {self.device}, got {targets.device}")
            if targets.numel():
                lo, hi = (int(v) for v in torch.aminmax(targets))
                if lo < -1 or hi >= cfg.num_actions:
                    raise ValueError(f"targets must lie in [-1, num_actions={cfg.num_actions}), got min {lo} max {hi}")
        return self._policy_forward(state, states, rtg, rewards, lens, discrete, targets, want_logits, state_embeds)

    @_on_device
    def _policy_forward(self, state, states, rtg, rewards, lens, discrete, targets, want_logits, state_embeds=False):
        cfg = self.cfg
        B, Tn = state.B, states.shape[1]
        out = {"action_tokens": torch.empty(B, Tn, cfg.act_dim, dtype=torch.int32, device=self.device),
               "action_preds": torch.empty(B, Tn, cfg.act_dim, dtype=torch.float32, device=self.device)}
        if want_logits:
            n = cfg.num_actions if discrete else cfg.head_out
            out["action_logits"] = torch.empty(B, Tn, n, dtype=torch.float32, device=self.device)
        if targets is not None:
            targets = targets.to(torch.int32).contiguous()
            out["action_logprobs"] = torch.empty(B, Tn, cfg.act_dim, dtype=torch.float32, device=self.device)
        so = L.XLSeqOutputs(tokens=out["action_tokens"].data_ptr(), actions=out["action_preds"].data_ptr(),
                            logits=_ptr(out.get("action_logits")).value, targets=_ptr(targets).value,
                            logprobs=_ptr(out.get("action_logprobs")).value)
        self._seq_call(state, states, rtg, rewards, lens, L.XL_FLAG_DISCRETE if discrete else 0, state_embeds, so)
        return out

    @_on_device
    def policy_step(self, state: StateCache, states: torch.Tensor, rtg: torch.Tensor,
                    rewards: Optional[torch.Tensor] = None, mode: int = L.XL_MODE_FUSED, flags: int = 0,
                    want_logits: bool = False, want_hidden: bool = False, out: Optional[dict] = None,
                    state_embeds: bool = False):
        cfg = self.cfg
        B = state.B
        if state_embeds:
            flags |= L.XL_FLAG_STATE_EMBEDS
        want = (B, cfg.d) if (flags & L.XL_FLAG_STATE_EMBEDS) else (B, cfg.state_dim)
        assert states.is_cuda and states.dtype == torch.float32 and tuple(states.shape) == want, \
            f"states must be a cuda fp32 tensor of shape {want}, got {tuple(states.shape)}"
        assert rtg.is_cuda and rtg.dtype == torch.float32 and rtg.numel() == B
        states, rtg = states.contiguous(), rtg.contiguous()
        if rewards is not None:
            rewards = rewards.to(self.device, torch.float32).contiguous()
        if out is None:
            out = {"action_tokens": torch.zeros(B, cfg.act_dim, dtype=torch.int32, device=self.device),
                   "action_preds": torch.zeros(B, cfg.act_dim, dtype=torch.float32, device=self.device)}
            if want_logits:
                n = cfg.num_actions if (flags & L.XL_FLAG_DISCRETE) else cfg.head_out
                out["action_logits"] = torch.empty(B, n, dtype=torch.float32, device=self.device)
            if want_hidden:
                out["last_hidden_state"] = torch.empty(B, cfg.tokens_per_step, cfg.d, dtype=torch.float32,
                                                       device=self.device)
        L.check(self.lib.xl_policy_step(
            self.handle, _ptr(state.buf), _ptr(states), _ptr(rtg), _ptr(rewards), _ptr(out["action_tokens"]),
            _ptr(out["action_preds"]), _ptr(out.get("action_logits")), _ptr(out.get("last_hidden_state")), B,
            mode, flags, self._stream()))
        return out

    @_on_device
    def policy_step_host(self, state: StateCache, h_states: torch.Tensor, h_rtg: torch.Tensor,
                         h_tokens: torch.Tensor, h_actions: torch.Tensor, mode: int = L.XL_MODE_FUSED,
# ... 84 lines not shown
```

Baseline: 70330.

## Defer mLSTM C-state writeback on alternate steps via stashed rank-1 updates

When the matrix-memory state is large enough to stream, the TMA state-step kernel now skips writing the updated C on every other step. It instead stashes k, v and the forget factors in a per-head side buffer and replays those rank-1 updates on the next load, cutting roughly half of the C write traffic. A pending counter and stash region are appended to the state buffer. A new sync kernel, called before state inspection, reset, prefill and non-deferring steps, folds any pending updates back into C. This adds extra smem, replay FMAs and extra synchronization paths, with a risk of inconsistency when state is read externally.

Measured after the change: 72760 (median of 6 runs). 1.03x the previous value.

```diff
diff --git a/include/xlstm_b200.h b/include/xlstm_b200.h
--- a/include/xlstm_b200.h
+++ b/include/xlstm_b200.h
@@ -112,6 +112,8 @@
 size_t xl_state_bytes(const xl_handle* h, int B);
 int xl_state_layout(const xl_handle* h, int B, int layer, int part, size_t* offset_bytes, size_t* size_bytes);
 
+int xl_state_sync(xl_handle* h, void* state, int B, void* stream);
+
 int xl_state_reset(xl_handle* h, void* state, const uint8_t* env_mask, int B, void* stream);
 
 int xl_set_token_ring(xl_handle* h, int32_t* ring, int slots, int next_slot, void* stream);
diff --git a/lram_b200/_lib.py b/lram_b200/_lib.py
--- a/lram_b200/_lib.py
+++ b/lram_b200/_lib.py
@@ -98,6 +98,8 @@
     lib.xl_state_layout.restype = i32
     lib.xl_state_reset.argtypes = [vp, vp, vp, i32, vp]
     lib.xl_state_reset.restype = i32
+    lib.xl_state_sync.argtypes = [vp, vp, i32, vp]
+    lib.xl_state_sync.restype = i32
     lib.xl_encoder_step.argtypes = [vp, vp, vp, vp, i32, i32, i32, u32, vp]
     lib.xl_encoder_step.restype = i32
     lib.xl_mlstm_cell_step.argtypes = [vp, vp, vp, vp, vp, vp, vp, vp, vp, vp, i32, i32, i32, i32, vp]
diff --git a/lram_b200/csrc/xl_api.cu b/lram_b200/csrc/xl_api.cu
--- a/lram_b200/csrc/xl_api.cu
+++ b/lram_b200/csrc/xl_api.cu
@@ -168,6 +168,27 @@
   return (size_t)(i - ns) * L.layer_bytes + (size_t)ns * L.slayer_bytes;
 }
 
+struct PendLayout {
+  int blocks;
+  size_t stash_off, pending_off, end;
+};
+
+PendLayout pend_layout(const xl_handle* h, int B) {
+  const xl_config& c = h->cfg;
+  PendLayout P;
+  P.blocks = c.num_blocks - __builtin_popcountll(h->slstm_mask);
+  const size_t bnh = (size_t)B * c.num_heads;
+  P.stash_off = layer_base(h, state_layout(h, B), c.num_blocks);
+  P.pending_off = align_up(P.stash_off + sizeof(float) * P.blocks * bnh * xl::stash_floats(h->DH), 256);
+  P.end = align_up(P.pending_off + sizeof(int32_t) * P.blocks * bnh, 256);
+  return P;
+}
+
+int mlstm_index(const xl_handle* h, int i) {
+  const uint64_t below = i >= 64 ? ~0ull : ((1ull << i) - 1ull);
+  return i - __builtin_popcountll(h->slstm_mask & below);
+}
+
 int check_batch(const xl_handle* h, int B) {
   if (!h) return fail(XL_ERR_INVALID_ARG, "null handle");
   if (B <= 0 || B > h->cfg.max_batch)
@@ -316,6 +337,10 @@
   sp.out_hi = tc_down ? sl.ws.a_hi : nullptr;
   sp.out_lo = tc_down ? sl.ws.a_lo : nullptr;
   sp.partial = sl.ws.partial;
+  const PendLayout P = pend_layout(h, sl.B);
+  const size_t env0 = ((size_t)mlstm_index(h, i) * sl.B + sl.b0) * NH;
+  sp.pending = (int*)((char*)state + P.pending_off) + env0;
+  sp.stash = (float*)((char*)state + P.stash_off) + env0 * xl::stash_floats(DH);
   sp.B = sl.Bk; sp.T = T; sp.NH = NH; sp.DH = DH; sp.inner = inner; sp.NCH = h->NCH;
   if (small_nch) sp.NCH = small_nch;
   if (up_fused) sp.NCH = xl::gemm_up_conv_chunks(inner);
@@ -414,11 +439,52 @@
   return XL_OK;
 }
 
-int block_state(xl_handle* h, void* state, const Slice& sl, int i, int T, unsigned flags) {
+xl::StateStepParams stream_params(const xl_handle* h, void* state, const Slice& sl, int i, int T, unsigned flags) {
   const BlockPlan bp = block_plan(h, sl, T, flags);
   const int small_nch = smallm_chunks(h, sl, T, flags);
-  const xl::StateStepParams sp = small_nch ? state_params(h, state, sl, i, T, false, 1, small_nch)
-                                           : state_params(h, state, sl, i, T, bp.tc_down, bp.up_sp, 0, bp.up_fused);
+  return small_nch ? state_params(h, state, sl, i, T, false, 1, small_nch)
+                   : state_params(h, state, sl, i, T, bp.tc_down, bp.up_sp, 0, bp.up_fused);
+}
+
+int state_sync(xl_handle* h, void* state, int B, cudaStream_t s) {
+  const xl_config& c = h->cfg;
+  const StateLayout L = state_layout(h, B);
+  const PendLayout P = pend_layout(h, B);
+  const int bnh = B * c.num_heads;
+  xl::StateSyncParams q;
+  memset(&q, 0, sizeof(q));
+  q.state = (char*)state;
+  q.BNH = bnh;
+  q.DH = h->DH;
+  for (int i = 0, j = 0; i < c.num_blocks; ++i) {
+    if (is_slstm(h, i)) continue;
+    if (q.blocks == 0) {
+      q.pending = (int*)((char*)state + P.pending_off) + (size_t)j * bnh;
+      q.stash = (float*)((char*)state + P.stash_off) + (size_t)j * bnh * xl::stash_floats(h->DH);
+    }
+    q.c_off[q.blocks++] = (int64_t)(layer_base(h, L, i) + L.c_off);
+    ++j;
+    if (q.blocks == xl::kMaxStateBlocks || j == P.blocks) {
+      xl::launch_state_sync(q, s);
+      h->launches += 1;
+      q.blocks = 0;
+    }
+  }
+  XL_CUDA(cudaGetLastError());
+  return XL_OK;
+}
+
+int sync_unless_deferring(xl_handle* h, void* state, const Slice& sl, int T, unsigned flags) {
+  int i = 0;
+  while (i < h->cfg.num_blocks && is_slstm(h, i)) ++i;
+  if (i == h->cfg.num_blocks) return XL_OK;
+  const xl::StateStepParams sp = stream_params(h, state, sl, i, T, flags);
+  if (!xl::state_streams(sp) || xl::state_step_defers(sp, h->num_sms)) return XL_OK;
+  return state_sync(h, state, sl.B, sl.s);
+}
+
+int block_state(xl_handle* h, void* state, const Slice& sl, int i, int T, unsigned flags) {
+  const xl::StateStepParams sp = stream_params(h, state, sl, i, T, flags);
   cudaEvent_t pe0 = nullptr, pe1 = nullptr;
   if (h->profiling) {
     XL_CUDA(cudaEventCreate(&pe0));
@@ -719,6 +785,9 @@
   const int d = c.embedding_dim, T = c.tokens_per_step;
   const float* post_w = (const float*)h->pw[XL_W_POST_NORM - XL_W_POST_NORM];
   const int MB = pick_microbatches(h, a.B, a.mode);
+  if (int rc = sync_unless_deferring(h, a.state, make_slice(h, a.B, 0, a.B, s),
+                                     a.mode == XL_MODE_FUSED ? T : 1, a.flags))
+    return rc;
   if (MB == 1) {
     const Slice sl = make_slice(h, a.B, 0, a.B, s);
     float* xt = (a.mode == XL_MODE_FUSED) ? sl.ws.x : sl.ws.xtok;
@@ -1403,7 +1472,14 @@
 
 size_t xl_state_bytes(const xl_handle* h, int B) {
   if (!h || B <= 0) return 0;
-  return layer_base(h, state_layout(h, B), h->cfg.num_blocks);
+  return pend_layout(h, B).end;
+}
+
+int xl_state_sync(xl_handle* h, void* state, int B, void* stream) {
+  int rc = check_batch(h, B);
+  if (rc) return rc;
+  if (!state) return fail(XL_ERR_INVALID_ARG, "null state");
+  return state_sync(h, state, B, (cudaStream_t)stream);
 }
 
 int xl_state_layout(const xl_handle* h, int B, int layer, int part, size_t* offset_bytes, size_t* size_bytes) {
@@ -1442,9 +1518,10 @@
   const StateLayout L = state_layout(h, B);
   const xl_config& c = h->cfg;
   if (!env_mask) {
-    XL_CUDA(cudaMemsetAsync(state, 0, layer_base(h, L, c.num_blocks), s));
+    XL_CUDA(cudaMemsetAsync(state, 0, xl_state_bytes(h, B), s));
     return XL_OK;
   }
+  if ((rc = state_sync(h, state, B, s))) return rc;
   for (int i = 0; i < c.num_blocks; ++i) {
     char* base = (char*)state + layer_base(h, L, i);
     if (is_slstm(h, i)) {
@@ -1474,9 +1551,11 @@
   rc = weights_ready(h, true);
   if (rc) return rc;
   cudaStream_t s = (cudaStream_t)stream;
+  const int step_T = (mode == XL_MODE_FUSED || T == 1) ? T : 1;
   if (!(flags & XL_FLAG_GRAPH) || h->profiling) {
     const Slice sl = make_slice(h, B, 0, B, s);
-    return run_encoder(h, state, sl, x_in, x_out, T, mode, flags & ~(unsigned)XL_FLAG_GRAPH);
+    rc = sync_unless_deferring(h, state, sl, step_T, flags);
+    return rc ? rc : run_encoder(h, state, sl, x_in, x_out, T, mode, flags & ~(unsigned)XL_FLAG_GRAPH);
   }
   const int key_mode = mode | (T << 8) | (1 << 16);
   for (auto& g : h->graphs) {
@@ -1494,7 +1573,8 @@
   XL_CUDA(cudaStreamBeginCapture(h->cap_stream, cudaStreamCaptureModeThreadLocal));
   {
     const Slice sl = make_slice(h, B, 0, B, h->cap_stream);
-    rc = run_encoder(h, state, sl, x_in, x_out, T, mode, flags & ~(unsigned)XL_FLAG_GRAPH);
+    rc = sync_unless_deferring(h, state, sl, step_T, flags);
+    if (!rc) rc = run_encoder(h, state, sl, x_in, x_out, T, mode, flags & ~(unsigned)XL_FLAG_GRAPH);
   }
   cudaError_t e = cudaStreamEndCapture(h->cap_stream, &graph);
   g.launches = h->launches - before;
@@ -1764,6 +1844,7 @@
       if (nzero == B) return XL_OK;
     }
   }
+  if ((rc = state_sync(h, c.state, B, s))) return rc;
   SeqPlan p;
   p.T = enc ? 1 : cf.tokens_per_step;
   if ((rc = seq_plan(h, c.state, lengths, B, S, p, s))) return rc;
diff --git a/lram_b200/csrc/xl_internal.h b/lram_b200/csrc/xl_internal.h
--- a/lram_b200/csrc/xl_internal.h
+++ b/lram_b200/csrc/xl_internal.h
@@ -144,8 +144,22 @@
   int num_layers;
   int max_cluster;
   int fuse_finalize;
+  int* pending;
+  float* stash;
   float ln_eps, cell_eps;
 };
+__host__ __device__ inline int64_t stash_floats(int DH) { return (int64_t)8 * DH + 4; }
+bool state_streams(const StateStepParams& p);
+bool state_step_defers(StateStepParams p, int num_sms);
+constexpr int kMaxStateBlocks = 64;
+struct StateSyncParams {
+  char* state;
+  int64_t c_off[kMaxStateBlocks];
+  int* pending;
+  float* stash;
+  int blocks, BNH, DH;
+};
+void launch_state_sync(const StateSyncParams& q, cudaStream_t s);
 cudaError_t launch_state_step(StateStepParams p, int num_sms, cudaStream_t s);
 bool state_step_fuses_finalize(StateStepParams p, int num_sms);
 cudaError_t launch_state_finalize(StateStepParams p, int num_sms, cudaStream_t s);
diff --git a/lram_b200/csrc/xl_state_step.cu b/lram_b200/csrc/xl_state_step.cu
--- a/lram_b200/csrc/xl_state_step.cu
+++ b/lram_b200/csrc/xl_state_step.cu
@@ -490,6 +490,20 @@
   if (tid == 0) p.m[tc.bh] = s_m[T];
 }
 
+__device__ __forceinline__ void mbar_expect_tx_only(uint32_t bar, uint32_t bytes) {
+  asm volatile("mbarrier.expect_tx.relaxed.cta.shared::cta.b64 [%0], %1;" ::"r"(bar), "r"(bytes) : "memory");
+}
+
+constexpr int kReplayMax = 4;
+constexpr int kReplayRing = 2 * kStages;
+__device__ __forceinline__ void flip_pending(const StateStepParams& p, int64_t bh, int ts, int T, int tid, int nthreads) {
+  if (ts) {
+    float* stash = p.stash + bh * stash_floats(p.DH);
+    for (int e = tid; e < stash_floats(p.DH); e += nthreads) stash[e] = 0.f;
+  }
+  if (tid == 0) p.pending[bh] = ts ? 0 : T;
+}
+
 template <int T, bool kStream, bool kFused>
 __global__ void __launch_bounds__(kBlock, 3)
 mlstm_state_stream_tma_kernel(const __grid_constant__ CUtensorMap mapC, StateStepParams p) {
@@ -497,10 +511,12 @@
   __shared__ float s_f[T], s_i[T], s_m[T + 1], s_pre[2 * T];
   __shared__ __align__(8) uint64_t s_bar[2 * kStages + 2];
   __shared__ float s_red[4 * 32], s_x[kMaxCluster * 8];
+  __shared__ __align__(16) float s_fr[kReplayMax];
 
   const TileCoord tc = tile_coord(p);
   const int DH = p.DH;
   const int W = p.cols_per_cta;
+  const bool defer = kStream && p.pending != nullptr;
   const bool leader = kFused && p.fuse_finalize == 2 && tc.rs == 0 && tc.cs == 0;
   const bool head_qk = leader && p.rows_split > 1;
   const int TX = W >> 2, TY = kThreads / TX;
@@ -515,6 +531,8 @@
   float* sn = sqk + (size_t)T * tstride;
   float* snum = sn + DH;
   float* sqkh = snum + (size_t)p.rows_split * T * DH;
+  float* svr = kFused ? sqkh + (p.rows_split > 1 ? (size_t)2 * T * DH : 0) : sqk + (size_t)T * tstride;
+  float* skr = svr + (size_t)kReplayMax * W;
   float* sacc = stage0;
   const uint32_t bar0 = smem_u32(s_bar);
   auto full_bar = [&](int s) { return bar0 + 8u * s; };
@@ -547,10 +565,21 @@
       uint64_t policy = 0;
       if (kStream) asm volatile("createpolicy.fractional.L2::evict_first.b64 %0, 1.0;" : "=l"(policy));
       const int grow0 = tc.slab_row0;
-      auto issue = [&](int i) {
+      const float* stash = defer ? p.stash + (int64_t)tc.bh * stash_floats(DH) : nullptr;
+      int ts = 0;
+      auto replay_k_bytes = [&](int i) { return (uint32_t)(ts * min(kStageRows, tc.nrows - i * kStageRows) * 4); };
+      auto load_replay_k = [&](int i) {
+        const int sk = i % kReplayRing;
+        for (int t = 0; t < ts; ++t)
+          bulk_copy_g2s(smem_u32(skr + (sk * kReplayMax + t) * kStageRows), stash + t * DH + tc.r0 + i * kStageRows,
+                        replay_k_bytes(i) / ts, full_bar(i % kStages));
+      };
+      auto issue = [&](int i, bool arrive) {
         const int s = i % kStages;
         mbar_wait(empty_bar(s), ((i / kStages) & 1) ^ 1);
-        mbar_expect_tx(full_bar(s), stage_bytes);
+        if (arrive) mbar_expect_tx(full_bar(s), stage_bytes + replay_k_bytes(i));
+        else mbar_expect_tx_only(full_bar(s), stage_bytes);
+        if (arrive && ts) load_replay_k(i);
         const uint32_t dst = sbase + s * stage_bytes;
         if (kStream) {
           asm volatile(
@@ -566,11 +595,14 @@
         }
       };
       const int pre = nblk < kStages ? nblk : kStages;
-      for (int i = 0; i < pre; ++i) issue(i);
+      for (int i = 0; i < pre; ++i) issue(i, !defer);
       pdl_wait();
       pdl_trigger();
       if (kFused) cluster_wait();
-      mbar_expect_tx(qk_bar, (uint32_t)(T * tc.nrows * 8 + (kFused ? DH * 4 : 0) + (head_qk ? T * DH * 8 : 0)));
+      if (defer) ts = p.pending[tc.bh];
+      const uint32_t qk_bytes = (uint32_t)(T * tc.nrows * 8 + (kFused ? DH * 4 : 0) + (head_qk ? T * DH * 8 : 0));
+      if (defer) mbar_expect_tx_only(qk_bar, qk_bytes);
+      else mbar_expect_tx(qk_bar, qk_bytes);
       if (kFused) bulk_copy_g2s(smem_u32(sn), p.n + (int64_t)tc.bh * DH, (uint32_t)(DH * 4), qk_bar);
       if (head_qk) {
 #pragma unroll
@@ -583,7 +615,19 @@
         bulk_copy_g2s(smem_u32(sqk + t * tstride),
                       p.qk + ((((int64_t)tc.b * T + t) * p.NH + tc.hd) * DH + tc.r0) * 2,
                       (uint32_t)(tc.nrows * 8), qk_bar);
-      for (int i = pre; i < nblk; ++i) issue(i);
+      if (defer) {
+        for (int i = 0; i < pre; ++i) {
+          mbar_expect_tx(full_bar(i), replay_k_bytes(i));
+          if (ts) load_replay_k(i);
+        }
+        mbar_expect_tx(qk_bar, ts ? 16u + (uint32_t)(ts * W * 4) : 0u);
+        if (ts) {
+          bulk_copy_g2s(smem_u32(s_fr), stash + 8 * DH, 16u, qk_bar);
+          for (int t = 0; t < ts; ++t)
+            bulk_copy_g2s(smem_u32(svr + t * W), stash + (kReplayMax + t) * DH + tc.c0, (uint32_t)(W * 4), qk_bar);
+        }
+      }
+      for (int i = pre; i < nblk; ++i) issue(i, true);
     } else {
       pdl_wait();
       pdl_trigger();
@@ -622,10 +666,28 @@
   const int64_t rs4 = tc.wc >> 2;
   constexpr int kRowsPerThread = 4;
   const bool fast = (TY * kRowsPerThread == kStageRows);
+  const int ts = defer ? p.pending[tc.bh] : 0;
+  const bool write_c = !defer || ts > 0;
   mbar_wait(qk_bar, 0);
+  if (defer && ts == 0) {
+    float* stash = p.stash + (int64_t)tc.bh * stash_floats(DH);
+    if (tc.rs == 0 && ty == 0) {
+#pragma unroll
+      for (int t = 0; t < T; ++t)
+        *reinterpret_cast<float4*>(stash + (kReplayMax + t) * DH + tc.c0 + 4 * tx) =
+            make_float4(vi[t][0], vi[t][1], vi[t][2], vi[t][3]);
+      if (tc.cs == 0 && tid < T) stash[2 * kReplayMax * DH + tid] = s_f[tid];
+    }
+    if (tc.cs == 0)
+      for (int e = tid; e < T * tc.nrows; e += kThreads) {
+        const int t = e / tc.nrows, r = e - t * tc.nrows;
+        stash[t * DH + tc.r0 + r] = sqk[t * tstride + 2 * r + 1];
+      }
+  }
   for (int i = 0; i < nblk; ++i) {
     const int s = i % kStages;
     const float* st = stage0 + (size_t)s * kStageRows * W;
+    const float* kr = skr + (i % kReplayRing) * kReplayMax * kStageRows;
     const int rblk = i * kStageRows;
     const int rcur = min(kStageRows, tc.nrows - rblk);
     mbar_wait(full_bar(s), (i / kStages) & 1);
@@ -636,21 +698,44 @@
         cv[j] = *reinterpret_cast<const float4*>(st + (ty + j * 8) * W + 4 * tx);
       __syncwarp();
       if (lane == 0) mbar_arrive(empty_bar(s));
+      for (int t = 0; t < ts; ++t) {
+        const float ft = s_fr[t];
+        const float4 vr = *reinterpret_cast<const float4*>(svr + t * W + 4 * tx);
+#pragma unroll
+        for (int j = 0; j < kRowsPerThread; ++j) {
+          const float k = kr[t * kStageRows + ty + j * 8];
+          cv[j].x = fmaf(ft, cv[j].x, k * vr.x);
+          cv[j].y = fmaf(ft, cv[j].y, k * vr.y);
+          cv[j].z = fmaf(ft, cv[j].z, k * vr.z);
+          cv[j].w = fmaf(ft, cv[j].w, k * vr.w);
+        }
+      }
       float4* rp = Cp + (int64_t)(rblk + ty) * rs4;
 #pragma unroll
       for (int j = 0; j < kRowsPerThread; ++j) {
         float c[4] = {cv[j].x, cv[j].y, cv[j].z, cv[j].w};
         row_update<T>(c, sqk + 2 * (rblk + ty + j * 8), tstride, f, vi, acc);
         const float4 o = make_float4(c[0], c[1], c[2], c[3]);
-        if (kStream) st_stream(rp + (int64_t)j * 8 * rs4, o);
-        else rp[(int64_t)j * 8 * rs4] = o;
+        if (kStream) {
+          if (write_c) st_stream(rp + (int64_t)j * 8 * rs4, o);
+        } else {
+          rp[(int64_t)j * 8 * rs4] = o;
+        }
       }
     } else {
       for (int r = ty; r < rcur; r += TY) {
-        const float4 cv = *reinterpret_cast<const float4*>(st + r * W + 4 * tx);
+        float4 cv = *reinterpret_cast<const float4*>(st + r * W + 4 * tx);
+        for (int t = 0; t < ts; ++t) {
+          const float ft = s_fr[t], k = kr[t * kStageRows + r];
+          const float4 vr = *reinterpret_cast<const float4*>(svr + t * W + 4 * tx);
+          cv.x = fmaf(ft, cv.x, k * vr.x);
+          cv.y = fmaf(ft, cv.y, k * vr.y);
+          cv.z = fmaf(ft, cv.z, k * vr.z);
+          cv.w = fmaf(ft, cv.w, k * vr.w);
+        }
         float c[4] = {cv.x, cv.y, cv.z, cv.w};
         row_update<T>(c, sqk + 2 * (rblk + r), tstride, f, vi, acc);
-        Cp[(int64_t)(rblk + r) * rs4] = make_float4(c[0], c[1], c[2], c[3]);
+        if (write_c) Cp[(int64_t)(rblk + r) * rs4] = make_float4(c[0], c[1], c[2], c[3]);
       }
       __syncwarp();
       if (lane == 0) mbar_arrive(empty_bar(s));
@@ -667,6 +752,7 @@
       leader_finalize<T>(p, tc, sacc, sqk, sqkh, sn, snum, tstride, s_f, s_i, s_m, s_red, xbar, tid);
     else
       fused_finalize<T>(p, tc, sacc, sqk, sn, tstride, s_f, s_i, s_m, s_red, s_x, xbar, tid);
+    if (defer && tc.rs == 0 && tc.cs == 0) flip_pending(p, tc.bh, ts, T, tid, kThreads);
     return;
   }
   write_partials<T>(p, tc, sacc, acc, tx, ty, TX, TY, tid);
@@ -707,7 +793,8 @@
   const size_t red = sizeof(float) * (size_t)TY * T * p.cols_per_cta;
   const size_t smem = 128 + (ring > red ? ring : red) +
                       sizeof(float) * ((size_t)2 * T * rows_per +
-                                       (kFused ? (size_t)p.DH * (1 + T * p.rows_split + (p.rows_split > 1 ? 2 * T : 0)) : 0));
+                                       (kFused ? (size_t)p.DH * (1 + T * p.rows_split + (p.rows_split > 1 ? 2 * T : 0)) : 0) +
+                                       (kStream ? (size_t)kReplayMax * (p.cols_per_cta + kReplayRing * kStageRows) : 0));
   if (cudaError_t e = ensure_dyn_smem<&mlstm_state_stream_tma_kernel<T, kStream, kFused>>(smem); e != cudaSuccess)
     return e;
   const int CS = p.DH / p.cols_per_cta;
@@ -753,6 +840,7 @@
 using tma::bulk_copy_g2s;
 using tma::mbar_arrive;
 using tma::mbar_expect_tx;
+using tma::mbar_expect_tx_only;
 using tma::mbar_init;
 using tma::mbar_wait;
 using tma::smem_u32;
@@ -764,10 +852,6 @@
 constexpr int kConsumerWarps = kThreads / 32;
 constexpr int kBlock = kThreads + 64;
 constexpr int kStageFloats = kStageRows * kW;
-
-__device__ __forceinline__ void mbar_expect_tx_only(uint32_t bar, uint32_t bytes) {
-  asm volatile("mbarrier.expect_tx.relaxed.cta.shared::cta.b64 [%0], %1;" ::"r"(bar), "r"(bytes) : "memory");
-}
 
 __host__ __device__ inline int meta_floats(int T, int DH) { return T * DH * 2 + T * kW + 16; }
 
@@ -1031,6 +1115,7 @@
 __global__ void __launch_bounds__(1024) mlstm_state_finalize_kernel(StateStepParams p) {
   __shared__ float s_f[T], s_i[T], s_m[T + 1], s_pre[2 * T];
   __shared__ float s_red[T * 32];
+  __shared__ int s_pend;
   const int bh = blockIdx.x;
   const int b = bh / p.NH, hd = bh - b * p.NH;
   const int DH = p.DH, inner = p.inner, RS = p.rows_split;
@@ -1043,6 +1128,7 @@
   const float wskip = (ok && p.skip) ? p.skip[ch] : 0.f;
   float2 qk[T];
   float num[T], act[T], zz[T];
+  if (p.pending && threadIdx.x == 0) s_pend = p.pending[bh];
   int sk_item = 0, sk_nseg = 0;
   if (p.sk_grid > 0 && ok) {
     const int nblk = DH >> 5;
@@ -1128,6 +1214,52 @@
     }
   }
   if (threadIdx.x == 0) p.m[bh] = s_m[T];
+  if (p.pending) tma::flip_pending(p, bh, s_pend, T, a, blockDim.x);
+}
+
+__global__ void __launch_bounds__(256) mlstm_state_sync_kernel(const __grid_constant__ StateSyncParams q) {
+  pdl_wait();
+  pdl_trigger();
+  const int j = blockIdx.y;
+  const int64_t bh = blockIdx.x;
+  int* pending = q.pending + (int64_t)j * q.BNH + bh;
+  const int ts = *pending;
+  if (ts == 0) return;
+  const int DH = q.DH, wc = slab_width(DH), TX = wc / 4, TY = blockDim.x / TX;
+  const int tx = threadIdx.x % TX, ty = threadIdx.x / TX;
+  float* stash = q.stash + ((int64_t)j * q.BNH + bh) * stash_floats(DH);
+  float* C = reinterpret_cast<float*>(q.state + q.c_off[j]) + bh * DH * DH;
+  if (ty < TY) {
+    for (int slab = 0; slab < DH / wc; ++slab) {
+      const int col = slab * wc + 4 * tx;
+      float f[tma::kReplayMax];
+      float4 vr[tma::kReplayMax];
+      for (int t = 0; t < ts; ++t) {
+        f[t] = stash[2 * tma::kReplayMax * DH + t];
+        vr[t] = *reinterpret_cast<const float4*>(stash + (tma::kReplayMax + t) * DH + col);
+      }
+      for (int r = ty; r < DH; r += TY) {
+        float4* cp = reinterpret_cast<float4*>(C + ((int64_t)slab * DH + r) * wc + 4 * tx);
+        float4 c = *cp;
+        for (int t = 0; t < ts; ++t) {
+          const float k = stash[t * DH + r];
+          c.x = fmaf(f[t], c.x, k * vr[t].x);
+          c.y = fmaf(f[t], c.y, k * vr[t].y);
+          c.z = fmaf(f[t], c.z, k * vr[t].z);
+          c.w = fmaf(f[t], c.w, k * vr[t].w);
+        }
+        *cp = c;
+      }
+    }
+  }
+  __syncthreads();
+  for (int e = threadIdx.x; e < stash_floats(DH); e += blockDim.x) stash[e] = 0.f;
+  if (threadIdx.x == 0) *pending = 0;
+}
+
+void launch_state_sync(const StateSyncParams& q, cudaStream_t s) {
+  if (q.blocks == 0) return;
+  launch_k(mlstm_state_sync_kernel, dim3((unsigned)q.BNH, (unsigned)q.blocks), dim3(256), 0, s, q);
 }
 
 void state_step_auto_tiling(int B, int NH, int DH, int num_sms, int* rows_split, int* cols_per_cta) {
@@ -1147,14 +1279,23 @@
          (p.cols_per_cta <= 0 || p.cols_per_cta == pers::kW);
 }
 
+bool state_streams(const StateStepParams& p) {
+  const size_t c_bytes = sizeof(float) * (size_t)p.B * p.NH * p.DH * p.DH;
+  return c_bytes * (size_t)(p.num_layers > 0 ? p.num_layers : 1) > ((size_t)64 << 20);
+}
+
+static bool tma_ok(const StateStepParams& p) {
+  const int rows_per = (p.DH + p.rows_split - 1) / p.rows_split;
+  return p.sk_grid == 0 && p.impl >= 1 && rows_per % 4 == 0;
+}
+
 template <int T>
 static cudaError_t launch_T(const StateStepParams& p, cudaStream_t s) {
-  const size_t c_bytes = sizeof(float) * (size_t)p.B * p.NH * p.DH * p.DH;
-  const bool stream = c_bytes * (size_t)(p.num_layers > 0 ? p.num_layers : 1) > ((size_t)64 << 20);
+  const bool stream = state_streams(p);
   if (p.sk_grid > 0) return stream ? pers::launch<T, true>(p, s) : pers::launch<T, false>(p, s);
   const int rows_per = (p.DH + p.rows_split - 1) / p.rows_split;
   cudaError_t e;
-  if (p.impl >= 1 && rows_per % 4 == 0) {
+  if (tma_ok(p)) {
     if (p.fuse_finalize == 1 || p.fuse_finalize == 2)
       e = stream ? tma::launch<T, true, true>(p, s) : tma::launch<T, false, true>(p, s);
     else
@@ -1219,7 +1360,22 @@
   }
 }
 
+bool state_step_defers(StateStepParams p, int num_sms) {
+  if (!p.pending) return false;
+  drop_unfusable(p, num_sms);
+  resolve_tiling(p, num_sms);
+  return state_streams(p) && tma_ok(p);
+}
+
+static void drop_pending(StateStepParams& p, int num_sms) {
+  if (!state_step_defers(p, num_sms)) {
+    p.pending = nullptr;
+    p.stash = nullptr;
+  }
+}
+
 cudaError_t launch_state_finalize(StateStepParams p, int num_sms, cudaStream_t s) {
+  drop_pending(p, num_sms);
   drop_unfusable(p, num_sms);
   resolve_tiling(p, num_sms);
   const int thr = ((p.DH + 31) / 32) * 32;
@@ -1234,6 +1390,7 @@
 }
 
 cudaError_t launch_state_step(StateStepParams p, int num_sms, cudaStream_t s) {
+  drop_pending(p, num_sms);
   drop_unfusable(p, num_sms);
   resolve_tiling(p, num_sms);
   if (p.cols_per_cta % 4 || p.DH % p.cols_per_cta || slab_width(p.DH) % p.cols_per_cta ||
diff --git a/lram_b200/engine.py b/lram_b200/engine.py
--- a/lram_b200/engine.py
+++ b/lram_b200/engine.py
@@ -97,6 +97,7 @@
         self.buf = torch.zeros(nbytes // 4, dtype=torch.float32, device=engine.device)
 
     def view(self, layer: int, part: int) -> torch.Tensor:
+        self.engine.sync(self)
         off, size = C.c_size_t(), C.c_size_t()
         L.check(self.engine.lib.xl_state_layout(self.engine.handle, self.B, layer, part, C.byref(off), C.byref(size)))
         flat = self.buf[off.value // 4: (off.value + size.value) // 4]
@@ -271,6 +272,10 @@
         L.check(self.lib.xl_state_reset(self.handle, _ptr(state.buf), _ptr(mask), state.B, self._stream()))
 
     @_on_device
+    def sync(self, state: StateCache):
+        L.check(self.lib.xl_state_sync(self.handle, _ptr(state.buf), state.B, self._stream()))
+
+    @_on_device
     def encoder_step(self, state: StateCache, x: torch.Tensor, mode: int = L.XL_MODE_FUSED, flags: int = 0,
                      out: Optional[torch.Tensor] = None):
         assert x.is_cuda and x.dtype == torch.float32 and x.dim() == 3 and x.shape[0] == state.B
```
